# ratschlab/metagraph

Measured on AMD Instinct MI355X. Metric: aligned reads/sec (150 bp, k=31), higher is better.
Workload: dtype int32; 1 GPU; 10000000 synthetic 150 bp reads per GPU vs 104197894-edge k=31 BOSS graph (98 Mbp iid genome + 200000 SNP windows), CLI-default scoring; reads_per_gpu=10000000, graph_edges=104197894, k=31, graph_mode=basic, parallelism=reads sharded x1, graph replicated

## Files before the change

### include/mgx.h

```cpp
#ifndef MGX_H_
#define MGX_H_

#include <stddef.h>
#include <stdint.h>

#ifdef __cplusplus
extern "C" {
#endif

#define MGX_ABI_VERSION 6

enum {
    MGX_OK = 0,
    MGX_ERR_INVALID = -1,
    MGX_ERR_NO_DEVICE = -2,
    MGX_ERR_UNSUPPORTED = -3,
    MGX_ERR_CONFIG = -4,
    MGX_ERR_CAPACITY = -5,
    MGX_ERR_OOM = -6
};

enum { MGX_MODE_BASIC = 0, MGX_MODE_CANONICAL = 1, MGX_MODE_PRIMARY = 2 };

enum { MGX_OP_CLIPPED = 0, MGX_OP_MISMATCH = 1, MGX_OP_MATCH = 2,
       MGX_OP_DELETION = 3, MGX_OP_INSERTION = 4, MGX_OP_NODE_INSERTION = 5 };

typedef struct mgx_boss_view {
    uint32_t k;
    uint32_t sigma;
    uint64_t n_edges;
    const uint8_t *W;
    const uint8_t *last;
    const uint64_t *F;
    const uint8_t *valid;
    uint32_t mode;
    uint32_t on_device;
} mgx_boss_view;

typedef struct mgx_config {
    uint64_t num_alternative_paths;
    uint64_t min_seed_length;
    uint64_t max_seed_length;
    uint64_t max_num_seeds_per_locus;
    int32_t min_cell_score;
    int32_t min_path_score;
    int32_t xdrop;
    int32_t _pad0;
    double min_exact_match;
    double max_nodes_per_seq_char;
    double max_ram_per_alignment;
    double rel_score_cutoff;
    int8_t gap_opening_penalty;
    int8_t gap_extension_penalty;
    int8_t left_end_bonus;
    int8_t right_end_bonus;
    uint8_t forward_and_reverse_complement;
    uint8_t chain_alignments;
    uint8_t post_chain_alignments;
    uint8_t global_xdrop;
    uint8_t allow_left_trim;
    uint8_t no_backtrack;
    uint8_t seed_complexity_filter;
    uint8_t alignment_edit_distance;
    int8_t alignment_match_score;
    int8_t alignment_mm_transition_score;
    int8_t alignment_mm_transversion_score;
    uint8_t _pad1[1];
    int8_t score_matrix[128][128];
} mgx_config;

void mgx_config_init_default(mgx_config *c);
void mgx_config_init_cli(mgx_config *c, uint32_t k);
void mgx_config_set_dna_matrix(mgx_config *c, int8_t match, int8_t mm_transition, int8_t mm_transversion);
void mgx_config_set_unit_matrix(mgx_config *c, int8_t match);
void mgx_config_set_scoring_matrix(mgx_config *c);

#define MGX_MAX_ALTERNATIVE_PATHS 4u

#define MGX_MAX_QUERY_LENGTH 32704u

typedef struct mgx_limits {
    uint32_t max_query_length;
    uint32_t max_columns;
    uint32_t max_seeds;
    uint64_t cell_arena_bytes;
} mgx_limits;
void mgx_limits_init_default(mgx_limits *l, uint32_t max_query_length);
int mgx_aligner_get_limits(const struct mgx_aligner *a, mgx_limits *out);

typedef struct mgx_graph mgx_graph;
typedef struct mgx_aligner mgx_aligner;

typedef struct mgx_cigar_op { uint32_t len; uint8_t op; uint8_t _pad[3]; } mgx_cigar_op;

typedef struct mgx_alignment {
    int32_t score;
    uint32_t offset;
    uint32_t clipping;
    uint32_t end_clipping;
    uint32_t num_matches;
    uint32_t n_nodes;
    uint32_t n_cigar;
    uint32_t seq_len;
    uint64_t nodes_begin;
    uint64_t cigar_begin;
    uint64_t seq_begin;
    uint8_t orientation;
    uint8_t _pad[3];
    uint32_t n_labels;
    uint64_t labels_begin;
} mgx_alignment;

typedef struct mgx_results {
    uint64_t n_queries;
    const uint64_t *aln_begin;
    const mgx_alignment *alignments;
    const uint64_t *nodes;
    const mgx_cigar_op *cigar;
    const char *seqs;
    const int32_t *status;
    const uint32_t *labels;
} mgx_results;

typedef struct mgx_mapping {
    uint64_t n_queries;
    const uint64_t *node_begin;
    const uint64_t *nodes_fwd;
    const uint64_t *nodes_rc;
} mgx_mapping;

typedef struct mgx_stats {
    uint64_t n_reads;
    uint64_t n_rank_lines;
    uint64_t n_select_lines;
    uint64_t n_bit_lines;
    uint64_t n_columns;
    uint64_t n_extensions;
    uint64_t n_seeds;
    uint64_t n_map_lines;
    uint64_t n_capacity_errors;
    uint64_t phase_cycles[8];
    uint64_t extend_cycles[8];
    double seed_kernel_ms, align_kernel_ms;
    double seeding_ms, sort_ms, extend_ms;
    uint64_t n_seed_lines;
    uint64_t n_fast_columns;
    uint64_t extend_kernels;
    uint64_t n_lane_reads;
    double lane_ms;
    uint64_t n_lane_lines;
    uint64_t n_lane_columns;
    uint64_t lane_bail_reads[32];
    uint64_t n_capacity_retried;
    uint64_t n_seed_lane_reads;
    double seed_lane_ms;
    uint64_t seed_lane_left_reads[16];
    uint64_t n_lane_exact_reads;
    uint64_t n_lane_exact_path_reads;
} mgx_stats;
enum { MGX_KERNEL_GRP8 = 1, MGX_KERNEL_GRP8_PRIM = 2, MGX_KERNEL_GRP8_ALT = 4, MGX_KERNEL_EXT64 = 8, MGX_KERNEL_LANE = 16,
       MGX_KERNEL_LAB64 = 32, MGX_KERNEL_GRP8_LAB = 64,
       MGX_KERNEL_LAB64_BX = 128, MGX_KERNEL_GRP8_LAB_BX = 256  };

int mgx_device_count(void);
const char *mgx_last_error(void);
uint32_t mgx_abi_version(void);

int mgx_graph_create(const mgx_boss_view *view, int device, mgx_graph **out);
void mgx_graph_destroy(mgx_graph *g);
uint32_t mgx_graph_k(const mgx_graph *g);
uint64_t mgx_graph_max_index(const mgx_graph *g);
uint64_t mgx_graph_device_bytes(const mgx_graph *g);
uint64_t mgx_graph_num_edges(const mgx_graph *g);
uint32_t mgx_graph_mode(const mgx_graph *g);

int mgx_aligner_create(const mgx_graph *g, const mgx_config *config,
                       const mgx_limits *limits, mgx_aligner **out);
void mgx_aligner_destroy(mgx_aligner *a);
int mgx_aligner_get_config(const mgx_aligner *a, mgx_config *out);

int mgx_align_batch(mgx_aligner *a, const char *seqs, const uint64_t *offsets, uint64_t n_queries,
                    int seqs_on_device, mgx_results *out);

int mgx_align_batch_device(mgx_aligner *a, const char *seqs, const uint64_t *offsets, uint64_t n_queries,
                           int seqs_on_device);
int mgx_fetch_results(mgx_aligner *a, mgx_results *out);
int mgx_device_results(mgx_aligner *a, const void **headers, uint64_t *header_bytes, uint64_t *n_queries,
                       const void **stream, uint64_t *stream_words);
typedef struct mgx_results_sizes { uint64_t n_alignments, n_nodes, n_cigar, n_seq_bytes, n_labels; } mgx_results_sizes;
int mgx_decode_results_device(mgx_aligner *a, mgx_results *out, mgx_results_sizes *sizes);
void mgx_decode_kernel_launch_counts(uint64_t *out4);
uint64_t mgx_device_stream_capacity(const mgx_aligner *a);
typedef struct mgx_raw_store mgx_raw_store;
int mgx_results_from_raw(const void *headers, uint64_t n_queries, const uint32_t *stream, uint64_t stream_words,
                         mgx_raw_store **store, mgx_results *out);
void mgx_raw_store_free(mgx_raw_store *store);
int mgx_chain_alignments(const mgx_config *config, uint32_t k, const mgx_results *in, const char *seqs, const uint64_t *offsets,
                         mgx_raw_store **store, mgx_results *out);
void mgx_aligner_keep_seeds(mgx_aligner *a, int keep);
int mgx_fetch_seed_info(mgx_aligner *a, uint32_t *info6, uint32_t *seeds, uint32_t *max_seeds_out);

int mgx_map_batch(mgx_aligner *a, const char *seqs, const uint64_t *offsets, uint64_t n_queries,
                  int seqs_on_device, mgx_mapping *out);

typedef struct mgx_map_counts { uint32_t n_discovered, n_kmers, n_unique; } mgx_map_counts;
typedef struct mgx_map_summary {
    uint64_t n_queries;
    const mgx_map_counts *counts;
    const uint64_t *node_begin;
    const uint64_t *nodes;
} mgx_map_summary;
enum { MGX_MAP_WANT_NODES = 1, MGX_MAP_KEEP_NODES = 2 };
int mgx_map_summary_batch(mgx_aligner *a, const char *seqs, const uint64_t *offsets, uint64_t n_queries,
                          int seqs_on_device, uint32_t map_length ,
                          uint32_t flags, mgx_map_summary *out);
int mgx_map_present(const mgx_map_counts *c, uint64_t query_len, uint32_t k, uint32_t map_length, double discovery_fraction);
enum { MGX_MAP_FMT_NODES = 0, MGX_MAP_FMT_COUNT_KMERS = 1, MGX_MAP_FMT_QUERY_PRESENCE = 2, MGX_MAP_FMT_FILTER_PRESENT = 3 };
size_t mgx_format_map(const mgx_map_summary *s, uint64_t query_index, const char *header, const char *query, size_t query_len,
                      uint32_t k, uint32_t map_length, int format, double discovery_fraction, char *buf, size_t buf_len);
void mgx_map_kernel_launch_counts(uint64_t *out4);

int mgx_aligner_stats(const mgx_aligner *a, mgx_stats *out);
void mgx_kernel_launch_counts(uint64_t *out5);

int mgx_aligner_set_pipeline(mgx_aligner *a, const char *name);
int mgx_device_trim(int device);
int mgx_aligner_set_stream(mgx_aligner *a, void *hip_stream);
int mgx_aligner_create_stream(mgx_aligner *a);
void *mgx_aligner_get_stream(const mgx_aligner *a);

typedef struct mgx_gather mgx_gather;
uint64_t mgx_gather_unique_id_bytes(void);
int mgx_gather_unique_id(void *id_out, uint64_t id_bytes);
int mgx_gather_create_rank(const void *unique_id, uint64_t id_bytes, int rank, int world, int root, int device, mgx_gather **out);
int mgx_gather_create_comm(void *nccl_comm, int rank, int world, int root, int device, mgx_gather **out);
int mgx_gather_create_local(const int *devices, int n_devices, int root, mgx_gather **out );
void mgx_gather_destroy(mgx_gather *g);
int mgx_gather_world(const mgx_gather *g);
int mgx_gather_rank(const mgx_gather *g);
int mgx_gather_start(mgx_gather *g, mgx_aligner *a);
int mgx_gather_finish(mgx_gather *g, uint64_t *n_queries, const void **headers, const uint32_t **streams, uint64_t *stream_words);

size_t mgx_format_tsv(const mgx_results *res, uint64_t query_index, const char *header,
                      const char *query, size_t query_len, int32_t min_path_score,
                      char *buf, size_t buf_len);

size_t mgx_format_json(const mgx_results *res, uint64_t query_index, const char *header,
                       const char *query, size_t query_len, uint32_t k, char *buf, size_t buf_len);

typedef struct mgx_annotation mgx_annotation;
int mgx_annotation_create(uint64_t n_rows, uint32_t n_labels, const uint64_t *const *columns, int device, mgx_annotation **out);
int mgx_annotation_create_sparse(uint64_t n_rows, uint32_t n_labels, const uint64_t *col_begin, const uint64_t *rows,
                                 int on_device, int device, mgx_annotation **out);
void mgx_annotation_destroy(mgx_annotation *a);
uint64_t mgx_annotation_device_bytes(const mgx_annotation *a);
uint64_t mgx_annotation_num_rows(const mgx_annotation *a);
uint32_t mgx_annotation_num_labels(const mgx_annotation *a);
int mgx_annotation_get_rows(mgx_annotation *a, const uint64_t *rows, uint64_t n, int rows_on_device,
                            uint64_t *out_begin, uint32_t *out_labels, uint64_t cap, int out_on_device, uint64_t *n_labels_out);

int mgx_annotation_set_coordinates(mgx_annotation *a, uint32_t n_labels, const uint64_t *col_begin, const uint64_t *rows,
                                   const uint64_t *coord_begin, const int64_t *coords);
int mgx_annotation_set_coordinates_device(mgx_annotation *a, uint32_t n_labels, const uint64_t *col_begin, const uint64_t *rows,
                                          const uint64_t *coord_begin, const int64_t *coords);
int mgx_annotation_has_coordinates(const mgx_annotation *a);
int mgx_annotation_get_row_tuples(mgx_annotation *a, const uint64_t *rows, uint64_t n, uint64_t *out_begin, uint32_t *out_labels,
                                  uint64_t label_cap, uint64_t *out_coord_begin, int64_t *out_coords, uint64_t coord_cap,
                                  uint64_t *n_labels_out, uint64_t *n_coords_out);

typedef struct mgx_chain_anchor {
    uint64_t label;
    int64_t coordinate;
    int32_t seed_clipping, seed_end;
    int32_t chain_score;
    uint32_t seed_index;
} mgx_chain_anchor;
int mgx_chain_seeds(const mgx_config *config, int device, const mgx_chain_anchor *anchors, const uint64_t *list_begin,
                    const uint32_t *query_size, uint64_t n_lists, mgx_chain_anchor *sorted_out, uint32_t *backtrace_out);

int mgx_seed_chainer_create(const mgx_graph *graph, const mgx_config *config, const mgx_limits *limits,
                            const struct mgx_annotation *annotation, mgx_aligner **out);
typedef struct mgx_chain_seed { uint32_t clipping, length, offset, n_nodes; uint64_t nodes_begin; } mgx_chain_seed;
typedef struct mgx_chain_tables {
    uint64_t n_queries;
    const uint64_t *seed_begin;
    const mgx_chain_seed *seeds;
    const uint64_t *nodes;
    const uint64_t *num_matching;
    const uint64_t *list_begin;
    const mgx_chain_anchor *anchors;
    const uint32_t *backtrace;
    const int32_t *status;
} mgx_chain_tables;
#define MGX_CHAIN_TABLES_ON_DEVICE 1u
int mgx_chain_tables_batch(mgx_aligner *a, const char *seqs, const uint64_t *offsets, uint64_t n, int seqs_on_device,
                           uint32_t flags, mgx_chain_tables *out);
int mgx_chain_tables_fetch(mgx_aligner *a, mgx_chain_tables *out_host);
void mgx_chain_tables_kernel_launch_counts(uint64_t *out4);

int mgx_labeled_aligner_create(const mgx_graph *graph, const mgx_config *config, const mgx_limits *limits,
                               const mgx_annotation *annotation, mgx_aligner **out);
size_t mgx_format_tsv_labeled(const mgx_results *res, uint64_t query_index, const char *header,
                              const char *query, size_t query_len, int32_t min_path_score,
                              const char *const *label_names, uint32_t n_label_names, char *buf, size_t buf_len);
typedef struct mgx_text {
    uint64_t n_queries;
    const char *text;
    const uint64_t *line_begin;
} mgx_text;
int mgx_format_tsv_batch(mgx_aligner *a, const char *headers, const uint64_t *header_offsets,
                         const char *const *label_names, uint32_t n_label_names, mgx_text *out);
void mgx_format_kernel_launch_counts(uint64_t *out4);
int mgx_format_map_batch(mgx_aligner *a, const char *headers, const uint64_t *header_offsets, int format,
                         double discovery_fraction, mgx_text *out);
void mgx_format_map_kernel_launch_counts(uint64_t *out4);
int mgx_format_json_batch(mgx_aligner *a, const char *headers, const uint64_t *header_offsets,
                          uint64_t first, uint64_t n, mgx_text *out);
void mgx_format_json_kernel_launch_counts(uint64_t *out4);

#define MGX_READS_FASTA 1u
#define MGX_READS_FASTQ 2u
typedef struct mgx_read_parser mgx_read_parser;
typedef struct mgx_reads {
    uint64_t n_records, consumed;
    uint32_t format;
    const char *seqs;
    const uint64_t *offsets;
    const uint64_t *host_offsets;
    const char *names;
    const uint64_t *name_offsets;
} mgx_reads;
int mgx_read_parser_create(int device, mgx_read_parser **out);
void mgx_read_parser_destroy(mgx_read_parser *p);
int mgx_parse_reads(mgx_read_parser *p, const char *text, uint64_t n_bytes, int text_on_device, int final, uint32_t flags,
                    mgx_reads *out);
int mgx_read_parser_slice(mgx_read_parser *p, uint64_t first, uint64_t n, const char **seqs, const uint64_t **offsets);
int mgx_read_parser_fetch(mgx_read_parser *p, char *seqs_out, uint64_t *offsets_out);
void mgx_parse_kernel_launch_counts(uint64_t *out4);
void *mgx_pinned_alloc(size_t bytes);
void mgx_pinned_free(void *p);

int mgx_results_from_raw_labeled(const void *headers, uint64_t n_queries, const uint32_t *stream, uint64_t stream_words,
                                 int labeled, mgx_raw_store **store, mgx_results *out);

typedef struct mgx_boss_file {
    uint32_t k;
    uint32_t sigma;
    uint32_t mode;
    uint32_t state;
    uint64_t n_edges;
    const uint64_t *F;
    const uint8_t *W;
    const uint8_t *last;
    void *owner;
} mgx_boss_file;
int mgx_boss_file_read(const char *path, mgx_boss_file *out);
void mgx_boss_file_free(mgx_boss_file *f);
int mgx_edgemask_read(const char *path, uint32_t state, uint64_t n_edges, uint8_t *valid_out);
int mgx_graph_load_dbg(const char *path, int device, mgx_graph **out);
int mgx_graph_load_dbg_device(const char *path, int device, mgx_graph **out);
int mgx_boss_file_decode_device(const char *path, int device, mgx_boss_file *out);
void mgx_dbg_decode_kernel_launch_counts(uint64_t *out4);

typedef struct mgx_column_file mgx_column_file;
int mgx_column_file_read(const char *const *paths, uint32_t n_paths, mgx_column_file **out);
void mgx_column_file_free(mgx_column_file *f);
uint64_t mgx_column_file_num_rows(const mgx_column_file *f);
uint32_t mgx_column_file_num_labels(const mgx_column_file *f);
const char *mgx_column_file_label(const mgx_column_file *f, uint32_t j);
const uint64_t *mgx_column_file_col_begin(const mgx_column_file *f);
const uint64_t *mgx_column_file_rows(const mgx_column_file *f);
int mgx_annotation_create_from_file(const mgx_column_file *f, int device, mgx_annotation **out);
int mgx_column_coord_file_read(const char *const *paths, uint32_t n_paths, mgx_column_file **out);
const uint64_t *mgx_column_file_coord_begin(const mgx_column_file *f);
const int64_t *mgx_column_file_coords(const mgx_column_file *f);
int mgx_annotation_load_columns_device(const char *const *paths, uint32_t n_paths, int device, mgx_annotation **out, mgx_column_file **names_out);
int mgx_column_file_decode_device(const char *const *paths, uint32_t n_paths, int device, mgx_column_file **out);
int mgx_annotation_load_coord_columns_device(const char *const *paths, uint32_t n_paths, int device, mgx_annotation **out, mgx_column_file **names_out);
int mgx_column_coord_file_decode_device(const char *const *paths, uint32_t n_paths, int device, mgx_column_file **out);
void mgx_column_decode_kernel_launch_counts(uint64_t *out4);

#ifdef __cplusplus
}
#endif
#endif
```

### metagraph_amd/capi.py

```python
import ctypes as C
import os

MGX_OK = 0
MGX_ABI_VERSION = 6
MGX_ERR_INVALID, MGX_ERR_NO_DEVICE, MGX_ERR_UNSUPPORTED, MGX_ERR_CONFIG, MGX_ERR_CAPACITY, MGX_ERR_OOM = -1, -2, -3, -4, -5, -6
OP_CHARS = "SX=DIG"


class BossView(C.Structure):
    _fields_ = [("k", C.c_uint32), ("sigma", C.c_uint32), ("n_edges", C.c_uint64),
                ("W", C.c_void_p), ("last", C.c_void_p), ("F", C.POINTER(C.c_uint64)),
                ("valid", C.c_void_p), ("mode", C.c_uint32), ("on_device", C.c_uint32)]


class BossFile(C.Structure):
    _fields_ = [("k", C.c_uint32), ("sigma", C.c_uint32), ("mode", C.c_uint32), ("state", C.c_uint32), ("n_edges", C.c_uint64),
                ("F", C.POINTER(C.c_uint64)), ("W", C.POINTER(C.c_uint8)), ("last", C.POINTER(C.c_uint8)), ("owner", C.c_void_p)]


class Config(C.Structure):
    _fields_ = [("num_alternative_paths", C.c_uint64), ("min_seed_length", C.c_uint64),
                ("max_seed_length", C.c_uint64), ("max_num_seeds_per_locus", C.c_uint64),
                ("min_cell_score", C.c_int32), ("min_path_score", C.c_int32), ("xdrop", C.c_int32),
                ("_pad0", C.c_int32),
                ("min_exact_match", C.c_double), ("max_nodes_per_seq_char", C.c_double),
                ("max_ram_per_alignment", C.c_double), ("rel_score_cutoff", C.c_double),
                ("gap_opening_penalty", C.c_int8), ("gap_extension_penalty", C.c_int8),
                ("left_end_bonus", C.c_int8), ("right_end_bonus", C.c_int8),
                ("forward_and_reverse_complement", C.c_uint8), ("chain_alignments", C.c_uint8),
                ("post_chain_alignments", C.c_uint8), ("global_xdrop", C.c_uint8),
                ("allow_left_trim", C.c_uint8), ("no_backtrack", C.c_uint8),
                ("seed_complexity_filter", C.c_uint8), ("alignment_edit_distance", C.c_uint8),
                ("alignment_match_score", C.c_int8), ("alignment_mm_transition_score", C.c_int8),
                ("alignment_mm_transversion_score", C.c_int8), ("_pad1", C.c_uint8 * 1),
                ("score_matrix", (C.c_int8 * 128) * 128)]


class Limits(C.Structure):
    _fields_ = [("max_query_length", C.c_uint32), ("max_columns", C.c_uint32), ("max_seeds", C.c_uint32),
                ("cell_arena_bytes", C.c_uint64)]


class CigarOp(C.Structure):
    _fields_ = [("len", C.c_uint32), ("op", C.c_uint8), ("_pad", C.c_uint8 * 3)]


class Alignment(C.Structure):
    _fields_ = [("score", C.c_int32), ("offset", C.c_uint32), ("clipping", C.c_uint32),
                ("end_clipping", C.c_uint32), ("num_matches", C.c_uint32), ("n_nodes", C.c_uint32),
                ("n_cigar", C.c_uint32), ("seq_len", C.c_uint32), ("nodes_begin", C.c_uint64),
                ("cigar_begin", C.c_uint64), ("seq_begin", C.c_uint64), ("orientation", C.c_uint8),
                ("_pad", C.c_uint8 * 3), ("n_labels", C.c_uint32), ("labels_begin", C.c_uint64)]


class Results(C.Structure):
    _fields_ = [("n_queries", C.c_uint64), ("aln_begin", C.POINTER(C.c_uint64)),
                ("alignments", C.POINTER(Alignment)), ("nodes", C.POINTER(C.c_uint64)),
                ("cigar", C.POINTER(CigarOp)), ("seqs", C.POINTER(C.c_char)), ("status", C.POINTER(C.c_int32)),
                ("labels", C.POINTER(C.c_uint32))]


class ResultsSizes(C.Structure):
    _fields_ = [("n_alignments", C.c_uint64), ("n_nodes", C.c_uint64), ("n_cigar", C.c_uint64), ("n_seq_bytes", C.c_uint64),
                ("n_labels", C.c_uint64)]


class Mapping(C.Structure):
    _fields_ = [("n_queries", C.c_uint64), ("node_begin", C.POINTER(C.c_uint64)),
                ("nodes_fwd", C.POINTER(C.c_uint64)), ("nodes_rc", C.POINTER(C.c_uint64))]


class MapCounts(C.Structure):
    _fields_ = [("n_discovered", C.c_uint32), ("n_kmers", C.c_uint32), ("n_unique", C.c_uint32)]


class MapSummary(C.Structure):
    _fields_ = [("n_queries", C.c_uint64), ("counts", C.POINTER(MapCounts)),
                ("node_begin", C.POINTER(C.c_uint64)), ("nodes", C.POINTER(C.c_uint64))]


class Text(C.Structure):
    _fields_ = [("n_queries", C.c_uint64), ("text", C.c_void_p), ("line_begin", C.POINTER(C.c_uint64))]


class Reads(C.Structure):
    _fields_ = [("n_records", C.c_uint64), ("consumed", C.c_uint64), ("format", C.c_uint32), ("seqs", C.c_void_p),
                ("offsets", C.c_void_p), ("host_offsets", C.POINTER(C.c_uint64)), ("names", C.c_void_p),
                ("name_offsets", C.POINTER(C.c_uint64))]


class ChainAnchor(C.Structure):
    _fields_ = [("label", C.c_uint64), ("coordinate", C.c_int64), ("seed_clipping", C.c_int32), ("seed_end", C.c_int32),
                ("chain_score", C.c_int32), ("seed_index", C.c_uint32)]


class ChainSeed(C.Structure):
    _fields_ = [("clipping", C.c_uint32), ("length", C.c_uint32), ("offset", C.c_uint32), ("n_nodes", C.c_uint32),
                ("nodes_begin", C.c_uint64)]


class ChainTables(C.Structure):
    _fields_ = [("n_queries", C.c_uint64), ("seed_begin", C.POINTER(C.c_uint64)), ("seeds", C.POINTER(ChainSeed)),
                ("nodes", C.POINTER(C.c_uint64)), ("num_matching", C.POINTER(C.c_uint64)), ("list_begin", C.POINTER(C.c_uint64)),
                ("anchors", C.POINTER(ChainAnchor)), ("backtrace", C.POINTER(C.c_uint32)), ("status", C.POINTER(C.c_int32))]


MGX_CHAIN_TABLES_ON_DEVICE = 1
MGX_READS_FASTA, MGX_READS_FASTQ = 1, 2
MGX_MAP_WANT_NODES = 1
MGX_MAP_KEEP_NODES = 2
MGX_MAP_FMT_NODES, MGX_MAP_FMT_COUNT_KMERS, MGX_MAP_FMT_QUERY_PRESENCE, MGX_MAP_FMT_FILTER_PRESENT = 0, 1, 2, 3


class Stats(C.Structure):
    _fields_ = [("n_reads", C.c_uint64), ("n_rank_lines", C.c_uint64), ("n_select_lines", C.c_uint64),
                ("n_bit_lines", C.c_uint64), ("n_columns", C.c_uint64), ("n_extensions", C.c_uint64),
                ("n_seeds", C.c_uint64), ("n_map_lines", C.c_uint64), ("n_capacity_errors", C.c_uint64), ("phase_cycles", C.c_uint64 * 8), ("extend_cycles", C.c_uint64 * 8),
                ("seed_kernel_ms", C.c_double), ("align_kernel_ms", C.c_double),
                ("seeding_ms", C.c_double), ("sort_ms", C.c_double), ("extend_ms", C.c_double), ("n_seed_lines", C.c_uint64),
                ("n_fast_columns", C.c_uint64), ("extend_kernels", C.c_uint64), ("n_lane_reads", C.c_uint64),
                ("lane_ms", C.c_double), ("n_lane_lines", C.c_uint64), ("n_lane_columns", C.c_uint64),
                ("lane_bail_reads", C.c_uint64 * 32), ("n_capacity_retried", C.c_uint64),
                ("n_seed_lane_reads", C.c_uint64), ("seed_lane_ms", C.c_double), ("seed_lane_left_reads", C.c_uint64 * 16),
                ("n_lane_exact_reads", C.c_uint64), ("n_lane_exact_path_reads", C.c_uint64)]


KERNEL_GRP8, KERNEL_GRP8_PRIM, KERNEL_GRP8_ALT, KERNEL_EXT64, KERNEL_LANE, KERNEL_LAB64, KERNEL_GRP8_LAB = 1, 2, 4, 8, 16, 32, 64
KERNEL_LAB64_BX, KERNEL_GRP8_LAB_BX = 128, 256


def results_to_py(res):
    out = []
    for q in range(res.n_queries):
        alns = []
        for ai in range(res.aln_begin[q], res.aln_begin[q + 1]):
            a = res.alignments[ai]
            nodes = [res.nodes[a.nodes_begin + i] for i in range(a.n_nodes)]
            cig = "".join("%d%s" % (res.cigar[a.cigar_begin + i].len, OP_CHARS[res.cigar[a.cigar_begin + i].op])
                          for i in range(a.n_cigar))
            seq = C.string_at(C.addressof(res.seqs.contents) + a.seq_begin, a.seq_len).decode() if a.seq_len else ""
            d = {"score": a.score, "offset": a.offset, "clipping": a.clipping,
                 "end_clipping": a.end_clipping, "num_matches": a.num_matches, "nodes": nodes,
                 "cigar": cig, "sequence": seq, "orientation": int(a.orientation)}
            if res.labels:
                d["labels"] = [res.labels[a.labels_begin + i] for i in range(a.n_labels)]
            alns.append(d)
        out.append(alns)
    return out


def chain_alignments(config, k, res, queries):
    import numpy as np
    blob = b"".join(q.encode() if isinstance(q, str) else bytes(q) for q in queries)
    offs = np.zeros(len(queries) + 1, dtype=np.uint64)
    offs[1:] = np.cumsum([len(q) for q in queries])
    store, out = C.c_void_p(), Results()
    rc = lib().mgx_chain_alignments(C.byref(config), k, C.byref(res), blob, offs.ctypes.data, C.byref(store), C.byref(out))
    if rc:
        raise RuntimeError(lib().mgx_last_error().decode())
    try:
        return results_to_py(out)
    finally:
        lib().mgx_raw_store_free(store)


def results_arrays(res):
    import numpy as np
    n = int(res.n_queries)

    def arr(ptr, count, dtype):
        if not count:
            return np.zeros(0, dtype=dtype)
        nbytes = count * np.dtype(dtype).itemsize
        return np.frombuffer((C.c_char * nbytes).from_address(C.addressof(ptr.contents)), dtype=dtype, count=count)

    aln_begin = arr(res.aln_begin, n + 1, np.uint64)
    na = int(aln_begin[-1]) if n else 0
    aln_dt = np.dtype([("score", "<i4"), ("offset", "<u4"), ("clipping", "<u4"), ("end_clipping", "<u4"),
                       ("num_matches", "<u4"), ("n_nodes", "<u4"), ("n_cigar", "<u4"), ("seq_len", "<u4"),
                       ("nodes_begin", "<u8"), ("cigar_begin", "<u8"), ("seq_begin", "<u8"), ("orientation", "u1"),
                       ("_pad", "u1", (3,)), ("n_labels", "<u4"), ("labels_begin", "<u8")])
    assert aln_dt.itemsize == C.sizeof(Alignment)
    alns = arr(res.alignments, na, aln_dt)
    tn = int(alns["n_nodes"].sum()) if na else 0
    tc = int(alns["n_cigar"].sum()) if na else 0
    ts = int(alns["seq_len"].sum()) if na else 0
    cig_dt = np.dtype([("len", "<u4"), ("op", "u1"), ("_pad", "u1", (3,))])
    return {"n": n, "aln_begin": aln_begin, "alns": alns, "nodes": arr(res.nodes, tn, np.uint64),
            "cigar": arr(res.cigar, tc, cig_dt), "seqs": arr(res.seqs, ts, np.uint8),
            "status": arr(res.status, n, np.int32)}


def count_result_mismatches(res_a, res_b):
    import numpy as np
    a, b = results_arrays(res_a), results_arrays(res_b)
    assert a["n"] == b["n"]
    fields = ["score", "offset", "clipping", "end_clipping", "num_matches", "n_nodes", "n_cigar", "seq_len", "orientation"]
    same = np.array_equal(a["aln_begin"], b["aln_begin"]) and len(a["alns"]) == len(b["alns"]) \
        and all(np.array_equal(a["alns"][f], b["alns"][f]) for f in fields) \
        and np.array_equal(a["nodes"], b["nodes"]) and np.array_equal(a["cigar"]["len"], b["cigar"]["len"]) \
        and np.array_equal(a["cigar"]["op"], b["cigar"]["op"]) and np.array_equal(a["seqs"], b["seqs"])
    if same:
        return 0
    pa, pb = results_to_py(res_a), results_to_py(res_b)
    return sum(1 for x, y in zip(pa, pb) if x != y)


_ROOT = os.path.dirname(os.path.dirname(os.path.abspath(__file__)))
LIB_PATH = os.environ.get("MGX_LIB_PATH") or os.path.join(_ROOT, "metagraph_amd", "_build", "libmgx.so")
_lib = None


def lib():
    global _lib
    if _lib is not None:
        return _lib
    if not os.path.exists(LIB_PATH):
        raise OSError("libmgx.so not built: run `python -c 'import __graft_entry__ as g; g.build()'` "
                      "(needs hipcc); the aligner has no CPU fallback")
    L = C.CDLL(LIB_PATH)
    L.mgx_last_error.restype = C.c_char_p
    L.mgx_abi_version.restype = C.c_uint32
    if L.mgx_abi_version() != MGX_ABI_VERSION:
        raise OSError("libmgx.so has ABI version %d, this binding was written for %d: rebuild" % (L.mgx_abi_version(), MGX_ABI_VERSION))
    L.mgx_annotation_create.argtypes = [C.c_uint64, C.c_uint32, C.POINTER(C.c_void_p), C.c_int, C.POINTER(C.c_void_p)]
    L.mgx_annotation_destroy.argtypes = [C.c_void_p]
    L.mgx_annotation_create_sparse.argtypes = [C.c_uint64, C.c_uint32, C.c_void_p, C.c_void_p, C.c_int, C.c_int, C.POINTER(C.c_void_p)]
    L.mgx_labeled_aligner_create.argtypes = [C.c_void_p, C.POINTER(Config), C.POINTER(Limits), C.c_void_p, C.POINTER(C.c_void_p)]
    L.mgx_seed_chainer_create.argtypes = [C.c_void_p, C.POINTER(Config), C.POINTER(Limits), C.c_void_p, C.POINTER(C.c_void_p)]
    L.mgx_chain_tables_batch.argtypes = [C.c_void_p, C.c_void_p, C.c_void_p, C.c_uint64, C.c_int, C.c_uint32, C.POINTER(ChainTables)]
    L.mgx_chain_tables_fetch.argtypes = [C.c_void_p, C.POINTER(ChainTables)]
    L.mgx_chain_tables_kernel_launch_counts.argtypes = [C.POINTER(C.c_uint64)]
    L.mgx_chain_tables_kernel_launch_counts.restype = None
    L.mgx_format_tsv_labeled.argtypes = [C.POINTER(Results), C.c_uint64, C.c_char_p, C.c_char_p, C.c_size_t, C.c_int32,
                                         C.POINTER(C.c_char_p), C.c_uint32, C.c_char_p, C.c_size_t]
    L.mgx_format_tsv_labeled.restype = C.c_size_t
    L.mgx_annotation_device_bytes.argtypes = [C.c_void_p]
    L.mgx_annotation_device_bytes.restype = C.c_uint64
    L.mgx_annotation_get_rows.argtypes = [C.c_void_p, C.c_void_p, C.c_uint64, C.c_int, C.c_void_p, C.c_void_p, C.c_uint64, C.c_int,
                                          C.POINTER(C.c_uint64)]
    L.mgx_device_count.restype = C.c_int
    L.mgx_boss_file_read.argtypes = [C.c_char_p, C.POINTER(BossFile)]
    L.mgx_boss_file_free.argtypes = [C.POINTER(BossFile)]
    L.mgx_edgemask_read.argtypes = [C.c_char_p, C.c_uint32, C.c_uint64, C.c_void_p]
    L.mgx_graph_load_dbg.argtypes = [C.c_char_p, C.c_int, C.POINTER(C.c_void_p)]
    L.mgx_graph_load_dbg_device.argtypes = [C.c_char_p, C.c_int, C.POINTER(C.c_void_p)]
    L.mgx_boss_file_decode_device.argtypes = [C.c_char_p, C.c_int, C.POINTER(BossFile)]
    L.mgx_dbg_decode_kernel_launch_counts.argtypes = [C.POINTER(C.c_uint64)]
    L.mgx_dbg_decode_kernel_launch_counts.restype = None
    L.mgx_column_file_read.argtypes = [C.POINTER(C.c_char_p), C.c_uint32, C.POINTER(C.c_void_p)]
    L.mgx_column_file_free.argtypes = [C.c_void_p]
    L.mgx_column_file_num_rows.argtypes = [C.c_void_p]
    L.mgx_column_file_num_rows.restype = C.c_uint64
    L.mgx_column_file_num_labels.argtypes = [C.c_void_p]
    L.mgx_column_file_num_labels.restype = C.c_uint32
    L.mgx_column_file_label.argtypes = [C.c_void_p, C.c_uint32]
    L.mgx_column_file_label.restype = C.c_char_p
    L.mgx_column_file_col_begin.argtypes = [C.c_void_p]
    L.mgx_column_file_col_begin.restype = C.POINTER(C.c_uint64)
    L.mgx_column_file_rows.argtypes = [C.c_void_p]
    L.mgx_column_file_rows.restype = C.POINTER(C.c_uint64)
    L.mgx_annotation_create_from_file.argtypes = [C.c_void_p, C.c_int, C.POINTER(C.c_void_p)]
    L.mgx_annotation_load_columns_device.argtypes = [C.POINTER(C.c_char_p), C.c_uint32, C.c_int, C.POINTER(C.c_void_p), C.POINTER(C.c_void_p)]
    L.mgx_column_file_decode_device.argtypes = [C.POINTER(C.c_char_p), C.c_uint32, C.c_int, C.POINTER(C.c_void_p)]
    L.mgx_column_coord_file_read.argtypes = [C.POINTER(C.c_char_p), C.c_uint32, C.POINTER(C.c_void_p)]
    L.mgx_column_file_coord_begin.argtypes = [C.c_void_p]
    L.mgx_column_file_coord_begin.restype = C.POINTER(C.c_uint64)
    L.mgx_column_file_coords.argtypes = [C.c_void_p]
    L.mgx_column_file_coords.restype = C.POINTER(C.c_int64)
    L.mgx_annotation_load_coord_columns_device.argtypes = [C.POINTER(C.c_char_p), C.c_uint32, C.c_int, C.POINTER(C.c_void_p), C.POINTER(C.c_void_p)]
    L.mgx_column_coord_file_decode_device.argtypes = [C.POINTER(C.c_char_p), C.c_uint32, C.c_int, C.POINTER(C.c_void_p)]
    L.mgx_column_decode_kernel_launch_counts.argtypes = [C.POINTER(C.c_uint64)]
    L.mgx_column_decode_kernel_launch_counts.restype = None
    L.mgx_graph_create.argtypes = [C.POINTER(BossView), C.c_int, C.POINTER(C.c_void_p)]
    L.mgx_graph_destroy.argtypes = [C.c_void_p]
    L.mgx_graph_k.argtypes = [C.c_void_p]
    L.mgx_graph_k.restype = C.c_uint32
    L.mgx_graph_max_index.argtypes = [C.c_void_p]
    L.mgx_graph_max_index.restype = C.c_uint64
    L.mgx_graph_device_bytes.argtypes = [C.c_void_p]
    L.mgx_graph_num_edges.argtypes = [C.c_void_p]
    L.mgx_graph_num_edges.restype = C.c_uint64
    L.mgx_graph_mode.argtypes = [C.c_void_p]
    L.mgx_graph_mode.restype = C.c_uint32
    L.mgx_graph_device_bytes.restype = C.c_uint64
    L.mgx_aligner_create.argtypes = [C.c_void_p, C.POINTER(Config), C.POINTER(Limits), C.POINTER(C.c_void_p)]
    L.mgx_aligner_destroy.argtypes = [C.c_void_p]
    L.mgx_aligner_get_config.argtypes = [C.c_void_p, C.POINTER(Config)]
    L.mgx_aligner_get_limits.argtypes = [C.c_void_p, C.POINTER(Limits)]
    L.mgx_align_batch.argtypes = [C.c_void_p, C.c_void_p, C.c_void_p, C.c_uint64, C.c_int, C.POINTER(Results)]
    L.mgx_align_batch_device.argtypes = [C.c_void_p, C.c_void_p, C.c_void_p, C.c_uint64, C.c_int]
    L.mgx_fetch_results.argtypes = [C.c_void_p, C.POINTER(Results)]
    L.mgx_aligner_keep_seeds.argtypes = [C.c_void_p, C.c_int]
    L.mgx_device_results.argtypes = [C.c_void_p, C.POINTER(C.c_void_p), C.POINTER(C.c_uint64), C.POINTER(C.c_uint64),
                                     C.POINTER(C.c_void_p), C.POINTER(C.c_uint64)]
    L.mgx_device_stream_capacity.argtypes = [C.c_void_p]
    L.mgx_device_stream_capacity.restype = C.c_uint64
    L.mgx_results_from_raw.argtypes = [C.c_void_p, C.c_uint64, C.c_void_p, C.c_uint64, C.POINTER(C.c_void_p), C.POINTER(Results)]
    L.mgx_chain_alignments.argtypes = [C.POINTER(Config), C.c_uint32, C.POINTER(Results), C.c_char_p, C.c_void_p,
                                       C.POINTER(C.c_void_p), C.POINTER(Results)]
    L.mgx_chain_alignments.restype = C.c_int
    L.mgx_results_from_raw_labeled.argtypes = [C.c_void_p, C.c_uint64, C.c_void_p, C.c_uint64, C.c_int, C.POINTER(C.c_void_p), C.POINTER(Results)]
    L.mgx_raw_store_free.argtypes = [C.c_void_p]
    L.mgx_gather_unique_id_bytes.restype = C.c_uint64
    L.mgx_gather_unique_id.argtypes = [C.c_void_p, C.c_uint64]
    L.mgx_gather_create_rank.argtypes = [C.c_void_p, C.c_uint64, C.c_int, C.c_int, C.c_int, C.c_int, C.POINTER(C.c_void_p)]
    L.mgx_gather_create_comm.argtypes = [C.c_void_p, C.c_int, C.c_int, C.c_int, C.c_int, C.POINTER(C.c_void_p)]
    L.mgx_gather_create_local.argtypes = [C.POINTER(C.c_int), C.c_int, C.c_int, C.POINTER(C.c_void_p)]
    L.mgx_gather_destroy.argtypes = [C.c_void_p]
    L.mgx_gather_destroy.restype = None
    L.mgx_gather_world.argtypes = [C.c_void_p]
    L.mgx_gather_rank.argtypes = [C.c_void_p]
    L.mgx_gather_start.argtypes = [C.c_void_p, C.c_void_p]
    L.mgx_gather_finish.argtypes = [C.c_void_p, C.POINTER(C.c_uint64), C.POINTER(C.c_void_p), C.POINTER(C.c_void_p), C.POINTER(C.c_uint64)]
    L.mgx_map_batch.argtypes = [C.c_void_p, C.c_void_p, C.c_void_p, C.c_uint64, C.c_int, C.POINTER(Mapping)]
    L.mgx_map_summary_batch.argtypes = [C.c_void_p, C.c_void_p, C.c_void_p, C.c_uint64, C.c_int, C.c_uint32, C.c_uint32,
                                        C.POINTER(MapSummary)]
    L.mgx_map_present.argtypes = [C.POINTER(MapCounts), C.c_uint64, C.c_uint32, C.c_uint32, C.c_double]
    L.mgx_format_map.argtypes = [C.POINTER(MapSummary), C.c_uint64, C.c_char_p, C.c_char_p, C.c_size_t, C.c_uint32, C.c_uint32,
                                 C.c_int, C.c_double, C.c_char_p, C.c_size_t]
    L.mgx_format_map.restype = C.c_size_t
    L.mgx_map_kernel_launch_counts.argtypes = [C.POINTER(C.c_uint64)]
    L.mgx_map_kernel_launch_counts.restype = None
    L.mgx_format_tsv_batch.argtypes = [C.c_void_p, C.c_char_p, C.c_void_p, C.POINTER(C.c_char_p), C.c_uint32, C.POINTER(Text)]
    L.mgx_format_kernel_launch_counts.argtypes = [C.POINTER(C.c_uint64)]
    L.mgx_format_kernel_launch_counts.restype = None
    L.mgx_format_map_batch.argtypes = [C.c_void_p, C.c_char_p, C.c_void_p, C.c_int, C.c_double, C.POINTER(Text)]
    L.mgx_format_map_kernel_launch_counts.argtypes = [C.POINTER(C.c_uint64)]
    L.mgx_format_map_kernel_launch_counts.restype = None
    L.mgx_format_json_batch.argtypes = [C.c_void_p, C.c_char_p, C.c_void_p, C.c_uint64, C.c_uint64, C.POINTER(Text)]
    L.mgx_format_json_kernel_launch_counts.argtypes = [C.POINTER(C.c_uint64)]
    L.mgx_format_json_kernel_launch_counts.restype = None
    L.mgx_decode_results_device.argtypes = [C.c_void_p, C.POINTER(Results), C.POINTER(ResultsSizes)]
    L.mgx_decode_kernel_launch_counts.argtypes = [C.POINTER(C.c_uint64)]
    L.mgx_decode_kernel_launch_counts.restype = None
    L.mgx_read_parser_create.argtypes = [C.c_int, C.POINTER(C.c_void_p)]
    L.mgx_read_parser_destroy.argtypes = [C.c_void_p]
    L.mgx_read_parser_destroy.restype = None
    L.mgx_parse_reads.argtypes = [C.c_void_p, C.c_void_p, C.c_uint64, C.c_int, C.c_int, C.c_uint32, C.POINTER(Reads)]
    L.mgx_read_parser_slice.argtypes = [C.c_void_p, C.c_uint64, C.c_uint64, C.POINTER(C.c_void_p), C.POINTER(C.c_void_p)]
    L.mgx_read_parser_fetch.argtypes = [C.c_void_p, C.c_void_p, C.c_void_p]
    L.mgx_parse_kernel_launch_counts.argtypes = [C.POINTER(C.c_uint64)]
    L.mgx_parse_kernel_launch_counts.restype = None
    L.mgx_pinned_alloc.argtypes = [C.c_size_t]
    L.mgx_pinned_alloc.restype = C.c_void_p
    L.mgx_pinned_free.argtypes = [C.c_void_p]
    L.mgx_pinned_free.restype = None
    L.mgx_aligner_stats.argtypes = [C.c_void_p, C.POINTER(Stats)]
    L.mgx_config_init_default.argtypes = [C.POINTER(Config)]
    L.mgx_config_init_cli.argtypes = [C.POINTER(Config), C.c_uint32]
    L.mgx_config_set_dna_matrix.argtypes = [C.POINTER(Config), C.c_int8, C.c_int8, C.c_int8]
    L.mgx_config_set_unit_matrix.argtypes = [C.POINTER(Config), C.c_int8]
    L.mgx_config_set_scoring_matrix.argtypes = [C.POINTER(Config)]
    L.mgx_limits_init_default.argtypes = [C.POINTER(Limits), C.c_uint32]
    L.mgx_format_tsv.argtypes = [C.POINTER(Results), C.c_uint64, C.c_char_p, C.c_char_p, C.c_size_t,
                                 C.c_int32, C.c_char_p, C.c_size_t]
    L.mgx_format_tsv.restype = C.c_size_t
    L.mgx_format_json.argtypes = [C.POINTER(Results), C.c_uint64, C.c_char_p, C.c_char_p, C.c_size_t,
                                  C.c_uint32, C.c_char_p, C.c_size_t]
    L.mgx_format_json.restype = C.c_size_t
    _lib = L
    return L


INT32_MAX = 2**31 - 1
NINF = -2**31 + 100
UINT64_MAX = 2**64 - 1
DBL_MAX = 1.7976931348623157e308


def config_default():
    c = Config()
    c.num_alternative_paths = 1
    c.max_num_seeds_per_locus = UINT64_MAX
    c.min_cell_score = NINF
    c.min_path_score = 0
    c.xdrop = INT32_MAX
    c.min_exact_match = 0.0
    c.max_nodes_per_seq_char = DBL_MAX
    c.max_ram_per_alignment = DBL_MAX
    c.rel_score_cutoff = 0.0
    c.gap_opening_penalty = -5
    c.gap_extension_penalty = -2
    c.forward_and_reverse_complement = 1
    c.global_xdrop = 1
    c.allow_left_trim = 1
    c.seed_complexity_filter = 1
    return c


def set_dna_matrix(c, match, transition, transversion):
    for i in range(128):
        for j in range(128):
            c.score_matrix[i][j] = transversion
    for a, b in (("A", "G"), ("G", "A"), ("C", "T"), ("T", "C")):
        c.score_matrix[ord(a)][ord(b)] = transition
    for a in "ACGT":
        c.score_matrix[ord(a)][ord(a)] = match


def set_unit_matrix(c, match):
    for i in range(128):
        for j in range(128):
            c.score_matrix[i][j] = -match
    for a in "ACGT":
        c.score_matrix[ord(a)][ord(a)] = match


def config_cli(k):
    c = config_default()
    c.min_seed_length = min(19, k)
    c.max_seed_length = UINT64_MAX
    c.max_num_seeds_per_locus = 1000
    c.min_path_score = 0
    c.xdrop = 27
    c.min_exact_match = 0.7
    c.max_nodes_per_seq_char = 5.0
    c.max_ram_per_alignment = 200.0
    c.rel_score_cutoff = 0.95
    c.gap_opening_penalty = -6
    c.gap_extension_penalty = -2
    c.left_end_bonus = 5
    c.right_end_bonus = 5
    c.alignment_edit_distance = 0
    c.alignment_match_score, c.alignment_mm_transition_score, c.alignment_mm_transversion_score = 2, 3, 3
    set_dna_matrix(c, 2, -3, -3)
    return c
# ... 10 lines not shown
```

### metagraph_amd/csrc/host_state.hpp

```cpp
#pragma once
#include <hip/hip_runtime.h>

#include <algorithm>
#include <chrono>
#include <cstdio>
#include <cstdlib>
#include <cstring>
#include <map>
#include <mutex>
#include <string>
#include <vector>

#include "../../include/mgx.h"
#include "host_common.hpp"

#define MGX_INTERNAL __attribute__((visibility("hidden")))

MGX_INTERNAL int fail(int code, const char *fmt, ...);
MGX_INTERNAL int hip_fail(hipError_t e, const char *expr, const char *file, int line);

#define HIP_TRY(expr)                                                                              \
    do {                                                                                           \
        hipError_t e_ = (expr);                                                                    \
        if (e_ != hipSuccess) return hip_fail(e_, #expr, __FILE__, __LINE__);                      \
    } while (0)

struct DevPool {
    enum { MAX_DEV = 16 };
    std::mutex mu;
    std::multimap<size_t, void *> blocks[MAX_DEV];
    size_t held[MAX_DEV] = { 0 };
    static int dev() { int d = 0; (void)hipGetDevice(&d); return d >= 0 && d < MAX_DEV ? d : -1; }
    void *take(size_t want, size_t *got) {
        const int d = dev();
        if (d < 0) return nullptr;
        std::lock_guard<std::mutex> lock(mu);
        auto it = blocks[d].lower_bound(want);
        if (it == blocks[d].end() || it->first > want + want / 2 + (1u << 20)) return nullptr;
        void *p = it->second;
        *got = it->first;
        held[d] -= it->first;
        blocks[d].erase(it);
        return p;
    }
    void give(void *p, size_t bytes) {
        const int d = dev();
        if (d < 0) { (void)hipFree(p); return; }
        std::lock_guard<std::mutex> lock(mu);
        blocks[d].emplace(bytes, p);
        held[d] += bytes;
    }
    size_t held_bytes() {
        const int d = dev();
        if (d < 0) return 0;
        std::lock_guard<std::mutex> lock(mu);
        return held[d];
    }
    void flush() {
        const int d = dev();
        if (d < 0) return;
        std::lock_guard<std::mutex> lock(mu);
        for (auto &e : blocks[d]) (void)hipFree(e.second);
        blocks[d].clear();
        held[d] = 0;
    }
};
MGX_INTERNAL extern DevPool g_pool;

struct DevBuf {
    void *p = nullptr;
    size_t bytes = 0;
    bool pooled = false;
    ~DevBuf() { release(); }
    void release() {
        if (!p) return;
        if (pooled) g_pool.give(p, bytes); else (void)hipFree(p);
        p = nullptr; bytes = 0;
    }
    int ensure(size_t n, bool exact = false) {
        if (n <= bytes) return MGX_OK;
        release();
        size_t want = exact ? n : n + n / 8 + 256;
        if (pooled) {
            size_t got = 0;
            if (void *q = g_pool.take(want, &got)) { p = q; bytes = got; return MGX_OK; }
        }
        hipError_t e = hipMalloc(&p, want);
        if (e != hipSuccess && g_pool.held_bytes()) {
            (void)hipGetLastError();
            g_pool.flush();
            e = hipMalloc(&p, want);
        }
        if (e != hipSuccess) { p = nullptr; return fail(MGX_ERR_OOM, "hipMalloc(%zu) failed: %s", want, hipGetErrorString(e)); }
        bytes = want;
        return MGX_OK;
    }
    template <class T> T *as() const { return static_cast<T *>(p); }
};

struct mgx_graph {
    int device = 0;
    mgx::DevGraph g;
    DevBuf blocks, last_hint, w_hint[4], sel_anchor, firstc, terminus, valid, prefix_tbl;
    uint64_t bytes = 0;
    uint32_t mode = MGX_MODE_BASIC;
    bool primary_tables = false;
    mutable std::mutex label_mu;
    mutable DevBuf canon_repr;
    mutable bool canon_repr_ready = false;
    mutable std::map<uint64_t, bool> dummy_clean;
};

#ifdef MGX_PROBES
static inline bool probe_env_set(const char *name) { const char *e = getenv(name); return e && *e && strcmp(e, "0") != 0; }
static inline uint32_t probe_env_u32(const char *name, uint32_t dflt) { const char *e = getenv(name); return e ? (uint32_t)atoi(e) : dflt; }
static inline uint32_t probe_env_pct(const char *name) { const char *e = getenv(name); return e ? (uint32_t)std::min(100, std::max(1, atoi(e))) : 100u; }
#else
static inline bool probe_env_set(const char *) { return false; }
static inline uint32_t probe_env_u32(const char *, uint32_t dflt) { return dflt; }
static inline uint32_t probe_env_pct(const char *) { return 100u; }
#endif
static inline bool env_int(const char *name, int *v) {
    const char *e = getenv(name);
    if (e) *v = atoi(e);
    return e != nullptr;
}

struct HostStageTimer {
    const char *name;
    std::chrono::steady_clock::time_point t0;
    static bool on() { static const bool v = probe_env_set("MGX_HOST_TIMERS"); return v; }
    explicit HostStageTimer(const char *n) : name(n), t0(std::chrono::steady_clock::now()) {}
    ~HostStageTimer() {
        if (on()) fprintf(stderr, "mgx host stage %-14s %8.1f us\n", name,
                          std::chrono::duration<double, std::micro>(std::chrono::steady_clock::now() - t0).count());
    }
};

enum CursorSlot {
    CUR_OUT = 0,
    CUR_READ = 1,
    CUR_SEED = 2,
    CUR_LMAX = CUR_SEED,
    CUR_RETRY = 3,
    CUR_MAP = 4,
    CUR_LANE_BAIL = 5,
    CUR_LANE_DONE = 6,
    CUR_SL_BAIL = 8,
    CUR_SL_DONE = 9,
    CUR_SL_BAIL2 = 10,
    CUR_SL_BAIL_BACK = 11,
    CUR_WORDS = 16
};

enum AlignEvent {
    EV_MAP_BEGIN, EV_MAP_END,
    EV_ALIGN_BEGIN, EV_ALIGN_END,
    EV_SEEDED,
    EV_SORTED,
    EV_LANE_END,
    EV_SEED_LANE_END,
    EV_COUNT
};

struct ChainTabState {
    enum { CT_PAIRS = 0, CT_SEEDS, CT_NODES, CT_ANCHORS, CT_ARRAYS };
    DevBuf counts, begins;
    DevBuf pair_key, pair_key_alt, pair_val, pair_val_alt;
    DevBuf kept, n_kept;
    DevBuf seeds, nodes, num_matching, status, qsize, penalty;
    DevBuf anchors, anchors_alt, backtrace, perm, perm_alt, k32, k32_alt, k64, k64_alt, sort_tmp, sort_tmp_anchors;
    std::vector<int32_t> h_penalty;
    uint64_t n = 0, n_seeds = 0, n_nodes = 0, n_anchors = 0;
    bool have = false;
    std::vector<uint64_t> h_seed_begin, h_nodes, h_num_matching, h_list_begin;
    std::vector<mgx_chain_seed> h_seeds;
    std::vector<mgx_chain_anchor> h_anchors;
    std::vector<uint32_t> h_backtrace;
    std::vector<int32_t> h_status;
};

struct mgx_aligner {
    const mgx_graph *graph = nullptr;
    const mgx_annotation *anno = nullptr;
    bool anno_dummy_clean = false;
    bool chainer = false;
    ChainTabState ct;
    mgx_config cfg;
    mgx::DevConfig dcfg;
    mgx_limits user_lim;
    bool have_user_lim = false;
    DevBuf mlen_fwd, mlen_rc;
    DevBuf pk_fwd, pk_rc, iv_fwd, iv_rc;
    DevBuf rng_fwd, rng_rc;
    bool have_rng = false;
    DevBuf score_matrix, seqs, offsets, counts, node_begin, nodes_fwd, nodes_rc, arena, results, stream, cursors, d_stats, d_stats_map, scan_tmp, dbg_seeds;
    DevBuf seed_hdr, seed_stream, work_key, work_key_sorted, order_in, order, sort_tmp, retry_list;
    DevBuf resume_pool[2], retry_list2, retry_key[2];
    DevBuf lane_scratch, lane_params, lane_bail, lane_hist;
    bool packed_valid = false;
    uint32_t lane_epoch = 0;
    uint64_t lane_done = 0;
    uint64_t lane_exact = 0;
    uint64_t lane_exact_path = 0;
    unsigned long long lane_hist_h[32] = { 0 };
    DevBuf seedlane_scratch, seedlane_params, seedlane_bail, seedlane_hist;
    uint64_t seedlane_launched = 0;
    uint32_t n_passes = 0;
    mgx::DevLimits lim;
    uint64_t n_reads = 0, total_kmers = 0;
    uint32_t n_slots = 0;
    bool keep_seeds = false;
    std::vector<mgx::ReadResult> h_results;
    std::vector<uint32_t> h_stream;
    mgx::HostResults host;
    mgx::HostResults host_chained;
    mgx::HostResults host_retried;
    bool retry_capacity = true;
    uint32_t label_scale = 1;
    const char *last_d_seqs = nullptr;
    const uint64_t *last_d_offsets = nullptr;
    hipStream_t hstream = nullptr;
    int device = 0;
    bool own_stream = false;
    uint64_t stage_generation = 0;
    uint64_t aligned_generation = 0;
    std::vector<uint64_t> m_node_begin, m_fwd, m_rc;
    DevBuf ms_counts, ms_nodes, ms_sorted;
    std::vector<mgx_map_counts> h_ms_counts;
    std::vector<uint64_t> h_ms_nodes;
    uint64_t ms_generation = 0;
    const char *ms_d_seqs = nullptr;
    const uint64_t *ms_d_offsets = nullptr;
    uint32_t ms_map_length = 0, ms_lmax = 0;
    bool ms_have_nodes = false;
    DevBuf mf_threshold;
    std::vector<uint64_t> h_mf_threshold;
    DevBuf tf_headers, tf_header_offsets, tf_names, tf_len, tf_begin, tf_text, tf_cap, tf_patch;
    char *h_text = nullptr;
    size_t h_text_bytes = 0;
    std::vector<uint64_t> h_line_begin;
    DevBuf rd_counts, rd_begins, rd_totals, rd_alns, rd_nodes, rd_cigar, rd_seqs, rd_status, rd_labels;
    enum { RD_H_ALN_BEGIN = 0, RD_H_ALNS, RD_H_NODES, RD_H_CIGAR, RD_H_SEQS, RD_H_STATUS, RD_H_LABELS, RD_H_N };
    void *h_rd[RD_H_N] = {};
    size_t h_rd_bytes[RD_H_N] = {};
    bool aligned_empty = false;
    mgx_stats hstats;
    hipEvent_t ev[EV_COUNT] = {};
    uint64_t kernels_ran = 0;
    uint64_t seed_scale = 1, seed_cap = 0;
    uint64_t arena_stride = 0;
    uint64_t out_words = 0;
    uint64_t out_min_words = 0;
    bool no_fast = false;
    struct Options {
        int ext64 = 1;
        int groups_per_wave = -1;
        int multi_pass = -1;
        int resume_cap = -1;
        int no_compact = 0, no_alias = 0, no_bt_runs = 0, no_flat = 0;
        int lane = -1;
        int exact = -1;
        int seed_lane = -1;
        int seed_wps = 8;
        int device_share = 1;
        int decode_on_device = 0;
        int map_pipe = 1;
    } opt;
};

static inline unsigned long long *cursor(const mgx_aligner *A, CursorSlot s) { return A->cursors.as<unsigned long long>() + s; }
static inline hipError_t clear_cursors(mgx_aligner *A, CursorSlot first, CursorSlot last) {
    return hipMemsetAsync(cursor(A, first), 0, (size_t)(last - first + 1) * 8, A->hstream);
}
static inline hipError_t copy_sync(mgx_aligner *A, void *dst, const void *src, size_t bytes, hipMemcpyKind kind) {
    if (hipError_t e = hipMemcpyAsync(dst, src, bytes, kind, A->hstream)) return e;
    return hipStreamSynchronize(A->hstream);
}

MGX_INTERNAL int aligner_create(const mgx_graph *g, const mgx_config *config, const mgx_limits *limits, const mgx_annotation *anno,
                                mgx_aligner **out);
MGX_INTERNAL int collect_stats(mgx_aligner *A, bool mapped, bool aligned);
MGX_INTERNAL int run_seeding(mgx_aligner *A, const char *d_seqs, const uint64_t *d_offsets, uint64_t n, uint32_t Lmax, uint64_t *seeds_wanted);
MGX_INTERNAL int refuse_chainer(const mgx_aligner *A, const char *call);
MGX_INTERNAL int exclusive_sum(mgx_aligner *A, uint64_t *in, uint64_t *out, uint64_t n);
MGX_INTERNAL hipError_t load_sort_kernels();
MGX_INTERNAL hipError_t load_map_kernels();

MGX_INTERNAL int graph_dummy_rows_clean(const mgx_graph *g, const mgx_annotation *anno, bool *clean);
MGX_INTERNAL int graph_canon_repr(const mgx_graph *g);

MGX_INTERNAL int stage_batch(mgx_aligner *A, const char *seqs, const uint64_t *offsets, uint64_t n, int on_device,
                             const char **d_seqs, const uint64_t **d_offsets, uint32_t *Lmax_out, uint32_t window = 0);
MGX_INTERNAL int run_map(mgx_aligner *A, const char *d_seqs, const uint64_t *d_offsets, uint64_t n, bool do_rc, bool mapped, uint32_t Lmax,
                         bool raw_edges = false);

MGX_INTERNAL int realign_capacity_queries(mgx_aligner *A, const char *d_seqs, const uint64_t *d_offsets, uint64_t n,
                                          const std::vector<uint64_t> &todo, std::vector<mgx::HostResults> &fixed,
                                          std::vector<uint8_t> &have, std::vector<uint64_t> &h_off, std::vector<char> &h_seq);
```

### metagraph_amd/csrc/kernel_units.hpp

```cpp
#pragma once
#include <stddef.h>
#include <stdint.h>

constexpr size_t MGX_ALIGN_PARAMS_BYTES = 728;
constexpr size_t MGX_LANE_PARAMS_BYTES = 856;
constexpr size_t MGX_SEED_LANE_PARAMS_BYTES = 824;
constexpr size_t MGX_DEV_GRAPH_BYTES = 160;
constexpr size_t MGX_FORMAT_ARGS_BYTES = 128;
constexpr size_t MGX_PARSE_ARGS_BYTES = 144;
constexpr size_t MGX_MAPFMT_ARGS_BYTES = 120;
constexpr size_t MGX_JSONFMT_ARGS_BYTES = 120;
constexpr size_t MGX_DECODE_ARGS_BYTES = 104;
constexpr unsigned MGX_SEED_STATIC_LDS_BYTES = 1792;

#ifndef MGX_SEL_ANCHOR_MAX
#define MGX_SEL_ANCHOR_MAX 8192
#endif

struct mgx_annotation;

extern "C" {

void mgx_set_last_error(const char *msg);

#define MGX_DECLARE_GRP8_BUILD(sfx)                                                                                          \
    int mgx_launch_align_grp8##sfx(const void *params, uint32_t n_groups, uint32_t lds_bytes, int phase, void *stream);      \
    int mgx_grp_waves_per_simd8##sfx(void);                                                                                  \
    unsigned mgx_grp_static_lds8##sfx(void);
MGX_DECLARE_GRP8_BUILD()
MGX_DECLARE_GRP8_BUILD(_prim)
MGX_DECLARE_GRP8_BUILD(_alt)
MGX_DECLARE_GRP8_BUILD(_lab)
MGX_DECLARE_GRP8_BUILD(_labx)
#undef MGX_DECLARE_GRP8_BUILD
int mgx_grp_max_alt8_lab(void);
int mgx_grp_max_alt8_labx(void);

int mgx_launch_ext64(const void *params, uint32_t blocks, uint32_t lds_bytes, void *stream);
unsigned mgx_ext64_static_lds(void);
int mgx_ext64_waves_per_simd(void);
int mgx_launch_lab64(const void *params, uint32_t blocks, uint32_t lds_bytes, void *stream);
unsigned mgx_lab64_static_lds(void);
int mgx_lab64_waves_per_simd(void);
int mgx_lab64_max_alt(void);
int mgx_launch_lab64x(const void *params, uint32_t blocks, uint32_t lds_bytes, void *stream);
unsigned mgx_lab64x_static_lds(void);
int mgx_lab64x_waves_per_simd(void);
int mgx_lab64x_max_alt(void);

int mgx_launch_seed(const void *params, uint32_t blocks, uint32_t lds_bytes, int wps8, void *stream);
int mgx_launch_seed_primary(const void *params, uint32_t blocks, uint32_t lds_bytes, int wps8, void *stream);
unsigned mgx_seed_static_lds(void);
int mgx_seed_load(void);

int mgx_launch_lane(const void *d_params, uint32_t blocks, void *stream);
int mgx_launch_lane_exact(const void *d_params, uint32_t blocks, int labeled, void *stream);
int mgx_lane_waves_per_simd(void);

int mgx_launch_seed_lane(const void *d_params, uint32_t blocks, int long_reads, void *stream);
int mgx_seed_lane_waves_per_simd(void);

int mgx_launch_map_summary(const uint64_t *node_begin, const uint32_t *fwd, const uint32_t *rc, uint32_t *sorted, void *counts,
                           uint64_t *out_nodes, const uint64_t *valid, uint64_t n_reads, uint32_t n_edges, int mode, int long_form,
                           void *stream);
int mgx_launch_map_subk(const void *dev_graph, const char *seqs, const uint64_t *offsets, const uint64_t *node_begin, uint32_t *nodes,
                        uint64_t n_reads, uint32_t map_length, void *stream);
uint32_t mgx_map_summary_short_max(void);

int mgx_launch_format_size(const void *args, void *stream);
int mgx_launch_format_write(const void *args, void *stream);
int mgx_launch_format_patch(uint64_t *line_len, const uint32_t *queries, const uint64_t *lens, uint32_t m, void *stream);

int mgx_launch_mapfmt_size(const void *args, void *stream);
int mgx_launch_mapfmt_write(const void *args, void *stream);

int mgx_launch_jsonfmt_size(const void *args, void *stream);
int mgx_launch_jsonfmt_write(const void *args, void *stream);

int mgx_launch_decode_size(const void *args, void *stream);
int mgx_launch_decode_write(const void *args, void *stream);

int mgx_launch_parse_count(const void *args, void *stream);
int mgx_launch_parse_table(const void *args, void *stream);
int mgx_launch_parse_classify(const void *args, void *stream);
int mgx_launch_parse_records(const void *args, void *stream);
int mgx_launch_parse_copy(const void *args, int names, void *stream);

void mgx_annotation_device_view(const mgx_annotation *a, int *device, uint64_t *n_rows, const uint64_t **head,
                                const uint32_t **count, const uint32_t **more);
uint64_t mgx_annotation_uid(const mgx_annotation *a);
void mgx_annotation_coord_view(const mgx_annotation *a, const uint64_t **row_entry, const uint64_t **coord_off, const int64_t **coords);

}
```

### metagraph_amd/csrc/lane_read.hpp

```cpp
#pragma once
#include "lane_types.hpp"

namespace mgx {

struct LaneChip {
    int32_t lane;
    uint64_t *qw; int32_t qstride;
    uint32_t *cold; int32_t cstride;
};

enum { CD_B_SCORE, CD_B_NOD, CD_B_I, CD_B_POS, CD_T_SCORE, CD_T_NOD, CD_T_POS,
       CD_FA_ALIVE, CD_FA_CONV, CD_FA_MAX,
       CD_D_SCORE0, CD_D_SCORE1, CD_D_SCORE2, CD_D_MAX0, CD_D_MAX1, CD_D_MAX2,
       CD_KID_N0, CD_KID_C, CD_KID_N1, CD_KID_R0, CD_KID_R1,
       CD_TABLE_CAP, CD_TSB_LO, CD_TSB_HI, CD_CELL_TOP, CD_NCOLS, CD_F_NODE, CD_F_IDX, CD_F_MAX,
       CD_SEED_LEN, CD_SEED_OFF, CD_NODE0, CD_CTR, CD_FWD_N_NODES, CD_FWD_N_SEQ, CD_HMS, CD_REPLAY_TOP, CD_S8_FILTER,
       LANE_COLD_WORDS };
static_assert(LANE_MAX_DEFER == 3, "CD_D_* above");
#define LANE_CI(f) (*(int32_t *)(chip.cold + (f) * chip.cstride))
#define LANE_CU(f) (*(chip.cold + (f) * chip.cstride))
#define LANE_REPLAY_MATCHING() ((LANE_CI(CD_HMS) >> 4) & 1)
#define LANE_SET_REPLAY_MATCHING(v) (LANE_CI(CD_HMS) = (LANE_CI(CD_HMS) & ~16) | ((v) ? 16 : 0))
#define LANE_TIE_MODE() ((LANE_CI(CD_HMS) >> 5) & 1)
#define LANE_SET_TIE_MODE(v) (LANE_CI(CD_HMS) = (LANE_CI(CD_HMS) & ~32) | ((v) ? 32 : 0))
// ... 844 lines not shown
        if (LANE_TIE_MODE() && ((double)tsize / (double)window_size >= cfg.max_nodes_per_seq_char
                                || (double)table_size_bytes() / 1000000.0 > cfg.max_ram_per_alignment)) LANE_BAIL(27);
        LANE_OPAQUE(read);
        const int32_t seed_off = c_seed_off, seed_len = c_seed_len;
        const uint32_t node0 = c_node0;
        const int32_t sroot = (cfg.left_end_bonus && !clipping) ? cfg.left_end_bonus : 0;
        const int32_t root_pushes = (int32_t)gld(arec() + 19), root_size = 1 + root_pushes;
        const int32_t root_ins = imax(sroot + go, NINF + ge);
        auto root_S = [&](int32_t pos) -> int32_t {
            return pos == 0 ? sroot : (pos >= 1 && pos <= root_pushes ? root_ins + (pos - 1) * ge : NINF);
        };
        (void)seed_len;
        if (!pass) {
        const int s = LANE_STRAND();
        const SeedHdr *hp2 = P.seed_hdr + read;
        const DevSeed *seeds = P.seed_stream + gld(&hp2->off) + (s ? (int32_t)gld(&hp2->n_seeds[0]) : 0);
        const uint32_t *rnodes = (s ? P.nodes_rc : P.nodes_fwd) + gld(P.node_begin + read);
        bool node0_merged = false;
        for (int32_t t = 1; t < n; ++t) {
            const DevSeed *sj = seeds + t;
            const int32_t cl = (int32_t)gld(&sj->clipping), len = (int32_t)gld(&sj->length), so = (int32_t)gld(&sj->offset);
            const int32_t nn = (int32_t)gld(&sj->n_nodes);
            const uint32_t ln = so == 0 ? gld(rnodes + cl + nn - 1) : gld(&sj->node);
            const int32_t lpos = len + cl - 1;
            const int32_t lscore = len * m + (!cl ? cfg.left_end_bonus : 0) + (!(L - cl - len) ? cfg.right_end_bonus : 0);
            if (ln == node0) {
                int32_t *cv = (int32_t *)(arec() + 32);
                if (!node0_merged) {
                    gst(arec() + 13, 0u); gst(arec() + 14, 0u);
                    for (int32_t c = 1; c < tsize; ++c) {
                        if (gld(lane_slot_word(slots(), c, 8)) != node0) break;
                        if (!(gld(lane_slot_word(slots(), c, 10)) & LANE_GEOM_ROW)) LANE_BAIL(7);
                        (void)lane_merge_column(slots(), LP.max_cols, cv, arec() + 13, c, start, cfg.rel_score_cutoff);
                    }
                    node0_merged = true;
                }
                const int32_t vstart = (int32_t)gld(arec() + 13), vlen = (int32_t)gld(arec() + 14);
                if (vlen == 0 || lpos < vstart || lpos - vstart >= vlen) LANE_BAIL(19);
                if ((int32_t)gld(cv + lpos) < lscore) LANE_BAIL(19);
                continue;
            }
            uint32_t hs = lane_hash(ln, hmask);
            int32_t idx = -1;
            for (;;) {
                const uint64_t he = gld(htab() + hs);
                if ((uint32_t)(he >> 44) != ptag) break;
                if ((uint32_t)he == ln) { idx = (int32_t)((he >> 32) & 0xFFFu); break; }
                hs = (hs + 1) & hmask;
            }
            if (idx < 0) LANE_BAIL(19);
            if (gld(lane_slot_word(slots(), idx, 8)) != ln) LANE_BAIL(19);
            const uint32_t geom = gld(lane_slot_word(slots(), idx, 10));
            const int32_t cbegin = (int32_t)(geom & 0xFFFF), csize = (int32_t)((geom >> 16) & 0xFF);
            const int32_t skip = cbegin ? 0 : 1;
            const int32_t qs = start + cbegin - (cbegin ? 1 : 0), qn = csize - skip;
            if (lpos < qs || lpos - qs >= qn) LANE_BAIL(19);
            if (!(geom & LANE_GEOM_ROW)) LANE_BAIL(19);
            const int32_t a = lpos - start + 1, x = a - (cbegin & ~3);
            int32_t v = NINF;
            if (a - cbegin >= 0 && a - cbegin < csize + 5 && x < LFW) {
                const int32_t d = (int32_t)(int8_t)gld(lane_s8_byte(slots(), LP.max_cols, idx, x));
                if (d != -128) v = (int32_t)gld(lane_slot_word(slots(), idx, 9)) + d;
            }
            if (v < lscore) LANE_BAIL(19);
        }
        }
        bool got = b_score != INT32_MIN;
        if (!got && !pass) LANE_BAIL(18);
        int32_t x_score = 0, x_offset = 0, x_clip = 0, x_end_clip = 0, x_n_runs = 0, x_j_hi = 0, x_n_nodes = 0, x_n_seq = 0;
        if (got) {
        const int32_t k_minus_1 = k - 1;
        const int32_t min_trace_length = k - seed_off;
        const int32_t cap = (int32_t)lim.max_path;
        const int32_t j_start = b_i;
        int32_t j = b_i, pos = b_pos;
        const int32_t score = b_score, end_pos = b_pos;
        int32_t n_runs = 0, n_trace = 0, n_seq = 0, n_path = 0;
        uint32_t cur_run = 0;
        int32_t align_offset = seed_off;
        int32_t j_stop = j;
        bool bad = false;
        auto push_op = [&](uint32_t op, uint32_t num) {
            if (n_runs == 0 || (cur_run & 7) != op) {
                if (n_runs >= LANE_MAX_RUNS) { bad = true; return; }
                if (n_runs) gst(lane_run_word(slots(), LP.max_cols, n_runs - 1), cur_run);
                cur_run = (num << 3) | op;
                ++n_runs;
            } else {
                cur_run += num << 3;
            }
        };
        auto slot_geom = [&](int32_t jj) -> uint32_t { return gld(lane_slot_word(slots(), jj, 10)); };
        auto slot_link = [&](int32_t jj) -> uint32_t { return gld(lane_slot_word(slots(), jj, 11)); };
        auto slot_flags = [&](int32_t jj, uint32_t geom, int32_t p) -> uint32_t {
            const int32_t begin = (int32_t)(geom & 0xFFFF), size = (int32_t)((geom >> 16) & 0xFF);
            const int32_t jx = p - begin, x = p - (begin & ~3);
            if (!(jx >= 0 && jx < size + 5 && x < LFW)) return 0;
            return gld(lane_slot_flag(slots(), jj, x));
        };
        for (;;) {
            if (!j) break;
            const uint32_t geom = slot_geom(j);
            const uint32_t link = slot_link(j);
            const uint32_t ccode = (geom >> 24) & 7u;
            const int32_t col_offset = (int32_t)(link >> 16);
            align_offset = imin(col_offset, k_minus_1);
            const uint32_t fl = slot_flags(j, geom, pos);
            const uint32_t last_op = n_runs ? (cur_run & 7) : 99u;
            if (!(fl & CF_REAL)) {
                j_stop = j;
                j = 0;
            } else if (pos && (fl & CF_S_IS_E) && (n_runs == 0 || last_op != OP_DELETION)) {
                uint32_t lop = OP_INSERTION;
                while (lop == OP_INSERTION && !bad) {
                    push_op(lop, 1);
                    lop = (slot_flags(j, geom, pos) & CF_E_EXT) ? OP_INSERTION : OP_MATCH;
                    --pos;
                }
            } else if (pos && (fl & CF_MATCH)) {
                ++n_trace;
                const int32_t ap = clipping + pos;
                const uint32_t op = (ap >= 1 && ap <= L) ? (qcode(ap - 1) + 1 == ccode ? OP_MATCH : OP_MISMATCH) : OP_CLIPPED;
                ++n_seq;
                push_op(op, 1);
                if (col_offset >= k_minus_1) ++n_path;
                --pos;
                j = (int32_t)(link & 0xFFFFu);
                j_stop = j;
            } else if ((fl & CF_S_IS_F) && (n_runs == 0 || last_op != OP_INSERTION)) {
                uint32_t lop = OP_DELETION;
                while (lop == OP_DELETION && j && !bad) {
                    const uint32_t g2 = slot_geom(j);
                    const uint32_t l2 = slot_link(j);
                    const int32_t o2 = (int32_t)(l2 >> 16);
                    align_offset = imin(o2, k_minus_1);
                    lop = (slot_flags(j, g2, pos) & CF_F_EXT) ? OP_DELETION : OP_MATCH;
                    ++n_trace;
                    ++n_seq;
                    push_op(OP_DELETION, 1);
                    if (o2 >= k_minus_1) ++n_path;
                    j = (int32_t)(l2 & 0xFFFFu);
                    j_stop = j;
                }
            } else {
                j_stop = j;
                break;
            }
            if (bad || n_seq > cap || n_path > cap) LANE_BAIL(20);
        }
        if (bad) LANE_BAIL(21);
        if (n_runs) gst(lane_run_word(slots(), LP.max_cols, n_runs - 1), cur_run);
        if (!(n_trace >= min_trace_length && n_path)) LANE_BAIL(22);
        {
            int32_t cur_cell_score;
            if (j == 0) {
                cur_cell_score = root_S(pos);
                if (!(pos >= 0 && pos < root_size + 5)) cur_cell_score = NINF;
            } else {
                const uint32_t geom = slot_geom(j);
                const int32_t begin = (int32_t)(geom & 0xFFFF), size = (int32_t)((geom >> 16) & 0xFF);
                const int32_t jx = pos - begin, x = pos - (begin & ~3);
                cur_cell_score = NINF;
                if (jx >= 0 && jx < size + 5 && x < LFW) {
                    if (!(geom & LANE_GEOM_ROW)) LANE_BAIL(29);
                    const int32_t v = (int32_t)(int8_t)gld(lane_s8_byte(slots(), LP.max_cols, j, x));
                    const int32_t cb = (int32_t)gld(lane_slot_word(slots(), j, 9));
                    if (v != -128) cur_cell_score = cb + v;
                }
            }
            const int32_t bt_best = score - cur_cell_score;
            if (score - min_cell_score < bt_best) LANE_BAIL(23);
            if (!(score >= min_start_score && (!pos || cur_cell_score == 0) && (pos || cur_cell_score == sroot)
                  && (cfg.allow_left_trim || !j))) LANE_BAIL(24);
        }
        x_clip = clipping + pos;
        x_end_clip = L - (clipping + end_pos);
        x_score = score; x_offset = align_offset; x_n_runs = n_runs;
        (void)j_stop;
        x_j_hi = j_start; x_n_seq = n_seq; x_n_nodes = n_path;
        if (x_offset && x_n_nodes > 1) {
            const int32_t trim = imin(x_offset, x_n_nodes - 1);
            if (trim > 0) { x_n_nodes -= trim; x_offset -= trim; }
        }
        }
        if (!pass) {
            gst(arec() + 0, (uint32_t)x_score); gst(arec() + 1, (uint32_t)x_offset); gst(arec() + 2, (uint32_t)x_clip);
            gst(arec() + 3, (uint32_t)x_end_clip); gst(arec() + 4, (uint32_t)x_n_runs); gst(arec() + 5, (uint32_t)x_j_hi);
            gst(arec() + 6, (uint32_t)x_n_nodes); gst(arec() + 7, (uint32_t)x_n_seq);
            LANE_SET_HAVE_ALN(1); LANE_SET_MODE(LANE_EMIT_SLOTS);
            if (!have_rc) break;
            if (!(x_score >= cfg.min_path_score)) LANE_SET_HAVE_ALN(0);
            if (!(x_clip && !x_offset)) break;
            if (!x_n_nodes) LANE_BAIL(26);
            {
                int32_t jj = x_j_hi, ni = x_n_nodes - 1;
                for (int32_t xx = x_n_seq - 1; xx >= 0; --xx) {
                    const uint32_t node = gld(lane_slot_word(slots(), jj, 8)), geom = gld(lane_slot_word(slots(), jj, 10)), link = gld(lane_slot_word(slots(), jj, 11));
                    gst(pa_code() + xx, (geom >> 24) & 7u);
                    if ((int32_t)(link >> 16) >= k - 1) { if (ni >= 0) gst(pa_node() + ni, node); --ni; }
                    jj = (int32_t)(link & 0xFFFFu);
                }
                for (int32_t xx = 0; xx < x_n_runs; ++xx) gst(runs_fwd() + xx, gld(lane_run_word(slots(), LP.max_cols, xx)));
            }
            gst(arec() + 8, (uint32_t)LANE_HAVE_ALN()); gst(arec() + 9, (uint32_t)x_score); gst(arec() + 10, (uint32_t)x_clip);
            gst(arec() + 11, (uint32_t)x_end_clip);
            c_fwd_n_nodes = x_n_nodes; c_fwd_n_seq = x_n_seq;
            LANE_SET_MODE(LANE_EMIT_ARRAYS);
            gst(arec() + 18, (uint32_t)x_end_clip);
            c_seed_len = x_n_seq; c_seed_off = 0; c_node0 = gld(pa_node() + (x_n_nodes - 1));
            if (!load_strand(1 - LANE_STRAND())) LANE_BAIL(5);
            LANE_CU(CD_S8_FILTER) = 0;
            return LR_AGAIN;
        }
        const int32_t fw_added = (int32_t)gld(arec() + 8);
        if (!got) { if (!fw_added) LANE_BAIL(31); break; }
        if (!x_offset && x_n_nodes) {
            bool take = true;
            if (fw_added) {
                const int32_t fw_score = (int32_t)gld(arec() + 9), fw_clip = (int32_t)gld(arec() + 10), fw_end_clip = (int32_t)gld(arec() + 11);
                const int32_t gcut = fw_score > 0 ? (int32_t)((double)fw_score * cfg.rel_score_cutoff) : fw_score;
                const int32_t b_qlen = L - x_clip - x_end_clip, f_qlen = L - fw_clip - fw_end_clip;
                const int32_t b_clip_rev = x_end_clip;
                const bool less = fw_score != x_score ? fw_score > x_score : (b_qlen != f_qlen ? b_qlen > f_qlen : b_clip_rev > fw_clip);
                if (x_score < gcut || less) take = false;
            }
            if (take) {
                LANE_SET_HAVE_ALN(1); LANE_SET_MODE(LANE_EMIT_SLOTS_REVERSED);
                gst(arec() + 0, (uint32_t)x_score); gst(arec() + 1, 0u); gst(arec() + 2, (uint32_t)x_end_clip);
                gst(arec() + 3, (uint32_t)x_clip); gst(arec() + 4, (uint32_t)x_n_runs); gst(arec() + 5, (uint32_t)x_j_hi);
                gst(arec() + 6, (uint32_t)x_n_nodes); gst(arec() + 7, (uint32_t)x_n_seq);
            }
        }
        } while (0);
    }
    LANE_T(5);
    {
        ReadResult &rr = R.rr;
        rr.status = ST_OK; rr.n_alignments = 0; rr.score = 0; rr.offset = 0; rr.n_nodes = rr.n_cigar = rr.seq_len = 0;
        rr.orientation = 0; rr.stream_off = 0;
        const SeedHdr *hp = P.seed_hdr + read;
        rr.num_matches_fwd = gld(&hp->num_matching[0]); rr.num_matches_rc = gld(&hp->num_matching[1]);
        rr.n_seeds_fwd = (uint32_t)gld(&hp->n_seeds[0]); rr.n_seeds_rc = (uint32_t)gld(&hp->n_seeds[1]);
        if (P.labeled) {
            const uint32_t nsw = gld(arec() + 15), nmw = gld(arec() + 25);
            rr.n_seeds_fwd = nsw & 0xFFFFu; rr.n_seeds_rc = nsw >> 16; rr.num_matches_fwd = nmw & 0xFFFFu; rr.num_matches_rc = nmw >> 16;
        }
        rr.n_extensions = (uint32_t)n_extensions; rr.n_columns = n > 0 ? (uint32_t)cols_done : 0u;
    }
    gst(arec() + 26, gld(arec() + 26) + (n > 0 ? (uint32_t)cols_done : 0u));
    gst(arec() + 27, gld(arec() + 27) + (LANE_CU(CD_CTR) & 0xFFFFu));
    gst(arec() + 28, gld(arec() + 28) + (LANE_CU(CD_CTR) >> 16));
    {
        const int32_t have_aln = n > 0 ? LANE_HAVE_ALN() : 0;
        const int32_t a_n_nodes = have_aln ? (int32_t)gld(arec() + 6) : 0;
        R.have_aln = (have_aln && a_n_nodes) ? 1 : 0;
        R.mode = LANE_MODE();
        R.strand = LANE_STRAND();
        R.words = 0; R.trim = 0;
        if (R.have_aln) {
            R.score = (int32_t)gld(arec() + 0); R.offset = (int32_t)gld(arec() + 1); R.clip = (int32_t)gld(arec() + 2);
            R.end_clip = (int32_t)gld(arec() + 3); R.n_runs = (int32_t)gld(arec() + 4); R.j_hi = (int32_t)gld(arec() + 5);
            R.n_nodes = a_n_nodes; R.n_seq = (int32_t)gld(arec() + 7);
            R.words = (uint32_t)R.n_nodes + (uint32_t)((R.clip ? 1 : 0) + R.n_runs + (R.end_clip ? 1 : 0)) + ((uint32_t)R.n_seq + 3) / 4;
            if (P.labeled) { R.words += 2; R.label = LANE_LABEL(); }
        }
    }
    LANE_T(6);
    return LR_DONE;
}

#undef replay_top
#undef c_fwd_n_nodes
#undef c_fwd_n_seq
#undef c_seed_len
#undef c_seed_off
#undef c_node0
#undef b_score
#undef b_nod
#undef b_i
#undef b_pos
#undef t_score
#undef t_nod
#undef t_pos
#undef fa_alive
#undef fa_conv
#undef fa_max_val
#undef d_score
#undef d_max
#undef kid_node0
#undef kid_codes
#undef kid_node1
#undef kid_rank0
#undef kid_rank1
#undef table_cap
#undef tsb_lo
#undef tsb_hi
#undef table_size_bytes
#undef cell_top
#undef cols_done
#undef f_node
#undef f_idx
#undef f_max_val

enum { LANE_EXACT_NONE = 0, LANE_EXACT_SPAN = 1, LANE_EXACT_PATH = 2 };

struct alignas(16) LaneNodeQuad { uint32_t v[4]; };
MGX_DEV bool lane_all_nodes(const uint32_t *p, const int32_t n) {
    int32_t x = 0;
    for (; x < n && ((uintptr_t)(p + x) & 15u); ++x)
        if (!gld(p + x)) return false;
    for (; x + 4 <= n; x += 4) {
        const LaneNodeQuad q = gld((const LaneNodeQuad *)(p + x));
        if (!q.v[0] || !q.v[1] || !q.v[2] || !q.v[3]) return false;
    }
    for (; x < n; ++x)
        if (!gld(p + x)) return false;
    return true;
}

MGX_DEV bool lane_exact_label_filter(const AlignParams &P, const uint64_t read, const SeedHdr *hp, const int32_t L, const bool have_rc,
                                     int32_t ns[2], uint32_t nm[2], uint32_t *label_out) {
    const int32_t k = (int32_t)P.g.k;
    uint32_t label = 0;
    bool have_label = false;
    const int32_t ns0_h = ns[0];
    for (int s2 = 0; s2 < 2; ++s2) {
        const int32_t n_in = ns[s2];
        if (!n_in) continue;
        if (s2 && !have_rc) continue;
        const DevSeed *sd0 = P.seed_stream + gld(&hp->off) + (s2 ? ns0_h : 0);
        const uint32_t *rn = (s2 ? P.nodes_rc : P.nodes_fwd) + gld(P.node_begin + read);
        uint64_t cov[4] = { 0, 0, 0, 0 };
        uint32_t cnt_m = 0;
        int32_t last_end = 0;
        bool counting = true;
        for (int32_t j = 0; j < n_in; ++j) {
            const DevSeed *sj = sd0 + j;
            const int32_t cl = (int32_t)gld(&sj->clipping), so = (int32_t)gld(&sj->offset), len = (int32_t)gld(&sj->length);
            const uint32_t node0 = so == 0 ? gld(rn + cl) : gld(&sj->node);
            uint64_t h = 0;
            if (node0 && node0 <= P.g.n && (uint64_t)node0 - 1 < P.anno_rows) h = gld(P.anno_head + ((uint64_t)node0 - 1));
            if ((h & 0xFFFF) != 1) return false;
            const uint32_t lbl = (uint32_t)(h >> 16);
            if (!have_label) { label = lbl; have_label = true; } else if (lbl != label) return false;
            const int32_t lo = cl, hi = imin(cl + k - so, L);
#pragma unroll
            for (int wq = 0; wq < 4; ++wq) {
                const int32_t a = imin(imax(lo - 64 * wq, 0), 64), b = imin(imax(hi - 64 * wq, 0), 64);
                const uint64_t below_b = b >= 64 ? ~0ull : (1ull << b) - 1ull, below_a = a >= 64 ? ~0ull : (1ull << a) - 1ull;
                cov[wq] |= below_b & ~below_a;
            }
            if (counting) {
                const int32_t q_end = cl + len;
                if (q_end > last_end) cnt_m += (uint32_t)((q_end - cl) - (cl < last_end ? last_end - cl : 0));
                last_end = q_end;
                if (so) counting = false;
            }
        }
        const uint32_t cnt = (uint32_t)(popc64(cov[0]) + popc64(cov[1]) + popc64(cov[2]) + popc64(cov[3]));
        const bool keep = !((double)cnt < P.cfg.min_exact_match * (double)L);
        ns[s2] = keep ? n_in : 0; nm[s2] = keep ? cnt_m : 0u;
    }
    *label_out = label;
    return have_label;
}

MGX_DEV bool lane_all_rows(const AlignParams &P, const uint32_t *p, const int32_t n, const uint32_t label) {
    const uint64_t want = ((uint64_t)label << 16) | 1u, gn = P.g.n, rows = P.anno_rows;
    const uint64_t *head = P.anno_head;
    auto row_ok = [&](const uint32_t node) -> bool { return node && node <= gn && (uint64_t)node - 1 < rows; };
    int32_t x = 0;
    for (; x < n && ((uintptr_t)(p + x) & 15u); ++x) {
        const uint32_t v = gld(p + x);
        if (!row_ok(v) || gld(head + ((uint64_t)v - 1)) != want) return false;
    }
    for (; x + 4 <= n; x += 4) {
        const LaneNodeQuad q = gld((const LaneNodeQuad *)(p + x));
        if (!row_ok(q.v[0]) || !row_ok(q.v[1]) || !row_ok(q.v[2]) || !row_ok(q.v[3])) return false;
        const uint64_t h0 = gld(head + ((uint64_t)q.v[0] - 1)), h1 = gld(head + ((uint64_t)q.v[1] - 1));
        const uint64_t h2 = gld(head + ((uint64_t)q.v[2] - 1)), h3 = gld(head + ((uint64_t)q.v[3] - 1));
        if (((h0 ^ want) | (h1 ^ want) | (h2 ^ want) | (h3 ^ want)) != 0) return false;
    }
    for (; x < n; ++x) {
        const uint32_t v = gld(p + x);
        if (!row_ok(v) || gld(head + ((uint64_t)v - 1)) != want) return false;
    }
    return true;
}

template <bool LABELED>
MGX_DEV int lane_exact_class(const LaneParams &LP, const uint64_t read, int32_t *L_out, int *strand, uint32_t hdr4[4], uint32_t *label_out) {
    const AlignParams &P = LP.P;
    const DevConfig &cfg = P.cfg;
    if (P.labeled && (!LABELED || !(P.labeled & 2u))) return LANE_EXACT_NONE;
    const bool labeled = LABELED && P.labeled != 0;
    const int32_t k = (int32_t)P.g.k;
    const int32_t L = (int32_t)(gld(P.offsets + read + 1) - gld(P.offsets + read));
    if (L > (int32_t)P.lim.Lmax || L > LANE_MAX_L || L < k) return LANE_EXACT_NONE;
    const SeedHdr *hp = P.seed_hdr + read;
    if (gld(&hp->status) != ST_OK) return LANE_EXACT_NONE;
    uint32_t nm[2] = { gld(&hp->num_matching[0]), gld(&hp->num_matching[1]) };
    int32_t ns[2] = { (int32_t)gld(&hp->n_seeds[0]), (int32_t)gld(&hp->n_seeds[1]) };
    const int32_t ns0_h = ns[0];
    const bool have_rc = cfg.fwd_and_rc != 0;
    const int32_t full = LP.self_score * L + cfg.left_end_bonus + cfg.right_end_bonus;
    uint32_t label = 0;
    if (labeled) {
        if (full < cfg.min_path_score || full < cfg.min_cell_score) return LANE_EXACT_NONE;
        bool cand = false;
        for (int s2 = 0; s2 < (have_rc ? 2 : 1); ++s2) {
            if (ns[s2] <= 0) continue;
            const DevSeed *sf = P.seed_stream + gld(&hp->off) + (s2 ? ns0_h : 0);
            cand = cand || (gld(&sf->clipping) == 0 && gld(&sf->offset) == 0 && ((int32_t)gld(&sf->length) == L || LP.exact >= 2u));
        }
        if (!cand) return LANE_EXACT_NONE;
        if (!lane_exact_label_filter(P, read, hp, L, have_rc, ns, nm, &label)) return LANE_EXACT_NONE;
    }
    const uint32_t nm0 = nm[0], nm1 = nm[1];
    const int32_t ns0 = ns[0], ns1 = ns[1];
    const int first = nm0 >= nm1 ? 0 : 1;
    const int s = have_rc ? first : 0;
    if (have_rc) {
        const uint32_t m_first = first ? nm1 : nm0, m_second = first ? nm0 : nm1;
        const int32_t n_second = first ? ns0 : ns1;
        if ((double)m_second >= (double)m_first * cfg.rel_score_cutoff && n_second > 0) return LANE_EXACT_NONE;
    }
    if ((s ? ns1 : ns0) <= 0) return LANE_EXACT_NONE;
    const DevSeed *s0 = P.seed_stream + gld(&hp->off) + (s ? ns0_h : 0);
    if (!(gld(&s0->clipping) == 0 && gld(&s0->offset) == 0)) return LANE_EXACT_NONE;
    const int32_t len = (int32_t)gld(&s0->length);
    if (len != L && LP.exact < 2u) return LANE_EXACT_NONE;
    if (full < cfg.min_path_score || full < cfg.min_cell_score) return LANE_EXACT_NONE;
    const uint32_t *rn = (s ? P.nodes_rc : P.nodes_fwd) + gld(P.node_begin + read);
    const int32_t nk = L - k + 1;
    if (len != L) {
        const int32_t next = len - k + 1;
        if (next > 0 && next < nk && !gld(rn + next)) return LANE_EXACT_NONE;
        if (!labeled && !lane_all_nodes(rn, nk)) return LANE_EXACT_NONE;
    }
    if (labeled && !lane_all_rows(P, rn, nk, label)) return LANE_EXACT_NONE;
    *L_out = L; *strand = s; *label_out = label;
    hdr4[0] = nm0; hdr4[1] = nm1; hdr4[2] = (uint32_t)ns0; hdr4[3] = (uint32_t)ns1;
    return len == L ? LANE_EXACT_SPAN : LANE_EXACT_PATH;
}

template <bool LABELED>
MGX_DEV int lane_exact_t(const LaneParams &LP, const uint64_t read, LaneResult &R) {
    int32_t L = 0;
    int s = 0;
    uint32_t h[4], label = 0;
    const int cls = lane_exact_class<LABELED>(LP, read, &L, &s, h, &label);
    if (cls == LANE_EXACT_NONE) return cls;
    const int32_t k = (int32_t)LP.P.g.k;
    ReadResult &rr = R.rr;
    rr.status = ST_OK; rr.n_alignments = 0; rr.score = 0; rr.offset = 0; rr.n_nodes = rr.n_cigar = rr.seq_len = 0;
    rr.orientation = 0; rr.stream_off = 0;
    rr.num_matches_fwd = h[0]; rr.num_matches_rc = h[1]; rr.n_seeds_fwd = h[2]; rr.n_seeds_rc = h[3];
    rr.n_extensions = 0; rr.n_columns = 0;
    R.have_aln = 1; R.mode = LANE_EMIT_EXACT; R.strand = s; R.trim = 0; R.label = label;
    R.score = LP.self_score * L + LP.P.cfg.left_end_bonus + LP.P.cfg.right_end_bonus;
    R.offset = 0; R.clip = 0; R.end_clip = 0; R.n_runs = 1; R.j_hi = 0; R.n_nodes = L - k + 1; R.n_seq = L;
    R.words = (uint32_t)R.n_nodes + 1u + ((uint32_t)L + 3) / 4 + ((LABELED && LP.P.labeled) ? 2u : 0u);
    return cls;
}
MGX_DEV int lane_exact(const LaneParams &LP, const uint64_t read, LaneResult &R) {
    return LP.P.labeled ? lane_exact_t<true>(LP, read, R) : lane_exact_t<false>(LP, read, R);
}

MGX_DEV int lane_read(const LaneParams &LP, uint64_t read, const uint32_t item, const int pass, uint8_t *scratch, const LaneChip &chip,
                      LaneCounters &ctr, LaneResult &R) {
    if (!pass && LP.exact && lane_exact(LP, read, R) != LANE_EXACT_NONE) return LR_DONE;
    return lane_read_dp(LP, read, item, pass, scratch, chip, ctr, R);
}

template <bool WITH_EXACT>
MGX_DEV void lane_emit_t(const LaneParams &LP, const uint64_t read, const uint8_t *scratch, const LaneChip &chip, LaneResult &R,
                         const uint64_t so) {
    const AlignParams &P = LP.P;
    const uint8_t *slots = scratch;
    ReadResult &rr = R.rr;
    if (R.have_aln) {
        if (so + R.words > P.out_capacity) {
            rr.status = ST_CAPACITY;
        } else {
            uint32_t *dst = P.out_stream + so;
            const int32_t n_cigar = (R.clip ? 1 : 0) + R.n_runs + (R.end_clip ? 1 : 0);
            uint8_t *dseq = (uint8_t *)(dst + R.n_nodes + n_cigar);
            const int32_t k_minus_1 = (int32_t)P.g.k - 1;
            int32_t nc = 0;
            if (R.clip) gst(dst + R.n_nodes + nc++, ((uint32_t)R.clip << 3) | OP_CLIPPED);
            if (R.mode == LANE_EMIT_SLOTS) {
                for (int32_t x = R.n_runs - 1; x >= 0; --x) gst(dst + R.n_nodes + nc++, gld(lane_run_word(slots, LP.max_cols, x)));
                int32_t j = R.j_hi, ni = R.n_nodes - 1;
                for (int32_t x = R.n_seq - 1; x >= 0; --x) {
                    const uint32_t node = gld(lane_slot_word(slots, j, 8)), geom = gld(lane_slot_word(slots, j, 10)), link = gld(lane_slot_word(slots, j, 11));
                    gst(dseq + x, decode_code((geom >> 24) & 7u));
                    if ((int32_t)(link >> 16) >= k_minus_1) { if (ni >= 0) gst(dst + ni, node); --ni; }
                    j = (int32_t)(link & 0xFFFFu);
                }
            } else if (WITH_EXACT && R.mode == LANE_EMIT_EXACT) {
                const uint64_t off = gld(P.offsets + read);
                const uint32_t *rn = (R.strand ? P.nodes_rc : P.nodes_fwd) + gld(P.node_begin + read);
                const uint64_t *pw = LP.pk[R.strand] + packed_word_begin(off, read);
                for (int32_t x = 0; x < R.n_nodes; ++x) gst(dst + x, gld(rn + x));
                gst(dst + R.n_nodes + nc++, ((uint32_t)R.n_seq << 3) | OP_MATCH);
                uint32_t *dw = dst + R.n_nodes + n_cigar;
                uint64_t qw = 0;
                for (int32_t x = 0; x < R.n_seq; x += 4) {
                    if (!(x & 31)) qw = gld(pw + (x >> 5));
                    uint32_t v = 0;
                    for (int t = 0; t < 4; ++t)
                        if (x + t < R.n_seq) v |= (uint32_t)decode_code(((uint32_t)(qw >> (2 * ((x + t) & 31))) & 3u) + 1u) << (8 * t);
                    gst(dw + (x >> 2), v);
                }
            } else if (R.mode == LANE_EMIT_ARRAYS) {
                const uint32_t *pn = (const uint32_t *)(lane_rest(LP, scratch, chip.lane) + (uint64_t)LP.hash_slots * 8) + 4 * LFW;
                const uint32_t *pc = pn + LP.max_cols, *pr = pc + LP.max_cols;
                for (int32_t x = R.n_runs - 1; x >= 0; --x) gst(dst + R.n_nodes + nc++, gld(pr + x));
                for (int32_t x = 0; x < R.n_nodes; ++x) gst(dst + x, gld(pn + x));
                for (int32_t x = 0; x < R.n_seq; ++x) gst(dseq + x, decode_code(gld(pc + x)));
            } else {
                for (int32_t x = 0; x < R.n_runs; ++x) gst(dst + R.n_nodes + nc++, gld(lane_run_word(slots, LP.max_cols, x)));
                int32_t j = R.j_hi, ni = 0;
                for (int32_t x = 0; x < R.n_seq; ++x) {
                    const uint32_t node = gld(lane_slot_word(slots, j, 8)), geom = gld(lane_slot_word(slots, j, 10)), link = gld(lane_slot_word(slots, j, 11));
                    gst(dseq + x, decode_code(5u - ((geom >> 24) & 7u)));
                    if ((int32_t)(link >> 16) >= k_minus_1) { if (ni < R.n_nodes) gst(dst + ni, node); ++ni; }
                    j = (int32_t)(link & 0xFFFFu);
                }
            }
            if (R.end_clip) gst(dst + R.n_nodes + nc++, ((uint32_t)R.end_clip << 3) | OP_CLIPPED);
            for (int32_t x = R.n_seq; x & 3; ++x) gst(dseq + x, (uint8_t)0);
            if (P.labeled) {
                uint32_t *lab = dst + R.n_nodes + n_cigar + ((uint32_t)R.n_seq + 3) / 4;
                gst(lab, 1u); gst(lab + 1, R.label);
            }
            rr.score = R.score; rr.offset = (uint32_t)R.offset;
            rr.n_nodes = (uint32_t)R.n_nodes; rr.n_cigar = (uint32_t)n_cigar; rr.seq_len = (uint32_t)R.n_seq;
            rr.orientation = (uint32_t)R.strand; rr.stream_off = so;
            rr.n_alignments = 1;
        }
    }
    {
        ReadResult *dst = P.results + read;
        gst(&dst->status, rr.status); gst(&dst->n_alignments, rr.n_alignments); gst(&dst->score, rr.score); gst(&dst->offset, rr.offset);
        gst(&dst->n_nodes, rr.n_nodes); gst(&dst->n_cigar, rr.n_cigar); gst(&dst->seq_len, rr.seq_len); gst(&dst->orientation, rr.orientation);
        gst(&dst->stream_off, rr.stream_off);
        gst(&dst->num_matches_fwd, rr.num_matches_fwd); gst(&dst->num_matches_rc, rr.num_matches_rc);
        gst(&dst->n_seeds_fwd, rr.n_seeds_fwd); gst(&dst->n_seeds_rc, rr.n_seeds_rc);
        gst(&dst->n_extensions, rr.n_extensions); gst(&dst->n_columns, rr.n_columns);
    }
    if (P.dbg_seeds) {
        const SeedHdr *hp = P.seed_hdr + read;
        const uint64_t h_off = gld(&hp->off);
        const int32_t ns0 = (int32_t)gld(&hp->n_seeds[0]), ns1 = (int32_t)gld(&hp->n_seeds[1]);
        for (int st = 0; st < 2; ++st) {
            const int32_t cnt = P.labeled ? (int32_t)(st ? rr.n_seeds_rc : rr.n_seeds_fwd) : (st ? ns1 : ns0);
            const DevSeed *src = P.seed_stream + h_off + (st ? ns0 : 0);
            for (int32_t i = 0; i < cnt; ++i) {
                DevSeed *d = P.dbg_seeds + ((uint64_t)read * 2 + st) * P.lim.max_seeds + i;
                gst(&d->clipping, gld(&src[i].clipping)); gst(&d->length, gld(&src[i].length));
                gst(&d->offset, gld(&src[i].offset)); gst(&d->n_nodes, gld(&src[i].n_nodes)); gst(&d->node, gld(&src[i].node));
            }
        }
    }
}

MGX_DEV void lane_emit(const LaneParams &LP, const uint64_t read, const uint8_t *scratch, const LaneChip &chip, LaneResult &R,
                       const uint64_t so) {
    lane_emit_t<true>(LP, read, scratch, chip, R, so);
}

}
```

### metagraph_amd/csrc/lane_types.hpp

```cpp
#pragma once
#include <algorithm>
#include <cstdlib>
#include <string>

#include "../../include/mgx.h"
#include "align_types.hpp"


namespace mgx {

#ifndef MGX_LANE_MAX_L
#define MGX_LANE_MAX_L 256
#endif
constexpr int LANE_MAX_L = MGX_LANE_MAX_L;
constexpr int LANE_MAX_L_HOST = 256;
constexpr int LANE_QWORDS = LANE_MAX_L / 32 + 2;
constexpr int LANE_MAX_RUNS = 16;
constexpr int LANE_MAX_SEEDS = 512;
constexpr int LANE_SLOT_WORDS = 12;
constexpr int LANE_WAVE = 64;
constexpr int LANE_MAX_DEFER = 3;
constexpr int LANE_DSLOT_WORDS = 80;
constexpr uint32_t LANE_GEOM_ROW = 1u << 31;
constexpr int LANE_S8_FILTER_SEEDS = 16;
constexpr int LANE_S8_WORDS = 8;

struct LaneParams {
    AlignParams P;
    const uint64_t *pk[2];
    const uint32_t *iv[2];
    uint8_t *scratch;
    uint64_t wave_stride;
    uint64_t rest_stride;
    uint32_t max_cols;
    uint32_t hash_slots;
    uint32_t tag_seed;
    uint32_t t4[4];
    int32_t self_score;
    uint32_t *bail_list;
    unsigned long long *bail_count;
    unsigned long long *done_count;
    unsigned long long *bail_hist;
    uint32_t exact;
    uint32_t done_key;
};
constexpr int LANE_HIST_EXACT = 48;
constexpr int LANE_HIST_EXACT_PATH = 49;

inline uint32_t lane_max_cols(uint32_t Lmax, int32_t xdrop) {
    return Lmax + (uint32_t)std::min<int64_t>(Lmax, std::max<int64_t>(xdrop, 0)) + 8;
}

inline uint64_t lane_rest_bytes(uint32_t max_cols, uint32_t hash_slots) {
    return (uint64_t)hash_slots * 8 + 2 * 2 * 32 * 4
           + (uint64_t)max_cols * 8 + LANE_MAX_RUNS * 4 + 32 * 4 + (uint64_t)(LANE_MAX_L_HOST + 8) * 4
           + (uint64_t)LANE_MAX_DEFER * LANE_DSLOT_WORDS * 4;
}
inline uint64_t lane_slots_bytes(uint32_t max_cols) { return (uint64_t)max_cols * LANE_SLOT_WORDS * LANE_WAVE * 4; }
inline uint64_t lane_s8_bytes(uint32_t max_cols) { return (uint64_t)max_cols * LANE_S8_WORDS * LANE_WAVE * 4; }
inline uint64_t lane_runs_bytes() { return (uint64_t)LANE_MAX_RUNS * LANE_WAVE * 4; }
inline uint64_t lane_wave_scratch_bytes(uint32_t max_cols, uint64_t rest_stride) {
    return lane_slots_bytes(max_cols) + lane_s8_bytes(max_cols) + lane_runs_bytes() + (uint64_t)LANE_WAVE * rest_stride;
}


inline bool lane_exact_config(const mgx_config &c, const DevConfig &d, uint32_t labeled_flags) {
    if ((labeled_flags & 1u) && !(labeled_flags & 2u)) return false;
    const char acgt[4] = { 'A', 'C', 'G', 'T' };
    const int m = c.score_matrix[(int)'A'][(int)'A'];
    for (int x = 0; x < 4; ++x)
        for (int y = 0; y < 4; ++y)
            if (x != y && c.score_matrix[(int)acgt[x]][(int)acgt[y]] >= m) return false;
    if (c.gap_opening_penalty >= 0) return false;
    if (c.right_end_bonus < 0 || d.right_end_bonus < 0) return false;
    if (c.xdrop < 0) return false;
    return true;
}

constexpr bool LANE_EXACT_AUTO_LABELED = true;

inline bool lane_enabled(const mgx_config &c, const DevConfig &d, uint32_t k, uint32_t Lmax, bool no_fast, LaneParams *LP, std::string *why,
                         uint32_t labeled_flags = 0) {
    auto no = [&](const char *w) { if (why) *why = w; return false; };
    if ((labeled_flags & 1u) && !(labeled_flags & 2u)) return no("label-aware: rows of dummy nodes hold labels");
    if (d.num_alt != 1 || d.post_chain) return no("alternative paths");
    if (d.canonical != 0) return no("CANONICAL / PRIMARY graph");
    if (k > 32 || k < 2) return no("k > 32: reads are not 2-bit packed");
    if (Lmax < 1 || Lmax > (uint32_t)LANE_MAX_L_HOST) return no("reads longer than a lane takes");
    if (no_fast || c.xdrop > 30000) return no("chain path off");
    if (d.branch_xdrop) return no("per-branch x-drop (global_xdrop = 0): the lane kernels encode the global rule");
    const char acgt[4] = { 'A', 'C', 'G', 'T' };
    const int m = c.score_matrix[(int)'A'][(int)'A'];
    if (m <= 0) return no("match score");
    for (int x = 0; x < 4; ++x) {
        if (c.score_matrix[(int)acgt[x]][(int)acgt[x]] != m) return no("match scores differ");
        uint32_t row = 0;
        for (int y = 0; y < 4; ++y) {
            const int v = c.score_matrix[(int)acgt[x]][(int)acgt[y]];
            if (v > m) return no("a mismatch scores above a match");
            row |= (uint32_t)(uint8_t)(int8_t)v << (8 * y);
        }
        LP->t4[x] = row;
    }
    if (c.gap_opening_penalty > 0 || c.gap_extension_penalty > 0) return no("positive gap scores");
    if (c.left_end_bonus < 0) return no("negative left end bonus");
    if (!(c.rel_score_cutoff >= 0.0 && c.rel_score_cutoff <= 1.0)) return no("rel_score_cutoff outside [0, 1]");
    LP->self_score = m;
    const char *ex = std::getenv("MGX_EMU_LANE_EXACT");
    const uint32_t level = (ex && (*ex == '1' || *ex == '2') && !ex[1]) ? (uint32_t)(*ex - '0') : 0u;
    LP->exact = (level && lane_exact_config(c, d, labeled_flags)) ? level : 0u;
    return true;
}

}
```

### metagraph_amd/csrc/mgx.hip

```cpp
#include <hip/hip_runtime.h>
#include "pack_swar.hpp"
#include <hipcub/hipcub.hpp>

#include <atomic>
#include <cstdarg>
#include <memory>

#define MGX_NO_EXTEND 1
#include "seed_kernel.hpp"
#include "host_state.hpp"
#include "lane_types.hpp"
#include "seed_lane.hpp"
#include "kernel_units.hpp"

using namespace mgx;
static_assert(sizeof(AlignParams) == MGX_ALIGN_PARAMS_BYTES && sizeof(LaneParams) == MGX_LANE_PARAMS_BYTES
              && sizeof(SeedLaneParams) == MGX_SEED_LANE_PARAMS_BYTES, "a parameter block differs from what the kernel units take");

static thread_local std::string g_err;
DevPool g_pool;

int fail(int code, const char *fmt, ...) {
    char buf[512];
    va_list ap;
    va_start(ap, fmt);
    vsnprintf(buf, sizeof(buf), fmt, ap);
    va_end(ap);
    g_err = buf;
    return code;
}
int hip_fail(hipError_t e, const char *expr, const char *file, int line) {
    return fail(e == hipErrorOutOfMemory ? MGX_ERR_OOM : MGX_ERR_NO_DEVICE, "%s: %s (%s:%d)", expr, hipGetErrorString(e), file, line);
}

__global__ void k_iota(uint32_t *v, uint64_t n) {
    uint64_t i = (uint64_t)blockIdx.x * blockDim.x + threadIdx.x;
    if (i < n) v[i] = (uint32_t)i;
}

hipError_t load_sort_kernels() {
    hipFuncAttributes attr;
    return hipFuncGetAttributes(&attr, reinterpret_cast<const void *>(&k_iota));
}

int exclusive_sum(mgx_aligner *A, uint64_t *in, uint64_t *out, uint64_t n) {
    size_t tmp_bytes = 0;
    HIP_TRY(hipcub::DeviceScan::ExclusiveSum(nullptr, tmp_bytes, in, out, (int)n, A->hstream));
    if (int rc = A->scan_tmp.ensure(tmp_bytes + 16)) return rc;
    HIP_TRY(hipcub::DeviceScan::ExclusiveSum(A->scan_tmp.p, tmp_bytes, in, out, (int)n, A->hstream));
    return MGX_OK;
}


enum LaunchCounter { CNT_NONE = -1, CNT_GRP8 = 0, CNT_GRP8_PRIM, CNT_GRP8_ALT, CNT_EXT64, CNT_LANE, CNT_N };
static std::atomic<uint64_t> g_kernel_launches[CNT_N];

struct ExtBuild {
    int (*launch_grp)(const void *params, uint32_t n_groups, uint32_t lds_bytes, int phase, void *stream);
    int (*launch_64)(const void *params, uint32_t blocks, uint32_t lds_bytes, void *stream);
    int (*waves_per_simd)(void);
    unsigned (*static_lds)(void);
    uint64_t kernel_bit;
    LaunchCounter counter;
};
enum ExtBuildId { EXT_GRP8, EXT_GRP8_PRIM, EXT_GRP8_ALT, EXT_GRP8_LAB, EXT_EXT64, EXT_LAB64, EXT_GRP8_LAB_BX, EXT_LAB64_BX };
static const ExtBuild g_ext_builds[] = {
    { mgx_launch_align_grp8, nullptr, mgx_grp_waves_per_simd8, mgx_grp_static_lds8, MGX_KERNEL_GRP8, CNT_GRP8 },
    { mgx_launch_align_grp8_prim, nullptr, mgx_grp_waves_per_simd8_prim, mgx_grp_static_lds8_prim, MGX_KERNEL_GRP8_PRIM, CNT_GRP8_PRIM },
    { mgx_launch_align_grp8_alt, nullptr, mgx_grp_waves_per_simd8_alt, mgx_grp_static_lds8_alt, MGX_KERNEL_GRP8_ALT, CNT_GRP8_ALT },
    { mgx_launch_align_grp8_lab, nullptr, mgx_grp_waves_per_simd8_lab, mgx_grp_static_lds8_lab, MGX_KERNEL_GRP8_LAB, CNT_NONE },
    { nullptr, mgx_launch_ext64, mgx_ext64_waves_per_simd, mgx_ext64_static_lds, MGX_KERNEL_EXT64, CNT_EXT64 },
    { nullptr, mgx_launch_lab64, mgx_lab64_waves_per_simd, mgx_lab64_static_lds, MGX_KERNEL_LAB64, CNT_NONE },
    { mgx_launch_align_grp8_labx, nullptr, mgx_grp_waves_per_simd8_labx, mgx_grp_static_lds8_labx, MGX_KERNEL_GRP8_LAB_BX, CNT_NONE },
    { nullptr, mgx_launch_lab64x, mgx_lab64x_waves_per_simd, mgx_lab64x_static_lds, MGX_KERNEL_LAB64_BX, CNT_NONE },
};
static uint32_t waves_per_cu(const ExtBuild &b) { return 4u * (uint32_t)b.waves_per_simd(); }
static const ExtBuild &group_build(bool labeled, bool primary, uint64_t agg_cap, bool branch_xdrop) {
    return g_ext_builds[labeled ? (branch_xdrop ? EXT_GRP8_LAB_BX : EXT_GRP8_LAB) : agg_cap > 1 ? EXT_GRP8_ALT : primary ? EXT_GRP8_PRIM : EXT_GRP8];
}

static uint32_t lds_budget(uint32_t waves_cu, uint32_t static_lds, uint32_t margin) { return (160u * 1024u) / waves_cu - static_lds - margin; }
static uint32_t lds_per_read(uint32_t Lmax, uint32_t waves_cu, uint32_t static_lds, uint32_t margin, uint32_t reads_per_wave = 1) {
    return std::min<uint32_t>(fast_lds_bytes(Lmax), lds_budget(waves_cu, static_lds, margin) / reads_per_wave) & ~15u;
}


extern "C" {

int mgx_device_count(void) {
    int n = 0;
    if (hipGetDeviceCount(&n) != hipSuccess) return 0;
    return n;
}
const char *mgx_last_error(void) { return g_err.c_str(); }
void mgx_set_last_error(const char *msg) { g_err = msg ? msg : ""; }
uint32_t mgx_abi_version(void) { return MGX_ABI_VERSION; }

void mgx_config_init_default(mgx_config *c) {
    memset(c, 0, sizeof(*c));
    c->num_alternative_paths = 1;
    c->max_num_seeds_per_locus = UINT64_MAX;
    c->min_cell_score = INT32_MIN + 100;
    c->min_path_score = 0;
    c->xdrop = INT32_MAX;
    c->max_nodes_per_seq_char = 1.7976931348623157e308;
    c->max_ram_per_alignment = 1.7976931348623157e308;
    c->gap_opening_penalty = -5;
    c->gap_extension_penalty = -2;
    c->forward_and_reverse_complement = 1;
    c->global_xdrop = 1;
    c->allow_left_trim = 1;
    c->seed_complexity_filter = 1;
}

void mgx_config_set_dna_matrix(mgx_config *c, int8_t match, int8_t mm_transition, int8_t mm_transversion) {
    for (int i = 0; i < 128; ++i)
        for (int j = 0; j < 128; ++j) c->score_matrix[i][j] = mm_transversion;
    c->score_matrix['A']['G'] = c->score_matrix['G']['A'] = mm_transition;
    c->score_matrix['C']['T'] = c->score_matrix['T']['C'] = mm_transition;
    c->score_matrix['A']['A'] = c->score_matrix['C']['C'] = c->score_matrix['G']['G'] = c->score_matrix['T']['T'] = match;
}

void mgx_config_set_unit_matrix(mgx_config *c, int8_t match) {
    for (int i = 0; i < 128; ++i)
        for (int j = 0; j < 128; ++j) c->score_matrix[i][j] = (int8_t)-match;
    c->score_matrix['A']['A'] = c->score_matrix['C']['C'] = c->score_matrix['G']['G'] = c->score_matrix['T']['T'] = match;
}

void mgx_config_set_scoring_matrix(mgx_config *c) {
    if (c->alignment_edit_distance) {
        mgx_config_set_unit_matrix(c, 1);
        c->left_end_bonus = 0;
        c->right_end_bonus = 0;
    } else {
        mgx_config_set_dna_matrix(c, c->alignment_match_score, (int8_t)-c->alignment_mm_transition_score,
                                  (int8_t)-c->alignment_mm_transversion_score);
    }
}

void mgx_config_init_cli(mgx_config *c, uint32_t k) {
    mgx_config_init_default(c);
    c->min_seed_length = std::min<uint64_t>(19, k);
    c->max_seed_length = UINT64_MAX;
    c->max_num_seeds_per_locus = 1000;
    c->xdrop = 27;
    c->min_exact_match = 0.7;
    c->max_nodes_per_seq_char = 5.0;
    c->max_ram_per_alignment = 200.0;
    c->rel_score_cutoff = 0.95;
    c->gap_opening_penalty = -6;
    c->gap_extension_penalty = -2;
    c->left_end_bonus = 5;
    c->right_end_bonus = 5;
    c->alignment_edit_distance = 0;
    c->alignment_match_score = 2;
    c->alignment_mm_transition_score = 3;
    c->alignment_mm_transversion_score = 3;
    mgx_config_set_scoring_matrix(c);
}

void mgx_limits_init_default(mgx_limits *l, uint32_t max_query_length) {
    memset(l, 0, sizeof(*l));
    l->max_query_length = max_query_length;
}

}

static int aligner_create_for(const mgx_graph *g, const mgx_config *config, const mgx_limits *limits, const mgx_annotation *anno, bool chainer,
                              mgx_aligner **out) {
    if (!g || !config || !out) return fail(MGX_ERR_INVALID, "null argument");
    auto *A = new mgx_aligner();
    std::unique_ptr<mgx_aligner> guard(A);
    A->chainer = chainer;
    A->graph = g;
    A->anno = anno;
    A->device = g->device;
    for (DevBuf *b : { &A->mlen_fwd, &A->mlen_rc, &A->pk_fwd, &A->pk_rc, &A->iv_fwd, &A->iv_rc, &A->rng_fwd, &A->rng_rc, &A->score_matrix,
                       &A->seqs, &A->offsets, &A->counts, &A->node_begin, &A->nodes_fwd, &A->nodes_rc, &A->arena, &A->results, &A->stream,
                       &A->cursors, &A->d_stats, &A->d_stats_map, &A->scan_tmp, &A->dbg_seeds, &A->seed_hdr, &A->seed_stream, &A->work_key,
                       &A->work_key_sorted, &A->order_in, &A->order, &A->sort_tmp, &A->retry_list, &A->resume_pool[0], &A->resume_pool[1],
                       &A->retry_list2, &A->retry_key[0], &A->retry_key[1], &A->lane_scratch, &A->lane_params, &A->lane_bail, &A->lane_hist, &A->seedlane_scratch, &A->seedlane_params,
                       &A->seedlane_bail, &A->seedlane_hist, &A->ms_counts, &A->ms_nodes, &A->ms_sorted, &A->mf_threshold, &A->tf_headers, &A->tf_header_offsets,
                       &A->tf_names, &A->tf_len, &A->tf_begin, &A->tf_text, &A->tf_cap, &A->tf_patch, &A->rd_counts, &A->rd_begins, &A->rd_totals, &A->rd_alns,
                       &A->rd_nodes, &A->rd_cigar, &A->rd_seqs, &A->rd_status, &A->rd_labels,
                       &A->ct.counts, &A->ct.begins, &A->ct.pair_key, &A->ct.pair_key_alt, &A->ct.pair_val, &A->ct.pair_val_alt, &A->ct.kept, &A->ct.n_kept,
                       &A->ct.seeds, &A->ct.nodes, &A->ct.num_matching, &A->ct.status, &A->ct.qsize, &A->ct.penalty, &A->ct.anchors, &A->ct.anchors_alt,
                       &A->ct.backtrace, &A->ct.perm, &A->ct.perm_alt, &A->ct.k32, &A->ct.k32_alt, &A->ct.k64, &A->ct.k64_alt, &A->ct.sort_tmp, &A->ct.sort_tmp_anchors })
        b->pooled = true;
    {
        std::string err;
        int rc = prepare_config(*config, g->g.k, &A->cfg, &A->dcfg, &err, anno != nullptr);
        if (rc) return fail(rc, "%s", err.c_str());
    }
    if (anno) {
        const int lab_max_alt = std::min(std::min(mgx_lab64_max_alt(), mgx_grp_max_alt8_lab()), std::min(mgx_lab64x_max_alt(), mgx_grp_max_alt8_labx()));
        if (A->cfg.num_alternative_paths > (uint64_t)lab_max_alt)
            return fail(MGX_ERR_UNSUPPORTED, "label-aware alignment: num_alternative_paths <= %d on the device", lab_max_alt);
        int adev = 0; uint64_t arows = 0; const uint64_t *h; const uint32_t *c, *m;
        mgx_annotation_device_view(anno, &adev, &arows, &h, &c, &m);
        if (adev != g->device) return fail(MGX_ERR_INVALID, "the annotation lives on device %d, the graph on device %d", adev, g->device);
        if (!chainer && mgx_annotation_has_coordinates(anno) && g->mode == MGX_MODE_BASIC)
            return fail(MGX_ERR_UNSUPPORTED, "label-aware alignment with coordinates (seed chaining) is not on the device");
        if (arows < g->g.n) return fail(MGX_ERR_INVALID, "the annotation has %llu rows, the graph %llu nodes (row = node - 1)",
                                        (unsigned long long)arows, (unsigned long long)g->g.n);
    }
    if (g->mode == MGX_MODE_CANONICAL) { A->dcfg.canonical = 1; A->dcfg.fwd_and_rc = 1; }
    if (g->mode == MGX_MODE_PRIMARY) { A->dcfg.canonical = g->primary_tables ? 3 : 2; A->dcfg.fwd_and_rc = 1; }
    mgx_config &c = A->cfg;
    if (limits) { A->user_lim = *limits; A->have_user_lim = true; }
    HIP_TRY(hipSetDevice(g->device));
    if (anno) {
        if (int rc = graph_dummy_rows_clean(g, anno, &A->anno_dummy_clean)) return rc;
        if (g->mode == MGX_MODE_CANONICAL) if (int rc = graph_canon_repr(g)) return rc;
    }
    if (int rc = A->score_matrix.ensure(128 * 128)) return rc;
    HIP_TRY(hipMemcpy(A->score_matrix.p, c.score_matrix, 128 * 128, hipMemcpyHostToDevice));
    if (int rc = A->cursors.ensure(CUR_WORDS * 8)) return rc;
    if (int rc = A->d_stats.ensure(sizeof(KernelStats))) return rc;
    if (int rc = A->d_stats_map.ensure(sizeof(KernelStats))) return rc;
    for (auto &e : A->ev) HIP_TRY(hipEventCreate(&e));
    memset(&A->hstats, 0, sizeof(A->hstats));
    memset(&A->lim, 0, sizeof(A->lim));
    *out = guard.release();
    return MGX_OK;
}

int aligner_create(const mgx_graph *g, const mgx_config *config, const mgx_limits *limits, const mgx_annotation *anno, mgx_aligner **out) {
    return aligner_create_for(g, config, limits, anno, false, out);
}
int refuse_chainer(const mgx_aligner *A, const char *call) {
    return A && A->chainer ? fail(MGX_ERR_UNSUPPORTED, "%s: a seed-chainer handle runs mgx_chain_tables_batch / mgx_chain_tables_fetch only", call) : MGX_OK;
}

extern "C" {

int mgx_aligner_create(const mgx_graph *g, const mgx_config *config, const mgx_limits *limits, mgx_aligner **out) {
    return aligner_create(g, config, limits, nullptr, out);
}
int mgx_seed_chainer_create(const mgx_graph *g, const mgx_config *config, const mgx_limits *limits, const mgx_annotation *annotation,
                            mgx_aligner **out) {
    if (!g || !config || !annotation || !out) return fail(MGX_ERR_INVALID, "null argument");
    if (g->mode != MGX_MODE_BASIC)
        return fail(MGX_ERR_UNSUPPORTED, "mgx_seed_chainer_create: graph mode %u (the reference has k-mer coordinates on BASIC graphs only)", g->mode);
    if (!mgx_annotation_has_coordinates(annotation))
        return fail(MGX_ERR_UNSUPPORTED, "mgx_seed_chainer_create: the annotation has no k-mer coordinates (LabeledAligner chains seeds only with them)");
    if (!config->forward_and_reverse_complement)
        return fail(MGX_ERR_UNSUPPORTED, "mgx_seed_chainer_create: forward_and_reverse_complement = 0 (the reference chains only where it seeds both strands)");
    if (config->chain_alignments)
        return fail(MGX_ERR_UNSUPPORTED, "mgx_seed_chainer_create: chain_alignments is set by LabeledAligner itself, never by the caller");
    mgx_config c = *config;
    c.global_xdrop = 0;
    if (int rc = aligner_create_for(g, &c, limits, annotation, true, out)) return rc;
    (*out)->cfg.chain_alignments = 1;
    return MGX_OK;
}
int mgx_labeled_aligner_create(const mgx_graph *g, const mgx_config *config, const mgx_limits *limits, const mgx_annotation *annotation,
                               mgx_aligner **out) {
    if (!annotation) return fail(MGX_ERR_INVALID, "null argument");
    return aligner_create(g, config, limits, annotation, out);
}

void mgx_aligner_destroy(mgx_aligner *a) {
    if (!a) return;
    (void)hipSetDevice(a->device);
    (void)hipStreamSynchronize(a->hstream);
    for (auto &e : a->ev) if (e) (void)hipEventDestroy(e);
    if (a->h_text) (void)hipHostFree(a->h_text);
    for (void *p : a->h_rd) if (p) (void)hipHostFree(p);
    if (a->own_stream) (void)hipStreamDestroy(a->hstream);
    delete a;
}

int mgx_aligner_get_config(const mgx_aligner *a, mgx_config *out) { *out = a->cfg; return MGX_OK; }

int mgx_aligner_get_limits(const mgx_aligner *a, mgx_limits *out) {
    if (!a || !out) return fail(MGX_ERR_INVALID, "null argument");
    memset(out, 0, sizeof(*out));
    out->max_query_length = a->lim.Lmax;
    out->max_columns = a->lim.max_columns;
    out->max_seeds = a->lim.max_seeds;
    out->cell_arena_bytes = (uint64_t)a->lim.cell_words * 4;
    return MGX_OK;
}

}

static int work_key_bits(uint64_t n) {
    int b = 12;
    for (uint64_t seg = n ? (n - 1) >> WORK_SEGMENT_SHIFT : 0; seg; seg >>= 1) ++b;
    return std::min(b, 32);
}

struct AlignPlan {
    uint64_t n = 0;
    bool labeled = false;
    uint32_t cus = 0;
    bool lane_ok = false;
    uint32_t lane_blocks = 0;
    uint64_t n_exact = 0;
    int key_bits = 0;
    LaneParams LP;
    uint64_t agg_cap = 1;
    const ExtBuild *grp = nullptr;
    uint64_t wave_slots = 0;
    uint64_t stride = 0, slots = 0;
    size_t sort_tmp_bytes = 0;
    AlignParams P;
};

static int plan_lane(mgx_aligner *A, AlignPlan &pl) {
    const DevLimits &l = A->lim;
    LaneParams &LP = pl.LP;
    memset(&LP, 0, sizeof(LP));
    std::string lane_why;
    pl.lane_blocks = pl.cus * 4u * (uint32_t)mgx_lane_waves_per_simd();
    pl.lane_ok = A->opt.lane != 0 && A->packed_valid && A->opt.multi_pass != 1
                 && lane_enabled(A->cfg, A->dcfg, A->graph->g.k, l.Lmax, A->no_fast, &LP, &lane_why,
                                 pl.labeled ? (1u | (A->anno_dummy_clean ? 2u : 0u)) : 0u)
                 && (A->opt.lane == 1 || pl.n >= (uint64_t)pl.lane_blocks * 16);
    const uint32_t lflags = pl.labeled ? (1u | (A->anno_dummy_clean ? 2u : 0u)) : 0u;
    const bool exact_auto = pl.n >= (uint64_t)pl.lane_blocks * 16 && (!pl.labeled || LANE_EXACT_AUTO_LABELED);
    LP.exact = (pl.lane_ok && A->opt.exact != 0 && lane_exact_config(A->cfg, A->dcfg, lflags)
                && (A->opt.exact >= 1 || exact_auto)) ? (A->opt.exact >= 1 ? (uint32_t)A->opt.exact : 2u) : 0u;
    pl.key_bits = work_key_bits(pl.n) + (LP.exact ? 1 : 0);
    LP.done_key = LP.exact ? 1u << work_key_bits(pl.n) : 0u;
    if (!pl.lane_ok) return MGX_OK;
    LP.max_cols = lane_max_cols(l.Lmax, A->dcfg.xdrop);
    LP.hash_slots = next_pow2(2ull * LP.max_cols);
    if (int hm; env_int("MGX_LANE_HASH_MULT", &hm)) LP.hash_slots *= (uint32_t)std::max(1, hm);
    LP.rest_stride = (lane_rest_bytes(LP.max_cols, LP.hash_slots) + 63) & ~63ull;
    LP.wave_stride = lane_wave_scratch_bytes(LP.max_cols, LP.rest_stride);
    const size_t before = A->lane_scratch.bytes;
    if (A->lane_scratch.ensure((size_t)pl.lane_blocks * LP.wave_stride, true) != MGX_OK) pl.lane_ok = false;
    else if (A->lane_scratch.bytes != before) HIP_TRY(hipMemsetAsync(A->lane_scratch.p, 0, A->lane_scratch.bytes, A->hstream));
    return MGX_OK;
}

static int size_arena(mgx_aligner *A, AlignPlan &pl) {
    const DevLimits &l = A->lim;
    const uint64_t n = pl.n, stride = arena_bytes(l);
    pl.stride = stride;
    size_t free_b = 0, total_b = 0;
    HIP_TRY(hipMemGetInfo(&free_b, &total_b));
    pl.wave_slots = (uint64_t)pl.cus * 4 * MGX_ALIGN_WAVES_PER_SIMD;
    pl.agg_cap = std::max<uint64_t>(1, A->cfg.post_chain_alignments ? (uint64_t)post_chain_capacity(A->cfg.num_alternative_paths) : A->cfg.num_alternative_paths);
    pl.grp = &group_build(pl.labeled, A->dcfg.canonical >= 2, pl.agg_cap, A->dcfg.branch_xdrop != 0);
    const uint64_t want_slots = std::max<uint64_t>(pl.wave_slots, (uint64_t)pl.cus * waves_per_cu(*pl.grp) * 8);
    const uint64_t later = n * (sizeof(ReadResult) + sizeof(SeedHdr) + 24 + 16)
                           + (n * (((uint64_t)l.Lmax + l.Lmax / 4 + 40) * pl.agg_cap) + 1024) * 4
                           + (n * 24 + A->total_kmers / 8 + 4096) * A->seed_scale * sizeof(DevSeed) + (1ull << 30);
    const uint64_t held = A->results.bytes + A->stream.bytes + A->seed_stream.bytes + A->seed_hdr.bytes;
    const uint64_t need_later = later > held ? later - held : 0;
    const uint64_t avail = (uint64_t)free_b + A->arena.bytes + g_pool.held_bytes();
    uint64_t budget = avail > need_later ? (avail - need_later) / 10 * 9 : avail / 2;
    const uint64_t share = (uint64_t)std::max(1, A->opt.device_share);
    budget /= share;
    uint64_t slots = std::min<uint64_t>(std::min<uint64_t>((want_slots + share - 1) / share, std::max<uint64_t>(n, 1)), std::max<uint64_t>(1, budget / stride));
    if (slots == 0) slots = 1;
    const size_t before = A->arena.bytes;
    if (int rc = A->arena.ensure(slots * stride, true)) return rc;
    if (A->arena.bytes != before || A->arena_stride != stride) {
        HIP_TRY(hipMemsetAsync(A->arena.p, 0, A->arena.bytes, A->hstream));
        A->arena_stride = stride;
    }
    pl.slots = slots;
    A->n_slots = (uint32_t)slots;
    if (probe_env_set("MGX_DEBUG_SLOTS")) fprintf(stderr, "run_align: n %llu stride %llu want_slots %llu slots %llu free %.1f GB\n", (unsigned long long)n, (unsigned long long)stride, (unsigned long long)want_slots, (unsigned long long)slots, free_b / 1e9);
    return MGX_OK;
}

static int size_buffers(mgx_aligner *A, AlignPlan &pl) {
    const DevLimits &l = A->lim;
    const uint64_t n = pl.n;
    if (int rc = A->results.ensure(n * sizeof(ReadResult))) return rc;
    uint64_t words_per_read = ((uint64_t)l.Lmax + l.Lmax / 4 + 40) * pl.agg_cap;
    if (pl.labeled) words_per_read = words_per_read * 2 + 16;
    A->out_words = std::max<uint64_t>(n * words_per_read + 1024, A->out_min_words);
    if (int rc = A->stream.ensure(A->out_words * 4)) return rc;
    if (A->keep_seeds) {
        if (int rc = A->dbg_seeds.ensure(n * 2 * (uint64_t)l.max_seeds * sizeof(DevSeed))) return rc;
        HIP_TRY(hipMemsetAsync(A->dbg_seeds.p, 0, n * 2 * (uint64_t)l.max_seeds * sizeof(DevSeed), A->hstream));
    }
    HIP_TRY(clear_cursors(A, CUR_OUT, CUR_RETRY));
    HIP_TRY(hipMemsetAsync(A->d_stats.p, 0, sizeof(KernelStats), A->hstream));
    A->seed_cap = std::min<uint64_t>(n * 2 * (uint64_t)l.max_seeds, (n * 24 + A->total_kmers / 8 + 4096) * A->seed_scale);
    if (int rc = A->seed_hdr.ensure(n * sizeof(SeedHdr))) return rc;
    if (int rc = A->seed_stream.ensure(A->seed_cap * sizeof(DevSeed))) return rc;
    if (int rc = A->work_key.ensure(n * 4)) return rc;
    if (int rc = A->work_key_sorted.ensure(n * 4)) return rc;
    if (int rc = A->order_in.ensure(n * 4)) return rc;
    if (int rc = A->order.ensure(n * 4)) return rc;
    if (int rc = A->retry_list.ensure(n * 4 + 4)) return rc;
    HIP_TRY(hipcub::DeviceRadixSort::SortPairs(nullptr, pl.sort_tmp_bytes, A->work_key.as<uint32_t>(), A->work_key_sorted.as<uint32_t>(),
                                               A->order_in.as<uint32_t>(), A->order.as<uint32_t>(), (int)n, 0, pl.key_bits, A->hstream));
    return A->sort_tmp.ensure(pl.sort_tmp_bytes);
}

static void fill_params(mgx_aligner *A, AlignPlan &pl, const char *d_seqs, const uint64_t *d_offsets) {
    AlignParams &P = pl.P;
    memset(&P, 0, sizeof(P));
    P.g = A->graph->g;
    P.cfg = A->dcfg;
    P.lim = A->lim;
    P.score_matrix = A->score_matrix.as<int8_t>();
    P.seqs = d_seqs;
    P.offsets = d_offsets;
    P.node_begin = A->node_begin.as<uint64_t>();
    P.nodes_fwd = A->nodes_fwd.as<uint32_t>();
    P.nodes_rc = A->nodes_rc.as<uint32_t>();
    P.mlen_fwd = A->mlen_fwd.as<uint8_t>();
    P.mlen_rc = A->mlen_rc.as<uint8_t>();
    P.rng_fwd = A->have_rng ? A->rng_fwd.as<uint2>() : nullptr;
    P.rng_rc = A->have_rng ? A->rng_rc.as<uint2>() : nullptr;
    P.n_reads = pl.n;
    P.arena = A->arena.as<uint8_t>();
    P.arena_stride = pl.stride;
    P.results = A->results.as<ReadResult>();
    P.out_stream = A->stream.as<uint32_t>();
    P.out_capacity = A->out_words;
    P.out_cursor = cursor(A, CUR_OUT);
    P.read_cursor = cursor(A, CUR_READ);
    P.stats = A->d_stats.as<KernelStats>();
    P.dbg_seeds = A->keep_seeds ? A->dbg_seeds.as<DevSeed>() : nullptr;
    P.no_fast = A->no_fast;
    if (A->packed_valid) {
        P.pkw[0] = A->pk_fwd.as<uint64_t>(); P.ivw[0] = A->iv_fwd.as<uint32_t>();
        P.pkw[1] = A->dcfg.fwd_and_rc ? A->pk_rc.as<uint64_t>() : nullptr; P.ivw[1] = A->dcfg.fwd_and_rc ? A->iv_rc.as<uint32_t>() : nullptr;
    }
    P.no_compact = A->opt.no_compact != 0;
    P.no_alias = A->opt.no_alias != 0;
    P.no_bt_runs = A->opt.no_bt_runs != 0;
    P.no_flat = A->opt.no_flat != 0 || A->cfg.post_chain_alignments;
    if (pl.labeled) {
        int adev = 0;
        mgx_annotation_device_view(A->anno, &adev, &P.anno_rows, &P.anno_head, &P.anno_count, &P.anno_more);
        P.labeled = 1u | (A->anno_dummy_clean ? 2u : 0u);
        P.anno_base = A->graph->mode == MGX_MODE_CANONICAL ? A->graph->canon_repr.as<uint32_t>() : nullptr;
        P.no_alias = 1;
    }
    P.ablate = probe_env_u32("MGX_ABLATE", 0u);
    P.seed_hdr = A->seed_hdr.as<SeedHdr>();
    P.seed_stream = A->seed_stream.as<DevSeed>();
    P.seed_capacity = A->seed_cap;
    P.seed_cursor = cursor(A, CUR_SEED);
    P.work_key = A->work_key.as<uint32_t>();
}

static int seed_by_lanes(mgx_aligner *A, AlignPlan &pl) {
    const DevLimits &l = A->lim;
    AlignParams &P = pl.P;
    const uint64_t n = pl.n;
    const bool seed_lane = A->opt.seed_lane != 0 && A->packed_valid && P.pkw[0] && P.ivw[0]
                           && (!A->dcfg.fwd_and_rc || (P.pkw[1] && P.ivw[1])) && P.mlen_fwd && P.rng_fwd
                           && (!A->dcfg.fwd_and_rc || (P.mlen_rc && P.rng_rc))
                           && seed_lane_enabled(A->dcfg, (uint32_t)A->graph->g.k, l.Lmax, true, true)
                           && (A->opt.seed_lane == 1 || n >= 4096);
    if (!seed_lane || !n) return MGX_OK;
    const bool long_reads = l.Lmax > (uint32_t)SL_SHORT_L;
    const uint32_t resident = pl.cus * 4 * (uint32_t)mgx_seed_lane_waves_per_simd();
    const uint32_t blocks1 = (uint32_t)std::min<uint64_t>(resident, (n + 63) / 64);
    const uint32_t blocks2 = (uint32_t)std::max<uint64_t>(1, std::min<uint64_t>(resident / (long_reads ? 2 : 1), (n / 4 + 63) / 64));
    const bool many = (uint64_t)A->graph->g.k >= A->dcfg.max_seed_length;
    const uint32_t me1 = many ? (long_reads ? SL_SEEDS_1_MANY_LONG : SL_SEEDS_1_MANY) : SL_SEEDS_1, mp1 = many ? SL_PENDING_1_MANY : SL_PENDING_1;
    const uint32_t me2 = long_reads ? SL_SEEDS_2_LONG : SL_SEEDS_2, mp2 = long_reads ? SL_PENDING_2_LONG : SL_PENDING_2;
    const uint64_t words1 = seed_lane_wave_scratch_words(me1, mp1), words2 = seed_lane_wave_scratch_words(me2, mp2);
    if (int rc = A->seedlane_scratch.ensure((size_t)std::max<uint64_t>(blocks1 * words1, blocks2 * words2) * 4)) return rc;
    if (int rc = A->seedlane_params.ensure(2 * sizeof(SeedLaneParams))) return rc;
    if (int rc = A->seedlane_bail.ensure(2 * (n * 4 + 4))) return rc;
    if (int rc = A->seedlane_hist.ensure(32 * 8)) return rc;
    HIP_TRY(hipMemsetAsync(A->seedlane_hist.p, 0, 32 * 8, A->hstream));
    HIP_TRY(clear_cursors(A, CUR_SL_BAIL, CUR_SL_BAIL_BACK));
    SeedLaneParams SP[2];
    memset(SP, 0, sizeof(SP));
    uint32_t *list1 = A->seedlane_bail.as<uint32_t>(), *list2 = list1 + n + 1;
    for (int ps = 0; ps < 2; ++ps) {
        SP[ps].P = P;
        SP[ps].P.n_items = n;
        SP[ps].scratch = A->seedlane_scratch.as<uint32_t>();
        SP[ps].long_reads = long_reads ? 1u : 0u;
        SP[ps].second_pass = (uint32_t)ps;
        SP[ps].list_len = n;
        SP[ps].done_count = cursor(A, CUR_SL_DONE);
    }
    SP[0].max_entries = me1; SP[0].max_pending = mp1;
    SP[0].bail_list = list1; SP[0].bail_count = cursor(A, CUR_SL_BAIL); SP[0].bail_count_back = cursor(A, CUR_SL_BAIL_BACK);
    SP[1].max_entries = me2; SP[1].max_pending = mp2;
    SP[1].in_list = list1; SP[1].in_count = cursor(A, CUR_SL_BAIL); SP[1].in_count_back = cursor(A, CUR_SL_BAIL_BACK);
    SP[1].bail_list = list2; SP[1].bail_count = cursor(A, CUR_SL_BAIL2);
    SP[1].bail_hist = A->seedlane_hist.as<unsigned long long>();
    HIP_TRY(copy_sync(A, A->seedlane_params.p, SP, sizeof(SP), hipMemcpyHostToDevice));
    if (int rc = mgx_launch_seed_lane(A->seedlane_params.p, blocks1, long_reads, A->hstream)) return fail(MGX_ERR_NO_DEVICE, "lane-per-read seeder: %d", rc);
    HIP_TRY(clear_cursors(A, CUR_READ, CUR_READ));
    if (int rc = mgx_launch_seed_lane(A->seedlane_params.as<SeedLaneParams>() + 1, blocks2, long_reads, A->hstream)) return fail(MGX_ERR_NO_DEVICE, "lane-per-read seeder, second pass: %d", rc);
    HIP_TRY(clear_cursors(A, CUR_READ, CUR_READ));
    P.seed_list = list2;
    P.n_items_ptr = cursor(A, CUR_SL_BAIL2);
    A->seedlane_launched = 1;
    return MGX_OK;
}

static int seed_by_waves(mgx_aligner *A, AlignPlan &pl) {
    const DevLimits &l = A->lim;
    AlignParams &P = pl.P;
    const bool primary = A->dcfg.canonical >= 2;
    const auto launch = primary ? mgx_launch_seed_primary : mgx_launch_seed;
    const uint32_t static_lds = mgx_seed_static_lds();
    uint32_t blocks, lds;
    const bool wps8 = A->opt.seed_wps == 8 && l.Lmax <= 192 && pl.slots >= (uint64_t)pl.cus * 4 * 8;
    if (wps8) {
        uint32_t lds8 = lds_per_read(l.Lmax, 4 * MGX_SEED_WPS, static_lds, 192u);
        lds8 = std::min<uint32_t>(lds8, probe_env_u32("MGX_SEED_LDS_CAP", lds8)) & ~15u;
        if (probe_env_set("MGX_SEED_LDS_PRINT")) fprintf(stderr, "k_seed: static_lds %u budget8 %u lds8 %u (fast_lds_bytes %u)\n", static_lds, lds_budget(4 * MGX_SEED_WPS, static_lds, 192u), lds8, fast_lds_bytes(l.Lmax));
        const uint32_t spct = probe_env_pct("MGX_SEED_WAVES_PCT");
        blocks = primary ? pl.cus * 4 * MGX_SEED_WPS : std::max(1u, pl.cus * 4 * MGX_SEED_WPS * spct / 100);
        lds = lds8;
    } else {
        blocks = (uint32_t)std::min<uint64_t>(pl.slots, pl.wave_slots);
        lds = lds_per_read(l.Lmax, 4 * MGX_ALIGN_WAVES_PER_SIMD, static_lds, 64u);
    }
    if (int rc = launch(&P, blocks, lds, wps8 ? 1 : 0, A->hstream))
        return primary ? fail(MGX_ERR_NO_DEVICE, "seeding kernel (PRIMARY): %d", rc) : hip_fail((hipError_t)rc, "hipGetLastError()", __FILE__, __LINE__);
    P.seed_list = nullptr; P.n_items_ptr = nullptr;
    return MGX_OK;
}

static int sort_by_work(mgx_aligner *A, AlignPlan &pl) {
    const uint64_t n = pl.n;
    k_iota<<<(uint32_t)((n + 255) / 256), 256, 0, A->hstream>>>(A->order_in.as<uint32_t>(), n);
    HIP_TRY(hipcub::DeviceRadixSort::SortPairs(A->sort_tmp.p, pl.sort_tmp_bytes, A->work_key.as<uint32_t>(), A->work_key_sorted.as<uint32_t>(),
                                               A->order_in.as<uint32_t>(), A->order.as<uint32_t>(), (int)n, 0, pl.key_bits, A->hstream));
    HIP_TRY(clear_cursors(A, CUR_READ, CUR_READ));
    pl.P.order = A->order.as<uint32_t>();
    return MGX_OK;
}

static int choose_multi_pass(mgx_aligner *A, const AlignPlan &pl, bool *multi) {
    *multi = false;
    if (pl.labeled || A->cfg.post_chain_alignments) return MGX_OK;
    *multi = A->opt.multi_pass == 1;
    if (A->opt.multi_pass < 0) {
        unsigned long long seeds_total = 0;
        HIP_TRY(copy_sync(A, &seeds_total, cursor(A, CUR_SEED), 8, hipMemcpyDeviceToHost));
        *multi = pl.n > 0 && seeds_total / pl.n >= 24;
    }
    return MGX_OK;
}

static int prepare_lane(mgx_aligner *A, AlignPlan &pl) {
    LaneParams &LP = pl.LP;
    if (int rc = A->lane_bail.ensure(pl.n * 4 + 4)) return rc;
    if (int rc = A->lane_params.ensure(sizeof(LaneParams))) return rc;
    if (int rc = A->lane_hist.ensure(64 * 8)) return rc;
    HIP_TRY(hipMemsetAsync(A->lane_hist.p, 0, 64 * 8, A->hstream));
    HIP_TRY(clear_cursors(A, CUR_LANE_BAIL, CUR_LANE_DONE));
    LP.pk[0] = A->pk_fwd.as<uint64_t>(); LP.pk[1] = A->pk_rc.as<uint64_t>();
    LP.iv[0] = A->iv_fwd.as<uint32_t>(); LP.iv[1] = A->iv_rc.as<uint32_t>();
    LP.scratch = A->lane_scratch.as<uint8_t>();
    LP.bail_list = A->lane_bail.as<uint32_t>();
    LP.bail_count = cursor(A, CUR_LANE_BAIL);
    LP.done_count = cursor(A, CUR_LANE_DONE);
    LP.bail_hist = A->lane_hist.as<unsigned long long>();
    return MGX_OK;
}

static int exact_by_lanes(mgx_aligner *A, AlignPlan &pl) {
    LaneParams &LP = pl.LP;
    LP.P = pl.P;
    LP.P.n_items = pl.n;
    HIP_TRY(copy_sync(A, A->lane_params.p, &LP, sizeof(LP), hipMemcpyHostToDevice));
    const uint32_t blocks = (uint32_t)std::min<uint64_t>((uint64_t)pl.cus * 4 * 8 * 4, (pl.n + 63) / 64);
    if (int rc = mgx_launch_lane_exact(A->lane_params.p, blocks, pl.labeled ? 1 : 0, A->hstream)) return fail(MGX_ERR_NO_DEVICE, "lane kernel, exact exit: %d", rc);
    unsigned long long done = 0;
    HIP_TRY(copy_sync(A, &done, cursor(A, CUR_LANE_DONE), 8, hipMemcpyDeviceToHost));
    pl.n_exact = done;
    unsigned long long path = 0;
    if (LP.exact >= 2u && done)
        HIP_TRY(copy_sync(A, &path, A->lane_hist.as<unsigned long long>() + LANE_HIST_EXACT_PATH, 8, hipMemcpyDeviceToHost));
    A->lane_exact = done - path;
    A->lane_exact_path = path;
    return MGX_OK;
}

static int extend_by_lanes(mgx_aligner *A, AlignPlan &pl, bool *all_done) {
    AlignParams &P = pl.P;
    LaneParams &LP = pl.LP;
    const uint64_t n = pl.n - pl.n_exact;
    if (n == 0) {
        A->lane_done = pl.n_exact;
        A->kernels_ran |= MGX_KERNEL_LANE;
        HIP_TRY(hipEventRecord(A->ev[EV_LANE_END], A->hstream));
        *all_done = true;
        return MGX_OK;
    }
    LP.P = P;
    LP.P.n_items = n;
    LP.tag_seed = ++A->lane_epoch * 0x632BE5ABu;
    HIP_TRY(copy_sync(A, A->lane_params.p, &LP, sizeof(LP), hipMemcpyHostToDevice));
    uint32_t blocks = (uint32_t)std::min<uint64_t>(pl.lane_blocks, (n + 63) / 64);
    if (int pct; env_int("MGX_LANE_BLOCKS_PCT", &pct)) blocks = std::max<uint32_t>(1u, (uint32_t)((uint64_t)blocks * (uint64_t)pct / 100));
    if (int rc = mgx_launch_lane(A->lane_params.p, blocks, A->hstream)) return fail(MGX_ERR_NO_DEVICE, "lane kernel: %d", rc);
    A->kernels_ran |= MGX_KERNEL_LANE;
    ++g_kernel_launches[CNT_LANE];
    HIP_TRY(hipEventRecord(A->ev[EV_LANE_END], A->hstream));
    unsigned long long counts[2] = { 0, 0 };
    HIP_TRY(copy_sync(A, counts, cursor(A, CUR_LANE_BAIL), 16, hipMemcpyDeviceToHost));
    A->lane_done = counts[1];
    HIP_TRY(copy_sync(A, A->lane_hist_h, A->lane_hist.p, 32 * 8, hipMemcpyDeviceToHost));
    if (int on; env_int("MGX_LANE_TIMERS", &on)) {
        unsigned long long t[16];
        HIP_TRY(copy_sync(A, t, A->lane_hist.as<unsigned long long>() + 32, sizeof(t), hipMemcpyDeviceToHost));
        fprintf(stderr, "k_lane timers (cycles of lane 0, summed over %u wavefronts): setup %llu children %llu column %llu node-table %llu commit %llu frontier %llu trace %llu result %llu | emit %llu kernel %llu\n",
                blocks, t[0], t[1], t[2], t[7], t[3], t[4], t[5], t[6], t[8], t[9]);
    }
    HIP_TRY(clear_cursors(A, CUR_READ, CUR_READ));
    P.order = A->lane_bail.as<uint32_t>();
    P.n_items = counts[0];
    *all_done = counts[0] == 0;
    return MGX_OK;
}

static int launch_extension(mgx_aligner *A, AlignPlan &pl) {
    const uint32_t Lmax = A->lim.Lmax;
    const int gpw_opt = A->opt.groups_per_wave;
    const uint64_t items = pl.P.n_items ? pl.P.n_items : pl.n;
    const ExtBuild *b = pl.grp;
    uint32_t gpw, count, lds;
    if (pl.labeled) {
        const ExtBuild &lab64 = g_ext_builds[A->dcfg.branch_xdrop ? EXT_LAB64_BX : EXT_LAB64];
        const uint64_t resident64 = (uint64_t)pl.cus * waves_per_cu(lab64);
        if ((items <= resident64 && A->opt.ext64 != 0) || A->opt.ext64 == 2) {
            b = &lab64; gpw = 1;
            count = (uint32_t)std::max<uint64_t>(1, std::min<uint64_t>(pl.slots, resident64));
        } else {
            gpw = gpw_opt > 0 ? (uint32_t)std::min(8, gpw_opt) : 0u;
            count = (uint32_t)pl.slots;
        }
    } else {
        const uint32_t pct = probe_env_pct("MGX_EXT_GROUPS_PCT");
        count = (uint32_t)std::min<uint64_t>(pl.slots, std::max<uint64_t>(1, pl.slots * pct / 100));
        const uint64_t resident_waves = (uint64_t)pl.cus * waves_per_cu(*pl.grp);
        const uint64_t busy = std::min<uint64_t>(count, std::max<uint64_t>(1, items));
        const uint64_t want_gpw = std::min<uint64_t>(8, std::max<uint64_t>(1, (busy + resident_waves - 1) / resident_waves));
        gpw = gpw_opt >= 0 ? (uint32_t)std::min(8, gpw_opt) : (want_gpw < 8 ? (uint32_t)want_gpw : 0u);
        if (A->opt.ext64 != 0 && gpw == 1) b = &g_ext_builds[EXT_EXT64];
    }
    if (b->launch_64) {
        lds = lds_per_read(Lmax, waves_per_cu(*b), b->static_lds(), 128u);
    } else {
        lds = lds_per_read(Lmax, waves_per_cu(*b), b->static_lds(), 64u, 8);
        if (!pl.labeled) lds = std::min<uint32_t>(lds, probe_env_u32("MGX_EXT_LDS_CAP", lds)) & ~15u;
    }
    pl.P.groups_per_wave = gpw;
    A->kernels_ran |= b->kernel_bit;
    if (b->counter != CNT_NONE) ++g_kernel_launches[b->counter];
    return b->launch_64 ? b->launch_64(&pl.P, count, lds, A->hstream) : b->launch_grp(&pl.P, count, lds, PH_EXTEND, A->hstream);
}

static int extend_multi_pass(mgx_aligner *A, AlignPlan &pl) {
    AlignParams &P = pl.P;
    const uint64_t n = pl.n;
    const uint32_t rb = resume_rec_bytes(A->lim, (uint32_t)std::max<uint64_t>(1, A->cfg.num_alternative_paths));
    size_t fb = 0, tb = 0;
    HIP_TRY(hipMemGetInfo(&fb, &tb));
    fb += g_pool.held_bytes();
    const uint64_t have = A->resume_pool[0].bytes + A->resume_pool[1].bytes;
    uint64_t cap = std::min<uint64_t>(n, ((uint64_t)fb / 2 + have) / (2ull * rb));
    if (cap > 0xFFFFFFF0ull) cap = 0xFFFFFFF0ull;
    if (A->opt.resume_cap >= 0) cap = std::min<uint64_t>(cap, (uint64_t)A->opt.resume_cap);
    if (cap == 0) {
        HIP_TRY((hipError_t)launch_extension(A, pl));
        return MGX_OK;
    }
    for (int b = 0; b < 2; ++b) {
        if (int rc = A->resume_pool[b].ensure(cap * rb, true)) return rc;
        if (int rc = A->retry_key[b].ensure(n * 4 + 4)) return rc;
    }
    if (int rc = A->retry_list2.ensure(n * 4 + 4)) return rc;
    DevBuf *lists[2] = { &A->retry_list, &A->retry_list2 };
    P.resume_rec_bytes = rb; P.resume_cap = (uint32_t)cap;
    P.retry_count = cursor(A, CUR_RETRY);
    P.resume_in = nullptr; P.resume_reads = nullptr;
    int out = 0;
    for (uint32_t pass = 0;; ++pass) {
        P.resume_out = A->resume_pool[out].as<uint8_t>();
        P.retry_list = lists[out]->as<uint32_t>();
        P.retry_key = A->retry_key[out].as<uint32_t>();
        P.seed_limit = multi_pass_seed_limit(pass);
        HIP_TRY((hipError_t)launch_extension(A, pl));
        unsigned long long c = 0;
        HIP_TRY(copy_sync(A, &c, cursor(A, CUR_RETRY), 8, hipMemcpyDeviceToHost));
        c = std::min<unsigned long long>(c, cap);
        A->n_passes = pass + 1;
        if (c == 0 || P.seed_limit == 0) break;
        k_iota<<<(uint32_t)((c + 255) / 256), 256, 0, A->hstream>>>(A->order_in.as<uint32_t>(), c);
        size_t tmp_bytes = pl.sort_tmp_bytes;
        HIP_TRY(hipcub::DeviceRadixSort::SortPairs(A->sort_tmp.p, tmp_bytes, A->retry_key[out].as<uint32_t>(), A->work_key_sorted.as<uint32_t>(),
                                                   A->order_in.as<uint32_t>(), A->order.as<uint32_t>(), (int)c, 0, 12, A->hstream));
        HIP_TRY(clear_cursors(A, CUR_READ, CUR_READ));
        HIP_TRY(clear_cursors(A, CUR_RETRY, CUR_RETRY));
        P.order = A->order.as<uint32_t>();
        P.n_items = c;
        P.resume_in = A->resume_pool[out].as<uint8_t>();
        P.resume_reads = lists[out]->as<uint32_t>();
        out ^= 1;
    }
    return MGX_OK;
}

static int seed_stage(mgx_aligner *A, const char *d_seqs, const uint64_t *d_offsets, uint64_t n, uint32_t Lmax, bool lane, AlignPlan &pl) {
    {
        std::string err;
        int rc = derive_limits(A->cfg, A->have_user_lim ? &A->user_lim : nullptr, Lmax, &A->lim, &err, A->anno != nullptr, A->label_scale);
        if (rc) return fail(rc, "%s", err.c_str());
    }
    hipDeviceProp_t prop;
    HIP_TRY(hipGetDeviceProperties(&prop, A->graph->device));
    pl.n = n;
    pl.labeled = A->anno != nullptr;
    pl.cus = (uint32_t)prop.multiProcessorCount;
    if (lane) {
        if (int rc = plan_lane(A, pl)) return rc;
    } else {
        memset(&pl.LP, 0, sizeof(pl.LP));
        pl.key_bits = work_key_bits(n);
    }
    if (int rc = size_arena(A, pl)) return rc;
    if (int rc = size_buffers(A, pl)) return rc;
    fill_params(A, pl, d_seqs, d_offsets);
    HIP_TRY(hipEventRecord(A->ev[EV_ALIGN_BEGIN], A->hstream));
    A->kernels_ran = 0;
    A->seedlane_launched = 0;
    if (int rc = seed_by_lanes(A, pl)) return rc;
    HIP_TRY(hipEventRecord(A->ev[EV_SEED_LANE_END], A->hstream));
    if (int rc = seed_by_waves(A, pl)) return rc;
    HIP_TRY(hipEventRecord(A->ev[EV_SEEDED], A->hstream));
    return MGX_OK;
}

static int run_align(mgx_aligner *A, const char *d_seqs, const uint64_t *d_offsets, uint64_t n, uint32_t Lmax) {
    AlignPlan pl;
    if (int rc = seed_stage(A, d_seqs, d_offsets, n, Lmax, true, pl)) return rc;
    A->n_passes = 1;
    A->lane_done = 0;
    A->lane_exact = 0;
    A->lane_exact_path = 0;
    memset(A->lane_hist_h, 0, sizeof(A->lane_hist_h));
    bool multi = false;
    const bool exact = pl.lane_ok && pl.LP.exact && n;
    if (exact) { if (int rc = choose_multi_pass(A, pl, &multi)) return rc; }
    const bool by_lanes = pl.lane_ok && !multi && n;
    if (by_lanes) { if (int rc = prepare_lane(A, pl)) return rc; }
    if (by_lanes && exact) { if (int rc = exact_by_lanes(A, pl)) return rc; }
    if (int rc = sort_by_work(A, pl)) return rc;
    HIP_TRY(hipEventRecord(A->ev[EV_SORTED], A->hstream));
    if (!exact) { if (int rc = choose_multi_pass(A, pl, &multi)) return rc; }
    HIP_TRY(hipEventRecord(A->ev[EV_LANE_END], A->hstream));
    bool all_done = false;
    if (pl.lane_ok && !multi && n) {
        if (int rc = extend_by_lanes(A, pl, &all_done)) return rc;
    }
    if (multi) {
        if (int rc = extend_multi_pass(A, pl)) return rc;
    } else if (!all_done) {
        HIP_TRY((hipError_t)launch_extension(A, pl));
    }
    HIP_TRY(hipEventRecord(A->ev[EV_ALIGN_END], A->hstream));
    return MGX_OK;
}

int run_seeding(mgx_aligner *A, const char *d_seqs, const uint64_t *d_offsets, uint64_t n, uint32_t Lmax, uint64_t *seeds_wanted) {
    AlignPlan pl;
    if (int rc = seed_stage(A, d_seqs, d_offsets, n, Lmax, false, pl)) return rc;
    for (AlignEvent e : { EV_SORTED, EV_LANE_END, EV_ALIGN_END }) HIP_TRY(hipEventRecord(A->ev[e], A->hstream));
    A->n_passes = 0;
    A->lane_done = A->lane_exact = A->lane_exact_path = 0;
    memset(A->lane_hist_h, 0, sizeof(A->lane_hist_h));
    unsigned long long wanted = 0;
    HIP_TRY(copy_sync(A, &wanted, cursor(A, CUR_SEED), 8, hipMemcpyDeviceToHost));
    *seeds_wanted = wanted;
    return MGX_OK;
}

int collect_stats(mgx_aligner *A, bool mapped, bool aligned) {
    HIP_TRY(hipStreamSynchronize(A->hstream));
    KernelStats ks, km;
    HIP_TRY(copy_sync(A, &ks, A->d_stats.p, sizeof(ks), hipMemcpyDeviceToHost));
    HIP_TRY(copy_sync(A, &km, A->d_stats_map.p, sizeof(km), hipMemcpyDeviceToHost));
    ks.rank_lines += km.rank_lines; ks.select_lines += km.select_lines; ks.bit_lines += km.bit_lines; ks.map_lines += km.map_lines;
    mgx_stats &s = A->hstats;
    memset(&s, 0, sizeof(s));
    s.n_reads = A->n_reads;
    s.n_rank_lines = ks.rank_lines; s.n_select_lines = ks.select_lines; s.n_bit_lines = ks.bit_lines;
    s.n_columns = ks.columns; s.n_extensions = ks.extensions; s.n_seeds = ks.seeds;
    s.n_map_lines = ks.map_lines; s.n_capacity_errors = ks.capacity_errors; s.n_seed_lines = ks.seed_lines;
    s.n_fast_columns = ks.fast_columns;
    s.extend_kernels = A->kernels_ran;
    s.n_lane_reads = A->lane_done;
    s.n_lane_exact_reads = A->lane_exact;
    s.n_lane_exact_path_reads = A->lane_exact_path;
    s.n_lane_lines = ks.lane_lines; s.n_lane_columns = ks.lane_columns;
    for (int x = 0; x < 32; ++x) s.lane_bail_reads[x] = A->lane_hist_h[x];
    if (int on; aligned && A->seedlane_launched && env_int("MGX_SL_TIMERS", &on)) {
        unsigned long long t[8];
        HIP_TRY(copy_sync(A, t, A->seedlane_hist.as<unsigned long long>() + 16, sizeof(t), hipMemcpyDeviceToHost));
        fprintf(stderr, "k_seed_lane timers (cycles of lane 0, summed over the wavefronts): strands %llu masks %llu scan %llu walks %llu dust %llu ranges+enumerate %llu publish %llu wave-mates %llu\n",
                t[0], t[1], t[2], t[3], t[4], t[5], t[6], t[7]);
    }
    if (aligned && A->seedlane_launched) {
        unsigned long long done = 0, why[16];
        HIP_TRY(copy_sync(A, &done, cursor(A, CUR_SL_DONE), 8, hipMemcpyDeviceToHost));
        HIP_TRY(copy_sync(A, why, A->seedlane_hist.p, sizeof(why), hipMemcpyDeviceToHost));
        s.n_seed_lane_reads = done;
        for (int x = 0; x < 16; ++x) s.seed_lane_left_reads[x] = why[x];
    }
    for (int x = 0; x < 8; ++x) { s.phase_cycles[x] = ks.cyc[x]; s.extend_cycles[x] = ks.xcyc[x]; }
    float ms = 0;
    if (mapped) { HIP_TRY(hipEventElapsedTime(&ms, A->ev[EV_MAP_BEGIN], A->ev[EV_MAP_END])); s.seed_kernel_ms = ms; }
    if (aligned) {
        HIP_TRY(hipEventElapsedTime(&ms, A->ev[EV_ALIGN_BEGIN], A->ev[EV_ALIGN_END])); s.align_kernel_ms = ms;
        HIP_TRY(hipEventElapsedTime(&ms, A->ev[EV_ALIGN_BEGIN], A->ev[EV_SEEDED])); s.seeding_ms = ms;
        HIP_TRY(hipEventElapsedTime(&ms, A->ev[EV_SEEDED], A->ev[EV_SORTED])); s.sort_ms = ms;
        HIP_TRY(hipEventElapsedTime(&ms, A->ev[EV_SORTED], A->ev[EV_ALIGN_END])); s.extend_ms = ms;
        HIP_TRY(hipEventElapsedTime(&ms, A->ev[EV_SORTED], A->ev[EV_LANE_END])); s.lane_ms = ms;
        if (A->seedlane_launched) { HIP_TRY(hipEventElapsedTime(&ms, A->ev[EV_ALIGN_BEGIN], A->ev[EV_SEED_LANE_END])); s.seed_lane_ms = ms; }
    }
    return MGX_OK;
}

extern "C" {

int mgx_device_trim(int device) {
    int cur = 0;
    HIP_TRY(hipGetDevice(&cur));
    HIP_TRY(hipSetDevice(device));
    g_pool.flush();
    HIP_TRY(hipSetDevice(cur));
    return MGX_OK;
}

int mgx_aligner_set_stream(mgx_aligner *A, void *hip_stream) {
    if (!A) return fail(MGX_ERR_INVALID, "null argument");
    HIP_TRY(hipSetDevice(A->graph->device));
    HIP_TRY(hipStreamSynchronize(A->hstream));
    if (A->own_stream) { (void)hipStreamDestroy(A->hstream); A->own_stream = false; }
    A->hstream = (hipStream_t)hip_stream;
    return MGX_OK;
}
int mgx_aligner_create_stream(mgx_aligner *A) {
    if (!A) return fail(MGX_ERR_INVALID, "null argument");
    HIP_TRY(hipSetDevice(A->graph->device));
    hipStream_t st = nullptr;
    HIP_TRY(hipStreamCreateWithFlags(&st, hipStreamNonBlocking));
    if (int rc = mgx_aligner_set_stream(A, st)) { (void)hipStreamDestroy(st); return rc; }
    A->own_stream = true;
    return MGX_OK;
}
void *mgx_aligner_get_stream(const mgx_aligner *A) { return A ? (void *)A->hstream : nullptr; }

int mgx_aligner_set_pipeline(mgx_aligner *A, const char *name) {
    if (!A) return fail(MGX_ERR_INVALID, "null argument");
    if (!name) return fail(MGX_ERR_INVALID, "unknown pipeline '(null)'");
    if (!strcmp(name, "general")) { A->no_fast = true; return MGX_OK; }
    if (!strcmp(name, "chain")) { A->no_fast = false; return MGX_OK; }
    if (strchr(name, '=')) {
        const std::string key(name, strchr(name, '=') - name);
        const int v = atoi(strchr(name, '=') + 1);
        mgx_aligner::Options &o = A->opt;
        if (key == "ext64") o.ext64 = v;
        else if (key == "groups_per_wave") o.groups_per_wave = std::min(8, v);
        else if (key == "multi_pass") o.multi_pass = v;
        else if (key == "resume_cap") o.resume_cap = std::max(-1, v);
        else if (key == "no_compact") o.no_compact = v;
        else if (key == "decode_on_device") o.decode_on_device = v != 0;
        else if (key == "no_alias") o.no_alias = v;
        else if (key == "no_bt_runs") o.no_bt_runs = v;
        else if (key == "no_flat") o.no_flat = v;
        else if (key == "lane") o.lane = v;
        else if (key == "exact") {
            if (v < -1 || v > 2) return fail(MGX_ERR_INVALID, "unknown option '%s'", name);
            o.exact = v;
        }
        else if (key == "device_share") o.device_share = std::max(1, std::min(v, 64));
        else if (key == "map_pipe") o.map_pipe = v;
        else if (key == "seed_wps") o.seed_wps = v;
        else if (key == "seed_lane") {
            if (v < -1 || v > 1) return fail(MGX_ERR_INVALID, "unknown option '%s'", name);
            o.seed_lane = v;
        }
        else if (key == "retry_capacity") A->retry_capacity = v != 0;
        else return fail(MGX_ERR_INVALID, "unknown option '%s'", name);
        return MGX_OK;
    }
    if (strcmp(name, "split8")) return fail(MGX_ERR_INVALID, "unknown pipeline '%s'", name);
    return MGX_OK;
}


int mgx_align_batch_device(mgx_aligner *A, const char *seqs, const uint64_t *offsets, uint64_t n, int on_device) {
    if (!A || !seqs || !offsets) return fail(MGX_ERR_INVALID, "null argument");
    if (int rc = refuse_chainer(A, "mgx_align_batch_device")) return rc;
    if (mgx_device_count() <= A->graph->device) return fail(MGX_ERR_NO_DEVICE, "no HIP device");
    HIP_TRY(hipSetDevice(A->graph->device));
    const char *d_seqs; const uint64_t *d_offsets; uint32_t Lmax;
    if (n == 0) { A->n_reads = 0; A->aligned_empty = true; return MGX_OK; }
    A->aligned_empty = false;
    { HostStageTimer t("stage_batch"); if (int rc = stage_batch(A, seqs, offsets, n, on_device, &d_seqs, &d_offsets, &Lmax)) return rc; }
    A->last_d_seqs = d_seqs; A->last_d_offsets = d_offsets; A->aligned_generation = A->stage_generation;
    bool mapped = A->cfg.max_seed_length >= A->graph->g.k;
    { HostStageTimer t("run_map"); if (int rc = run_map(A, d_seqs, d_offsets, n, A->dcfg.fwd_and_rc != 0, mapped, Lmax)) return rc; }
    for (;;) {
        { HostStageTimer t("run_align"); if (int rc = run_align(A, d_seqs, d_offsets, n, Lmax)) return rc; }
        { HostStageTimer t("collect_stats"); if (int rc = collect_stats(A, mapped, true)) return rc; }
        unsigned long long out_wanted = 0, seeds_wanted = 0;
        HIP_TRY(copy_sync(A, &out_wanted, cursor(A, CUR_OUT), 8, hipMemcpyDeviceToHost));
        bool again = false;
        if (out_wanted > A->out_words) { A->out_min_words = out_wanted + out_wanted / 8 + 1024; again = true; }
        HIP_TRY(copy_sync(A, &seeds_wanted, cursor(A, CUR_SEED), 8, hipMemcpyDeviceToHost));
        if (seeds_wanted > A->seed_cap) {
            A->seed_scale = seeds_wanted / std::max<uint64_t>(1, A->seed_cap / A->seed_scale) + 2;
            again = true;
        }
        if (!again) break;
    }
    A->h_results.clear();
    return MGX_OK;
}


int mgx_aligner_stats(const mgx_aligner *A, mgx_stats *out) { *out = A->hstats; return MGX_OK; }
void mgx_kernel_launch_counts(uint64_t *out5) { for (int x = 0; x < 5; ++x) out5[x] = g_kernel_launches[x].load(); }

}
```

### metagraph_amd/csrc/mgx_lane.hip

```cpp
#include <hip/hip_runtime.h>

#define mgx mgx_lane_ns
#include "wave.hpp"
#include "graph_build.hpp"
#include "lane_read.hpp"
#include "kernel_units.hpp"

using namespace mgx;

#ifndef MGX_LANE_WAVES_PER_SIMD
#define MGX_LANE_WAVES_PER_SIMD 2
#endif

__global__ void __launch_bounds__(64, MGX_LANE_WAVES_PER_SIMD) k_lane(const LaneParams *__restrict__ LPp) {
    const LaneParams &LP = *LPp;
    __shared__ uint64_t s_qw[LANE_QWORDS][64];
    __shared__ uint32_t s_cold[LANE_COLD_WORDS][64];
    const int lane = (int)threadIdx.x;
    uint8_t *scratch = LP.scratch + (uint64_t)blockIdx.x * LP.wave_stride + 4u * (uint32_t)lane;
    LaneChip chip;
    chip.lane = lane;
    chip.qw = &s_qw[0][lane]; chip.qstride = 64;
    chip.cold = &s_cold[0][lane]; chip.cstride = 64;
    const uint64_t n_items = LP.P.n_items ? LP.P.n_items : LP.P.n_reads;
    LaneCounters ctr;
    memset(&ctr, 0, sizeof(ctr));
#if MGX_LANE_TIMERS
    const uint64_t t_kernel = cycle_clock();
    uint64_t t_emit = 0;
#endif
    {
        uint32_t *rec = lane_record(LP, scratch, lane);
        for (int x = 26; x < 32; ++x) gst(rec + x, 0u);
    }
    uint64_t read = 0, item = 0;
    int pass = 0;
    bool holding = false;
    for (;;) {
        LV<bool> wantv;
        wantv.v = !holding;
        const uint64_t wm = wave_ballot(wantv);
        LV<uint64_t> bv;
        bv.v = 0;
        if (lane == 0 && wm) bv.v = atomicAdd(LP.P.read_cursor, (unsigned long long)popc64(wm));
        const uint64_t base = wave_bcast(bv, 0);
        if (!holding) {
            item = base + (uint64_t)popc64(wm & ((1ull << lane) - 1));
            pass = 0;
            if (item < n_items) { holding = true; read = LP.P.order ? (uint64_t)gld(LP.P.order + item) : item; }
        }
        LV<bool> actv;
        actv.v = holding;
        if (!wave_ballot(actv)) break;
        const bool active = holding;
        int rc = LR_DONE;
        LaneResult R;
        R.words = 0; R.have_aln = 0;
        if (active) rc = lane_read_dp(LP, read, (uint32_t)item, pass, scratch, chip, ctr, R);
        if (active && rc == LR_AGAIN) pass = 1; else holding = false;
        const bool done = active && rc == LR_DONE, bail = active && rc == LR_BAIL;
        LV<int32_t> wv;
        wv.v = done ? (int32_t)R.words : 0;
        const LV<int32_t> pre = wave_prefix_sum_excl(wv);
        const int32_t total = wave_sum(wv);
        LV<uint64_t> sv;
        sv.v = 0;
        if (lane == 0 && total) sv.v = atomicAdd(LP.P.out_cursor, (unsigned long long)total);
        const uint64_t so = wave_bcast(sv, 0) + (uint64_t)pre.v;
#if MGX_LANE_TIMERS
        const uint64_t te0 = cycle_clock();
#endif
        if (done) {
            lane_emit_t<false>(LP, read, scratch, chip, R, so);
            uint32_t *rec = lane_record(LP, scratch, lane);
            gst(rec + 29, gld(rec + 29) + 1u); gst(rec + 30, gld(rec + 30) + R.rr.n_extensions);
            gst(rec + 31, gld(rec + 31) + (uint32_t)(R.rr.status != ST_OK));
        }
#if MGX_LANE_TIMERS
        t_emit += cycle_clock() - te0;
#endif
        LV<bool> bl;
        bl.v = bail;
        const uint64_t bm = wave_ballot(bl);
        if (bm) {
            LV<uint64_t> pv;
            pv.v = 0;
            if (lane == 0) pv.v = atomicAdd(LP.bail_count, (unsigned long long)popc64(bm));
            const uint64_t p0 = wave_bcast(pv, 0);
            if (bail) gst(LP.bail_list + p0 + (uint64_t)popc64(bm & ((1ull << lane) - 1)), (uint32_t)read);
            uint64_t left = bm;
            while (left) {
                LV<uint32_t> rv;
                rv.v = ctr.reason;
                const uint32_t code = wave_bcast(rv, ctz64(left)) & 31u;
                LV<bool> same;
                same.v = bail && (ctr.reason & 31u) == code;
                const uint64_t sm = wave_ballot(same);
                if (lane == 0) atomicAdd(LP.bail_hist + code, (unsigned long long)popc64(sm));
                left &= ~sm;
            }
        }
    }
    const uint32_t *rec = lane_record(LP, scratch, lane);
    LV<int32_t> v;
    v.v = (int32_t)gld(rec + 27); const int32_t rl = wave_sum(v);
    v.v = (int32_t)gld(rec + 28); const int32_t sl = wave_sum(v);
    v.v = (int32_t)gld(rec + 26); const int32_t cl = wave_sum(v);
    v.v = (int32_t)gld(rec + 29); const int32_t nd = wave_sum(v);
    v.v = (int32_t)gld(rec + 30); const int32_t ne = wave_sum(v);
    v.v = (int32_t)gld(rec + 31); const int32_t nc = wave_sum(v);
#if MGX_LANE_TIMERS
    if (lane == 0) {
        for (int x = 0; x < 8; ++x) atomicAdd(LP.bail_hist + 32 + x, (unsigned long long)ctr.t[x]);
        atomicAdd(LP.bail_hist + 40, (unsigned long long)t_emit);
        atomicAdd(LP.bail_hist + 41, (unsigned long long)(cycle_clock() - t_kernel));
    }
#endif
    if (lane == 0) {
        atomicAdd(&LP.P.stats->rank_lines, (unsigned long long)rl);
        atomicAdd(&LP.P.stats->select_lines, (unsigned long long)sl);
        atomicAdd(&LP.P.stats->columns, (unsigned long long)cl);
        atomicAdd(&LP.P.stats->fast_columns, (unsigned long long)cl);
        atomicAdd(&LP.P.stats->lane_lines, (unsigned long long)rl + (unsigned long long)sl);
        atomicAdd(&LP.P.stats->lane_columns, (unsigned long long)cl);
        atomicAdd(&LP.P.stats->extensions, (unsigned long long)ne);
        atomicAdd(&LP.P.stats->capacity_errors, (unsigned long long)nc);
        atomicAdd(LP.done_count, (unsigned long long)nd);
    }
}

template <bool LABELED>
__device__ __forceinline__ void lane_exact_body(const LaneParams &LP) {
    const int lane = (int)threadIdx.x;
    const uint64_t n_reads = LP.P.n_reads;
    LaneChip chip;
    chip.lane = lane; chip.qw = nullptr; chip.qstride = 0; chip.cold = nullptr; chip.cstride = 0;
    uint32_t n_done = 0, n_path = 0, n_cap = 0;
    for (uint64_t base = (uint64_t)blockIdx.x * 64; base < n_reads; base += (uint64_t)gridDim.x * 64) {
        const uint64_t read = base + (uint64_t)lane;
        LaneResult R;
        R.words = 0;
        LV<bool> hv;
        const int cls = read < n_reads ? lane_exact_t<LABELED>(LP, read, R) : LANE_EXACT_NONE;
        hv.v = cls != LANE_EXACT_NONE;
        if (!wave_ballot(hv)) continue;
        LV<int32_t> wv;
        wv.v = hv.v ? (int32_t)R.words : 0;
        const LV<int32_t> pre = wave_prefix_sum_excl(wv);
        const int32_t total = wave_sum(wv);
        LV<uint64_t> sv;
        sv.v = 0;
        if (lane == 0) sv.v = atomicAdd(LP.P.out_cursor, (unsigned long long)total);
        const uint64_t so = wave_bcast(sv, 0) + (uint64_t)pre.v;
        if (hv.v) {
            lane_emit_t<true>(LP, read, nullptr, chip, R, so);
            gst(LP.P.work_key + read, LP.done_key);
            ++n_done; n_path += (uint32_t)(cls == LANE_EXACT_PATH); n_cap += (uint32_t)(R.rr.status != ST_OK);
        }
    }
    LV<int32_t> v;
    v.v = (int32_t)n_done; const int32_t nd = wave_sum(v);
    v.v = (int32_t)n_cap; const int32_t nc = wave_sum(v);
    v.v = (int32_t)n_path; const int32_t np = wave_sum(v);
    if (lane == 0 && nd) {
        atomicAdd(LP.done_count, (unsigned long long)nd);
        atomicAdd(LP.bail_hist + LANE_HIST_EXACT, (unsigned long long)nd);
        if (np) atomicAdd(LP.bail_hist + LANE_HIST_EXACT_PATH, (unsigned long long)np);
        if (nc) atomicAdd(&LP.P.stats->capacity_errors, (unsigned long long)nc);
    }
}

__global__ void __launch_bounds__(64) k_lane_exact(const LaneParams *__restrict__ LPp) { lane_exact_body<false>(*LPp); }
__global__ void __launch_bounds__(64) k_lane_exact_labeled(const LaneParams *__restrict__ LPp) { lane_exact_body<true>(*LPp); }

extern "C" int mgx_launch_lane(const void *d_params, uint32_t blocks, void *stream) {
    static_assert(sizeof(LaneParams) == MGX_LANE_PARAMS_BYTES, "LaneParams differs from what mgx.hip passes");
    k_lane<<<blocks, 64, 0, (hipStream_t)stream>>>(static_cast<const LaneParams *>(d_params));
    return (int)hipGetLastError();
}
extern "C" int mgx_launch_lane_exact(const void *d_params, uint32_t blocks, int labeled, void *stream) {
    if (labeled) k_lane_exact_labeled<<<blocks, 64, 0, (hipStream_t)stream>>>(static_cast<const LaneParams *>(d_params));
    else k_lane_exact<<<blocks, 64, 0, (hipStream_t)stream>>>(static_cast<const LaneParams *>(d_params));
    return (int)hipGetLastError();
}
extern "C" int mgx_lane_waves_per_simd(void) { return MGX_LANE_WAVES_PER_SIMD; }
```

Baseline: 15.22 million reads/s.

## Add exact fast path for reads with a single substitution via graph walk

Adds an exact-mode level where reads with exactly one contiguous run of missing k-mers are treated as single-substitution candidates. The first pass gathers them into a list. A second kernel walks the graph across the mismatch, checks seed consistency and score cutoffs, and emits a match/mismatch/match alignment directly, so these reads skip the DP lane kernel. This adds an extra kernel launch and more classification work, and the checks have to reproduce what DP would output.

Result: faster. 16.64 million reads/s (median of 6 runs) (+9.3%).

```diff
diff --git a/include/mgx.h b/include/mgx.h
--- a/include/mgx.h
+++ b/include/mgx.h
@@ -157,6 +157,7 @@
     uint64_t seed_lane_left_reads[16];
     uint64_t n_lane_exact_reads;
     uint64_t n_lane_exact_path_reads;
+    uint64_t n_lane_exact_sub_reads;
 } mgx_stats;
 enum { MGX_KERNEL_GRP8 = 1, MGX_KERNEL_GRP8_PRIM = 2, MGX_KERNEL_GRP8_ALT = 4, MGX_KERNEL_EXT64 = 8, MGX_KERNEL_LANE = 16,
        MGX_KERNEL_LAB64 = 32, MGX_KERNEL_GRP8_LAB = 64,
diff --git a/metagraph_amd/capi.py b/metagraph_amd/capi.py
--- a/metagraph_amd/capi.py
+++ b/metagraph_amd/capi.py
@@ -122,7 +122,8 @@
                 ("lane_ms", C.c_double), ("n_lane_lines", C.c_uint64), ("n_lane_columns", C.c_uint64),
                 ("lane_bail_reads", C.c_uint64 * 32), ("n_capacity_retried", C.c_uint64),
                 ("n_seed_lane_reads", C.c_uint64), ("seed_lane_ms", C.c_double), ("seed_lane_left_reads", C.c_uint64 * 16),
-                ("n_lane_exact_reads", C.c_uint64), ("n_lane_exact_path_reads", C.c_uint64)]
+                ("n_lane_exact_reads", C.c_uint64), ("n_lane_exact_path_reads", C.c_uint64),
+                ("n_lane_exact_sub_reads", C.c_uint64)]
 
 
 KERNEL_GRP8, KERNEL_GRP8_PRIM, KERNEL_GRP8_ALT, KERNEL_EXT64, KERNEL_LANE, KERNEL_LAB64, KERNEL_GRP8_LAB = 1, 2, 4, 8, 16, 32, 64
diff --git a/metagraph_amd/csrc/host_state.hpp b/metagraph_amd/csrc/host_state.hpp
--- a/metagraph_amd/csrc/host_state.hpp
+++ b/metagraph_amd/csrc/host_state.hpp
@@ -203,6 +203,7 @@
     uint64_t lane_done = 0;
     uint64_t lane_exact = 0;
     uint64_t lane_exact_path = 0;
+    uint64_t lane_exact_sub = 0;
     unsigned long long lane_hist_h[32] = { 0 };
     DevBuf seedlane_scratch, seedlane_params, seedlane_bail, seedlane_hist;
     uint64_t seedlane_launched = 0;
diff --git a/metagraph_amd/csrc/kernel_units.hpp b/metagraph_amd/csrc/kernel_units.hpp
--- a/metagraph_amd/csrc/kernel_units.hpp
+++ b/metagraph_amd/csrc/kernel_units.hpp
@@ -3,7 +3,7 @@
 #include <stdint.h>
 
 constexpr size_t MGX_ALIGN_PARAMS_BYTES = 728;
-constexpr size_t MGX_LANE_PARAMS_BYTES = 856;
+constexpr size_t MGX_LANE_PARAMS_BYTES = 864;
 constexpr size_t MGX_SEED_LANE_PARAMS_BYTES = 824;
 constexpr size_t MGX_DEV_GRAPH_BYTES = 160;
 constexpr size_t MGX_FORMAT_ARGS_BYTES = 128;
@@ -55,6 +55,7 @@
 
 int mgx_launch_lane(const void *d_params, uint32_t blocks, void *stream);
 int mgx_launch_lane_exact(const void *d_params, uint32_t blocks, int labeled, void *stream);
+int mgx_launch_lane_exact_sub(const void *d_params, uint32_t blocks, void *stream);
 int mgx_lane_waves_per_simd(void);
 
 int mgx_launch_seed_lane(const void *d_params, uint32_t blocks, int long_reads, void *stream);
diff --git a/metagraph_amd/csrc/lane_read.hpp b/metagraph_amd/csrc/lane_read.hpp
--- a/metagraph_amd/csrc/lane_read.hpp
+++ b/metagraph_amd/csrc/lane_read.hpp
@@ -1170,7 +1170,7 @@
 #undef f_idx
 #undef f_max_val
 
-enum { LANE_EXACT_NONE = 0, LANE_EXACT_SPAN = 1, LANE_EXACT_PATH = 2 };
+enum { LANE_EXACT_NONE = 0, LANE_EXACT_SPAN = 1, LANE_EXACT_PATH = 2, LANE_EXACT_SUB = 3 };
 
 struct alignas(16) LaneNodeQuad { uint32_t v[4]; };
 MGX_DEV bool lane_all_nodes(const uint32_t *p, const int32_t n) {
@@ -1183,6 +1183,36 @@
     }
     for (; x < n; ++x)
         if (!gld(p + x)) return false;
+    return true;
+}
+
+struct LaneZeroRun { int32_t a, b; bool ok; };
+MGX_DEV LaneZeroRun lane_zero_run_word(LaneZeroRun r, const uint32_t v, const int32_t x) {
+    if (v) return r;
+    if (r.a < 0) { r.a = x; r.b = x; }
+    else if (r.b == x - 1) r.b = x;
+    else r.ok = false;
+    return r;
+}
+MGX_DEV bool lane_one_zero_run(const uint32_t *p, const int32_t n, int32_t &lo, int32_t &hi) {
+    LaneZeroRun r = { -1, -1, true };
+    int32_t x = 0;
+    for (; x < n && ((uintptr_t)(p + x) & 15u); ++x) {
+        r = lane_zero_run_word(r, gld(p + x), x);
+        if (!r.ok) return false;
+    }
+    for (; x + 4 <= n; x += 4) {
+        const LaneNodeQuad q = gld((const LaneNodeQuad *)(p + x));
+        if (q.v[0] && q.v[1] && q.v[2] && q.v[3]) continue;
+        r = lane_zero_run_word(r, q.v[0], x); r = lane_zero_run_word(r, q.v[1], x + 1);
+        r = lane_zero_run_word(r, q.v[2], x + 2); r = lane_zero_run_word(r, q.v[3], x + 3);
+        if (!r.ok) return false;
+    }
+    for (; x < n; ++x) {
+        r = lane_zero_run_word(r, gld(p + x), x);
+        if (!r.ok) return false;
+    }
+    lo = r.a; hi = r.b;
     return true;
 }
 
@@ -1257,7 +1287,8 @@
 }
 
 template <bool LABELED>
-MGX_DEV int lane_exact_class(const LaneParams &LP, const uint64_t read, int32_t *L_out, int *strand, uint32_t hdr4[4], uint32_t *label_out) {
+MGX_DEV int lane_exact_class(const LaneParams &LP, const uint64_t read, int32_t *L_out, int *strand, uint32_t hdr4[4], uint32_t *label_out,
+                             int32_t &run_lo, int32_t &run_hi) {
     const AlignParams &P = LP.P;
     const DevConfig &cfg = P.cfg;
     if (P.labeled && (!LABELED || !(P.labeled & 2u))) return LANE_EXACT_NONE;
@@ -1301,7 +1332,18 @@
     if (full < cfg.min_path_score || full < cfg.min_cell_score) return LANE_EXACT_NONE;
     const uint32_t *rn = (s ? P.nodes_rc : P.nodes_fwd) + gld(P.node_begin + read);
     const int32_t nk = L - k + 1;
-    if (len != L) {
+    int cls = len == L ? LANE_EXACT_SPAN : LANE_EXACT_PATH;
+    if (!LABELED && len != L && LP.exact >= 3u) {
+        int32_t lo = -1, hi = -1;
+        if (!lane_one_zero_run(rn, nk, lo, hi)) return LANE_EXACT_NONE;
+        if (lo >= 0) {
+            const int32_t len_run = hi - lo + 1;
+            if (lo < 1 || len_run > k || (hi != nk - 1 && len_run != k)) return LANE_EXACT_NONE;
+            run_lo = lo; run_hi = hi;
+            cls = LANE_EXACT_SUB;
+        }
+    }
+    if ((LABELED || LP.exact < 3u) && len != L) {
         const int32_t next = len - k + 1;
         if (next > 0 && next < nk && !gld(rn + next)) return LANE_EXACT_NONE;
         if (!labeled && !lane_all_nodes(rn, nk)) return LANE_EXACT_NONE;
@@ -1309,16 +1351,17 @@
     if (labeled && !lane_all_rows(P, rn, nk, label)) return LANE_EXACT_NONE;
     *L_out = L; *strand = s; *label_out = label;
     hdr4[0] = nm0; hdr4[1] = nm1; hdr4[2] = (uint32_t)ns0; hdr4[3] = (uint32_t)ns1;
-    return len == L ? LANE_EXACT_SPAN : LANE_EXACT_PATH;
+    return cls;
 }
 
 template <bool LABELED>
-MGX_DEV int lane_exact_t(const LaneParams &LP, const uint64_t read, LaneResult &R) {
+MGX_DEV int lane_exact_t(const LaneParams &LP, const uint64_t read, LaneResult &R, int32_t &run_lo, int32_t &run_hi) {
     int32_t L = 0;
     int s = 0;
     uint32_t h[4], label = 0;
-    const int cls = lane_exact_class<LABELED>(LP, read, &L, &s, h, &label);
+    const int cls = lane_exact_class<LABELED>(LP, read, &L, &s, h, &label, run_lo, run_hi);
     if (cls == LANE_EXACT_NONE) return cls;
+    if (cls == LANE_EXACT_SUB) { R.strand = s; return cls; }
     const int32_t k = (int32_t)LP.P.g.k;
     ReadResult &rr = R.rr;
     rr.status = ST_OK; rr.n_alignments = 0; rr.score = 0; rr.offset = 0; rr.n_nodes = rr.n_cigar = rr.seq_len = 0;
@@ -1331,17 +1374,124 @@
     R.words = (uint32_t)R.n_nodes + 1u + ((uint32_t)L + 3) / 4 + ((LABELED && LP.P.labeled) ? 2u : 0u);
     return cls;
 }
+MGX_DEV uint32_t lane_sub_step(const DevGraph &g, const uint32_t vv, const uint32_t c, LineCtr &lc) {
+    const uint64_t v = vv;
+    ++lc.rank_lines;
+    const Block cur = load_block(g, (uint32_t)(v >> 6));
+    const uint32_t w = block_W(cur, (int)(v & 63));
+    if (v > 1 && w == 0) return 0;
+    Block tgt;
+    const uint64_t lst = fwd_from(g, v, cur, w % SIGMA, tgt, lc);
+    if (!lst) return 0;
+    const uint64_t e = pick_edge_from(g, lst, tgt, c, lc);
+    return (e >= 2 && in_graph(g, e)) ? (uint32_t)e : 0u;
+}
+MGX_DEV int lane_sub_children(const DevGraph &g, const uint32_t v, uint32_t *first, uint32_t *first_code, LineCtr &lc) {
+    uint64_t nodes[4] = { 0, 0, 0, 0 };
+    uint32_t codes[4] = { 0, 0, 0, 0 };
+    const int n = outgoing(g, v, nodes, codes, lc);
+    *first = (uint32_t)nodes[0]; *first_code = codes[0];
+    return n;
+}
+
+MGX_DEV bool lane_exact_sub(const LaneParams &LP, const uint64_t read, const int s, const int32_t lo, const int32_t hi,
+                            uint32_t *walk, const int32_t wstride, LaneResult &R, LineCtr &lc) {
+    const AlignParams &P = LP.P;
+    const DevConfig &cfg = P.cfg;
+    const int32_t k = (int32_t)P.g.k, m = LP.self_score;
+    const uint64_t off = gld(P.offsets + read);
+    const int32_t L = (int32_t)(gld(P.offsets + read + 1) - off);
+    const int32_t nk = L - k + 1, p = lo + k - 1;
+    if (lo < 1 || hi < lo || hi >= nk || hi - lo + 1 > k || hi - lo + 1 > LANE_SUB_MAX_WALK) return false;
+    const uint32_t *rn = (s ? P.nodes_rc : P.nodes_fwd) + gld(P.node_begin + read);
+    const uint64_t wb = packed_word_begin(off, read);
+    const uint64_t *pw = LP.pk[s] + wb;
+    for (int32_t j = 0; j < (L + 31) >> 5; ++j)
+        if (gld(LP.iv[s] + wb + j)) return false;
+    auto qcode = [&](const int32_t j) -> uint32_t { return ((uint32_t)(gld(pw + (j >> 5)) >> (2 * (j & 31))) & 3u) + 1u; };
+    uint32_t g_node = 0, g = 0;
+    const uint32_t qp = qcode(p);
+    if (lane_sub_children(P.g, gld(rn + lo - 1), &g_node, &g, lc) != 1 || g == qp) return false;
+    const int32_t mm = (int32_t)(int8_t)(LP.t4[g - 1] >> (8 * (qp - 1)));
+    const int32_t lb = cfg.left_end_bonus, rb = cfg.right_end_bonus;
+    const int32_t core = m * (L - 1) + mm + lb, score = core + rb;
+    if (score < cfg.min_path_score || score < cfg.min_cell_score) return false;
+    if (!(mm + m * (L - 1 - p) + rb > 0)) return false;
+    if (!((double)(4 * L + 1) / (double)L < cfg.max_nodes_per_seq_char)) return false;
+    if (!((double)(4 * L + 1) * (double)(272 + 24 * (L + 1)) / 1'000'000 <= cfg.max_ram_per_alignment)) return false;
+    if (core < (int32_t)((double)(m * p + lb) * cfg.rel_score_cutoff)) return false;
+    uint32_t cur = g_node;
+    walk[0] = cur;
+    for (int32_t x = 1; x <= hi - lo; ++x) {
+        const uint32_t nx = lane_sub_step(P.g, cur, qcode(p + x), lc);
+        if (!nx) return false;
+        cur = nx;
+        walk[x * wstride] = cur;
+    }
+    if (hi < nk - 1) {
+        const uint32_t nx = lane_sub_step(P.g, cur, qcode(p + k), lc);
+        if (!nx || nx != gld(rn + hi + 1)) return false;
+    }
+    for (int32_t x = imax(L - 2 * k, 0); x <= lo - 2; ++x) {
+        uint32_t f = 0, fc = 0;
+        if (lane_sub_children(P.g, gld(rn + x), &f, &fc, lc) != 1) return false;
+    }
+    const SeedHdr *hp = P.seed_hdr + read;
+    const int32_t ns0 = (int32_t)gld(&hp->n_seeds[0]), ns1 = (int32_t)gld(&hp->n_seeds[1]);
+    const DevSeed *seeds = P.seed_stream + gld(&hp->off) + (s ? ns0 : 0);
+    const int32_t n = s ? ns1 : ns0;
+    for (int32_t t = 1; t < n; ++t) {
+        const DevSeed *sj = seeds + t;
+        const int32_t cl = (int32_t)gld(&sj->clipping), len = (int32_t)gld(&sj->length), so = (int32_t)gld(&sj->offset);
+        const int32_t lpos = len + cl - 1;
+        const int32_t lscore = len * m + (!cl ? lb : 0) + (!(L - cl - len) ? rb : 0);
+        const int32_t prefix = m * (lpos + 1) + lb + (lpos >= p ? mm - m : 0) + (lpos == L - 1 ? rb : 0);
+        if (lpos < 0 || lpos >= L || prefix < lscore) return false;
+        if (so) {
+            const int32_t x = lpos - k + 1;
+            if (x < 0) return false;
+            const uint32_t on_path = (x >= lo && x <= hi) ? walk[(x - lo) * wstride] : gld(rn + x);
+            if (gld(&sj->node) != on_path) return false;
+        }
+    }
+    ReadResult &rr = R.rr;
+    rr.status = ST_OK; rr.n_alignments = 0; rr.score = 0; rr.offset = 0; rr.n_nodes = rr.n_cigar = rr.seq_len = 0;
+    rr.orientation = 0; rr.stream_off = 0;
+    rr.num_matches_fwd = gld(&hp->num_matching[0]); rr.num_matches_rc = gld(&hp->num_matching[1]);
+    rr.n_seeds_fwd = (uint32_t)ns0; rr.n_seeds_rc = (uint32_t)ns1;
+    rr.n_extensions = 0; rr.n_columns = 0;
+    R.have_aln = 1; R.mode = LANE_EMIT_EXACT; R.strand = s; R.trim = 0; R.label = g;
+    R.score = score;
+    R.offset = 0; R.clip = 0; R.end_clip = 0; R.n_runs = p == L - 1 ? 2 : 3; R.j_hi = p; R.n_nodes = nk; R.n_seq = L;
+    R.words = (uint32_t)R.n_nodes + (uint32_t)R.n_runs + ((uint32_t)L + 3) / 4;
+    return true;
+}
+static_assert(LANE_COLD_WORDS >= LANE_SUB_MAX_WALK, "the host model keeps a walk in the lane's cold words");
+
+MGX_DEV int lane_exact_walked(const LaneParams &LP, const uint64_t read, LaneResult &R, uint8_t *scratch, const LaneChip &chip) {
+    int32_t run_lo = 0, run_hi = 0;
+    const int cls = LP.P.labeled ? lane_exact_t<true>(LP, read, R, run_lo, run_hi) : lane_exact_t<false>(LP, read, R, run_lo, run_hi);
+    if (cls != LANE_EXACT_SUB) return cls;
+    if (!scratch || !chip.cold) return LANE_EXACT_NONE;
+    LineCtr lc = { 0, 0, 0 };
+    const bool ok = lane_exact_sub(LP, read, R.strand, run_lo, run_hi, chip.cold, chip.cstride, R, lc);
+    uint32_t *rec = lane_record(LP, scratch, chip.lane);
+    gst(rec + 27, gld(rec + 27) + lc.rank_lines + lc.bit_lines); gst(rec + 28, gld(rec + 28) + lc.select_lines);
+    return ok ? LANE_EXACT_SUB : LANE_EXACT_NONE;
+}
 MGX_DEV int lane_exact(const LaneParams &LP, const uint64_t read, LaneResult &R) {
-    return LP.P.labeled ? lane_exact_t<true>(LP, read, R) : lane_exact_t<false>(LP, read, R);
+    int32_t run_lo = 0, run_hi = 0;
+    const int cls = LP.P.labeled ? lane_exact_t<true>(LP, read, R, run_lo, run_hi) : lane_exact_t<false>(LP, read, R, run_lo, run_hi);
+    return cls == LANE_EXACT_SUB ? LANE_EXACT_NONE : cls;
 }
 
 MGX_DEV int lane_read(const LaneParams &LP, uint64_t read, const uint32_t item, const int pass, uint8_t *scratch, const LaneChip &chip,
                       LaneCounters &ctr, LaneResult &R) {
-    if (!pass && LP.exact && lane_exact(LP, read, R) != LANE_EXACT_NONE) return LR_DONE;
+    if (!pass && LP.exact && lane_exact_walked(LP, read, R, scratch, chip) != LANE_EXACT_NONE) return LR_DONE;
     return lane_read_dp(LP, read, item, pass, scratch, chip, ctr, R);
 }
 
-template <bool WITH_EXACT>
+template <bool WITH_EXACT, bool WITH_SUB = false>
 MGX_DEV void lane_emit_t(const LaneParams &LP, const uint64_t read, const uint8_t *scratch, const LaneChip &chip, LaneResult &R,
                          const uint64_t so) {
     const AlignParams &P = LP.P;
@@ -1370,15 +1520,23 @@
                 const uint64_t off = gld(P.offsets + read);
                 const uint32_t *rn = (R.strand ? P.nodes_rc : P.nodes_fwd) + gld(P.node_begin + read);
                 const uint64_t *pw = LP.pk[R.strand] + packed_word_begin(off, read);
-                for (int32_t x = 0; x < R.n_nodes; ++x) gst(dst + x, gld(rn + x));
-                gst(dst + R.n_nodes + nc++, ((uint32_t)R.n_seq << 3) | OP_MATCH);
+                const bool sub = WITH_SUB && R.n_runs > 1;
+                const int32_t sp = sub ? R.j_hi : -1, lo = sub ? sp - k_minus_1 : R.n_nodes;
+                for (int32_t x = 0; x < R.n_nodes; ++x) gst(dst + x, (x >= lo && x <= sp) ? chip.cold[(x - lo) * chip.cstride] : gld(rn + x));
+                if (sub) {
+                    gst(dst + R.n_nodes + nc++, ((uint32_t)sp << 3) | OP_MATCH);
+                    gst(dst + R.n_nodes + nc++, (1u << 3) | OP_MISMATCH);
+                    if (R.n_runs > 2) gst(dst + R.n_nodes + nc++, ((uint32_t)(R.n_seq - 1 - sp) << 3) | OP_MATCH);
+                } else {
+                    gst(dst + R.n_nodes + nc++, ((uint32_t)R.n_seq << 3) | OP_MATCH);
+                }
                 uint32_t *dw = dst + R.n_nodes + n_cigar;
                 uint64_t qw = 0;
                 for (int32_t x = 0; x < R.n_seq; x += 4) {
                     if (!(x & 31)) qw = gld(pw + (x >> 5));
                     uint32_t v = 0;
                     for (int t = 0; t < 4; ++t)
-                        if (x + t < R.n_seq) v |= (uint32_t)decode_code(((uint32_t)(qw >> (2 * ((x + t) & 31))) & 3u) + 1u) << (8 * t);
+                        if (x + t < R.n_seq) v |= (uint32_t)decode_code(x + t == sp ? R.label : ((uint32_t)(qw >> (2 * ((x + t) & 31))) & 3u) + 1u) << (8 * t);
                     gst(dw + (x >> 2), v);
                 }
             } else if (R.mode == LANE_EMIT_ARRAYS) {
@@ -1436,7 +1594,7 @@
 
 MGX_DEV void lane_emit(const LaneParams &LP, const uint64_t read, const uint8_t *scratch, const LaneChip &chip, LaneResult &R,
                        const uint64_t so) {
-    lane_emit_t<true>(LP, read, scratch, chip, R, so);
-}
-
-}
+    lane_emit_t<true, true>(LP, read, scratch, chip, R, so);
+}
+
+}
diff --git a/metagraph_amd/csrc/lane_types.hpp b/metagraph_amd/csrc/lane_types.hpp
--- a/metagraph_amd/csrc/lane_types.hpp
+++ b/metagraph_amd/csrc/lane_types.hpp
@@ -43,9 +43,14 @@
     unsigned long long *bail_hist;
     uint32_t exact;
     uint32_t done_key;
+    struct LaneSubCand *sub_list;
 };
+struct alignas(16) LaneSubCand { uint32_t read, strand, lo, hi; };
 constexpr int LANE_HIST_EXACT = 48;
 constexpr int LANE_HIST_EXACT_PATH = 49;
+constexpr int LANE_HIST_EXACT_SUB = 50;
+constexpr int LANE_HIST_SUB_CAND = 51;
+constexpr int LANE_SUB_MAX_WALK = 32;
 
 inline uint32_t lane_max_cols(uint32_t Lmax, int32_t xdrop) {
     return Lmax + (uint32_t)std::min<int64_t>(Lmax, std::max<int64_t>(xdrop, 0)) + 8;
@@ -77,7 +82,26 @@
     return true;
 }
 
+inline bool lane_exact_sub_config(const mgx_config &c, const DevConfig &d, uint32_t labeled_flags) {
+    if (labeled_flags || !lane_exact_config(c, d, labeled_flags)) return false;
+    const char acgt[4] = { 'A', 'C', 'G', 'T' };
+    const int m = c.score_matrix[(int)'A'][(int)'A'];
+    int lo = m, hi = -128;
+    for (int x = 0; x < 4; ++x)
+        for (int y = 0; y < 4; ++y)
+            if (x != y) { const int v = c.score_matrix[(int)acgt[x]][(int)acgt[y]]; lo = std::min(lo, v); hi = std::max(hi, v); }
+    if (!((int64_t)c.gap_opening_penalty + m < lo)) return false;
+    if (!(2 * hi - lo < m) || !(hi - lo < m)) return false;
+    if (!((int64_t)lo + c.xdrop >= 0)) return false;
+    return true;
+}
+inline uint32_t lane_exact_level(const mgx_config &c, const DevConfig &d, uint32_t labeled_flags, uint32_t level) {
+    if (!level || !lane_exact_config(c, d, labeled_flags)) return 0u;
+    return level >= 3u ? (lane_exact_sub_config(c, d, labeled_flags) ? 3u : 2u) : level;
+}
+
 constexpr bool LANE_EXACT_AUTO_LABELED = true;
+constexpr bool LANE_EXACT_AUTO_SUB = true;
 
 inline bool lane_enabled(const mgx_config &c, const DevConfig &d, uint32_t k, uint32_t Lmax, bool no_fast, LaneParams *LP, std::string *why,
                          uint32_t labeled_flags = 0) {
@@ -107,8 +131,9 @@
     if (!(c.rel_score_cutoff >= 0.0 && c.rel_score_cutoff <= 1.0)) return no("rel_score_cutoff outside [0, 1]");
     LP->self_score = m;
     const char *ex = std::getenv("MGX_EMU_LANE_EXACT");
-    const uint32_t level = (ex && (*ex == '1' || *ex == '2') && !ex[1]) ? (uint32_t)(*ex - '0') : 0u;
-    LP->exact = (level && lane_exact_config(c, d, labeled_flags)) ? level : 0u;
+    const uint32_t level = (ex && *ex >= '1' && *ex <= '3' && !ex[1]) ? (uint32_t)(*ex - '0') : 0u;
+    LP->exact = lane_exact_level(c, d, labeled_flags, level);
+    LP->sub_list = nullptr;
     return true;
 }
 
diff --git a/metagraph_amd/csrc/mgx.hip b/metagraph_amd/csrc/mgx.hip
--- a/metagraph_amd/csrc/mgx.hip
+++ b/metagraph_amd/csrc/mgx.hip
@@ -320,8 +320,10 @@
                  && (A->opt.lane == 1 || pl.n >= (uint64_t)pl.lane_blocks * 16);
     const uint32_t lflags = pl.labeled ? (1u | (A->anno_dummy_clean ? 2u : 0u)) : 0u;
     const bool exact_auto = pl.n >= (uint64_t)pl.lane_blocks * 16 && (!pl.labeled || LANE_EXACT_AUTO_LABELED);
-    LP.exact = (pl.lane_ok && A->opt.exact != 0 && lane_exact_config(A->cfg, A->dcfg, lflags)
-                && (A->opt.exact >= 1 || exact_auto)) ? (A->opt.exact >= 1 ? (uint32_t)A->opt.exact : 2u) : 0u;
+    const uint32_t exact_auto_level = (!pl.labeled && LANE_EXACT_AUTO_SUB) ? 3u : 2u;
+    LP.exact = (pl.lane_ok && A->opt.exact != 0 && (A->opt.exact >= 1 || exact_auto))
+                   ? lane_exact_level(A->cfg, A->dcfg, lflags, A->opt.exact >= 1 ? (uint32_t)A->opt.exact : exact_auto_level) : 0u;
+    LP.sub_list = nullptr;
     pl.key_bits = work_key_bits(pl.n) + (LP.exact ? 1 : 0);
     LP.done_key = LP.exact ? 1u << work_key_bits(pl.n) : 0u;
     if (!pl.lane_ok) return MGX_OK;
@@ -548,7 +550,7 @@
 
 static int prepare_lane(mgx_aligner *A, AlignPlan &pl) {
     LaneParams &LP = pl.LP;
-    if (int rc = A->lane_bail.ensure(pl.n * 4 + 4)) return rc;
+    if (int rc = A->lane_bail.ensure(std::max<uint64_t>(pl.n * 4 + 4, LP.exact >= 3u ? pl.n * sizeof(LaneSubCand) : 0))) return rc;
     if (int rc = A->lane_params.ensure(sizeof(LaneParams))) return rc;
     if (int rc = A->lane_hist.ensure(64 * 8)) return rc;
     HIP_TRY(hipMemsetAsync(A->lane_hist.p, 0, 64 * 8, A->hstream));
@@ -557,6 +559,7 @@
     LP.iv[0] = A->iv_fwd.as<uint32_t>(); LP.iv[1] = A->iv_rc.as<uint32_t>();
     LP.scratch = A->lane_scratch.as<uint8_t>();
     LP.bail_list = A->lane_bail.as<uint32_t>();
+    LP.sub_list = A->lane_bail.as<LaneSubCand>();
     LP.bail_count = cursor(A, CUR_LANE_BAIL);
     LP.done_count = cursor(A, CUR_LANE_DONE);
     LP.bail_hist = A->lane_hist.as<unsigned long long>();
@@ -570,14 +573,19 @@
     HIP_TRY(copy_sync(A, A->lane_params.p, &LP, sizeof(LP), hipMemcpyHostToDevice));
     const uint32_t blocks = (uint32_t)std::min<uint64_t>((uint64_t)pl.cus * 4 * 8 * 4, (pl.n + 63) / 64);
     if (int rc = mgx_launch_lane_exact(A->lane_params.p, blocks, pl.labeled ? 1 : 0, A->hstream)) return fail(MGX_ERR_NO_DEVICE, "lane kernel, exact exit: %d", rc);
+    if (LP.exact >= 3u && !pl.labeled) {
+        if (int rc = mgx_launch_lane_exact_sub(A->lane_params.p, blocks, A->hstream)) return fail(MGX_ERR_NO_DEVICE, "lane kernel, exact exit (substitutions): %d", rc);
+    }
     unsigned long long done = 0;
     HIP_TRY(copy_sync(A, &done, cursor(A, CUR_LANE_DONE), 8, hipMemcpyDeviceToHost));
     pl.n_exact = done;
-    unsigned long long path = 0;
+    static_assert(LANE_HIST_EXACT_SUB == LANE_HIST_EXACT_PATH + 1, "read back together");
+    unsigned long long apart[2] = { 0, 0 };
     if (LP.exact >= 2u && done)
-        HIP_TRY(copy_sync(A, &path, A->lane_hist.as<unsigned long long>() + LANE_HIST_EXACT_PATH, 8, hipMemcpyDeviceToHost));
-    A->lane_exact = done - path;
-    A->lane_exact_path = path;
+        HIP_TRY(copy_sync(A, apart, A->lane_hist.as<unsigned long long>() + LANE_HIST_EXACT_PATH, LP.exact >= 3u ? 16 : 8, hipMemcpyDeviceToHost));
+    A->lane_exact = done - apart[0] - apart[1];
+    A->lane_exact_path = apart[0];
+    A->lane_exact_sub = apart[1];
     return MGX_OK;
 }
 
@@ -743,7 +751,7 @@
     A->n_passes = 1;
     A->lane_done = 0;
     A->lane_exact = 0;
-    A->lane_exact_path = 0;
+    A->lane_exact_path = A->lane_exact_sub = 0;
     memset(A->lane_hist_h, 0, sizeof(A->lane_hist_h));
     bool multi = false;
     const bool exact = pl.lane_ok && pl.LP.exact && n;
@@ -773,7 +781,7 @@
     if (int rc = seed_stage(A, d_seqs, d_offsets, n, Lmax, false, pl)) return rc;
     for (AlignEvent e : { EV_SORTED, EV_LANE_END, EV_ALIGN_END }) HIP_TRY(hipEventRecord(A->ev[e], A->hstream));
     A->n_passes = 0;
-    A->lane_done = A->lane_exact = A->lane_exact_path = 0;
+    A->lane_done = A->lane_exact = A->lane_exact_path = A->lane_exact_sub = 0;
     memset(A->lane_hist_h, 0, sizeof(A->lane_hist_h));
     unsigned long long wanted = 0;
     HIP_TRY(copy_sync(A, &wanted, cursor(A, CUR_SEED), 8, hipMemcpyDeviceToHost));
@@ -798,6 +806,7 @@
     s.n_lane_reads = A->lane_done;
     s.n_lane_exact_reads = A->lane_exact;
     s.n_lane_exact_path_reads = A->lane_exact_path;
+    s.n_lane_exact_sub_reads = A->lane_exact_sub;
     s.n_lane_lines = ks.lane_lines; s.n_lane_columns = ks.lane_columns;
     for (int x = 0; x < 32; ++x) s.lane_bail_reads[x] = A->lane_hist_h[x];
     if (int on; aligned && A->seedlane_launched && env_int("MGX_SL_TIMERS", &on)) {
@@ -877,7 +886,7 @@
         else if (key == "no_flat") o.no_flat = v;
         else if (key == "lane") o.lane = v;
         else if (key == "exact") {
-            if (v < -1 || v > 2) return fail(MGX_ERR_INVALID, "unknown option '%s'", name);
+            if (v < -1 || v > 3) return fail(MGX_ERR_INVALID, "unknown option '%s'", name);
             o.exact = v;
         }
         else if (key == "device_share") o.device_share = std::max(1, std::min(v, 64));
diff --git a/metagraph_amd/csrc/mgx_lane.hip b/metagraph_amd/csrc/mgx_lane.hip
--- a/metagraph_amd/csrc/mgx_lane.hip
+++ b/metagraph_amd/csrc/mgx_lane.hip
@@ -141,8 +141,25 @@
         LaneResult R;
         R.words = 0;
         LV<bool> hv;
-        const int cls = read < n_reads ? lane_exact_t<LABELED>(LP, read, R) : LANE_EXACT_NONE;
-        hv.v = cls != LANE_EXACT_NONE;
+        int32_t run_lo = 0, run_hi = 0;
+        const int cls = read < n_reads ? lane_exact_t<LABELED>(LP, read, R, run_lo, run_hi) : LANE_EXACT_NONE;
+        if constexpr (!LABELED) {
+            LV<bool> cv;
+            cv.v = cls == LANE_EXACT_SUB;
+            const uint64_t cm = wave_ballot(cv);
+            if (cm) {
+                LV<uint64_t> pv;
+                pv.v = 0;
+                if (lane == 0) pv.v = atomicAdd(LP.bail_hist + LANE_HIST_SUB_CAND, (unsigned long long)popc64(cm));
+                const uint64_t p0 = wave_bcast(pv, 0) + (uint64_t)popc64(cm & ((1ull << lane) - 1));
+                if (cv.v) {
+                    LaneSubCand c;
+                    c.read = (uint32_t)read; c.strand = (uint32_t)R.strand; c.lo = (uint32_t)run_lo; c.hi = (uint32_t)run_hi;
+                    gst(LP.sub_list + p0, c);
+                }
+            }
+        }
+        hv.v = cls == LANE_EXACT_SPAN || cls == LANE_EXACT_PATH;
         if (!wave_ballot(hv)) continue;
         LV<int32_t> wv;
         wv.v = hv.v ? (int32_t)R.words : 0;
@@ -171,6 +188,62 @@
 }
 
 __global__ void __launch_bounds__(64) k_lane_exact(const LaneParams *__restrict__ LPp) { lane_exact_body<false>(*LPp); }
+
+__global__ void __launch_bounds__(64) k_lane_exact_sub(const LaneParams *__restrict__ LPp) {
+    const LaneParams &LP = *LPp;
+    __shared__ uint32_t s_walk[LANE_SUB_MAX_WALK][64];
+    const int lane = (int)threadIdx.x;
+    const uint64_t n_cand = (uint64_t)gld(LP.bail_hist + LANE_HIST_SUB_CAND);
+    LaneChip chip;
+    chip.lane = lane; chip.qw = nullptr; chip.qstride = 0; chip.cold = &s_walk[0][lane]; chip.cstride = 64;
+    LineCtr lc = { 0, 0, 0 };
+    uint32_t n_done = 0, n_cap = 0;
+    for (uint64_t base = (uint64_t)blockIdx.x * 64; base < n_cand; base += (uint64_t)gridDim.x * 64) {
+        const uint64_t at = base + (uint64_t)lane;
+        LaneResult R;
+        R.words = 0;
+        LV<bool> hv;
+        hv.v = false;
+        uint64_t read = 0;
+        if (at < n_cand) {
+            const LaneSubCand c = gld(LP.sub_list + at);
+            read = c.read;
+            hv.v = lane_exact_sub(LP, read, (int)c.strand, (int32_t)c.lo, (int32_t)c.hi, chip.cold, chip.cstride, R, lc);
+        }
+        if (!wave_ballot(hv)) continue;
+        LV<int32_t> wv;
+        wv.v = hv.v ? (int32_t)R.words : 0;
+        const LV<int32_t> pre = wave_prefix_sum_excl(wv);
+        const int32_t total = wave_sum(wv);
+        LV<uint64_t> sv;
+        sv.v = 0;
+        if (lane == 0) sv.v = atomicAdd(LP.P.out_cursor, (unsigned long long)total);
+        const uint64_t so = wave_bcast(sv, 0) + (uint64_t)pre.v;
+        if (hv.v) {
+            lane_emit_t<true, true>(LP, read, nullptr, chip, R, so);
+            gst(LP.P.work_key + read, LP.done_key);
+            ++n_done; n_cap += (uint32_t)(R.rr.status != ST_OK);
+        }
+    }
+    LV<int32_t> v;
+    v.v = (int32_t)n_done; const int32_t nd = wave_sum(v);
+    v.v = (int32_t)n_cap; const int32_t nc = wave_sum(v);
+    v.v = (int32_t)(lc.rank_lines + lc.bit_lines); const int32_t rl = wave_sum(v);
+    v.v = (int32_t)lc.select_lines; const int32_t sl = wave_sum(v);
+    if (lane == 0) {
+        if (nd) {
+            atomicAdd(LP.done_count, (unsigned long long)nd);
+            atomicAdd(LP.bail_hist + LANE_HIST_EXACT, (unsigned long long)nd);
+            atomicAdd(LP.bail_hist + LANE_HIST_EXACT_SUB, (unsigned long long)nd);
+        }
+        if (nc) atomicAdd(&LP.P.stats->capacity_errors, (unsigned long long)nc);
+        if (rl | sl) {
+            atomicAdd(&LP.P.stats->rank_lines, (unsigned long long)rl);
+            atomicAdd(&LP.P.stats->select_lines, (unsigned long long)sl);
+            atomicAdd(&LP.P.stats->lane_lines, (unsigned long long)rl + (unsigned long long)sl);
+        }
+    }
+}
 __global__ void __launch_bounds__(64) k_lane_exact_labeled(const LaneParams *__restrict__ LPp) { lane_exact_body<true>(*LPp); }
 
 extern "C" int mgx_launch_lane(const void *d_params, uint32_t blocks, void *stream) {
@@ -183,4 +256,8 @@
     else k_lane_exact<<<blocks, 64, 0, (hipStream_t)stream>>>(static_cast<const LaneParams *>(d_params));
     return (int)hipGetLastError();
 }
+extern "C" int mgx_launch_lane_exact_sub(const void *d_params, uint32_t blocks, void *stream) {
+    k_lane_exact_sub<<<blocks, 64, 0, (hipStream_t)stream>>>(static_cast<const LaneParams *>(d_params));
+    return (int)hipGetLastError();
+}
 extern "C" int mgx_lane_waves_per_simd(void) { return MGX_LANE_WAVES_PER_SIMD; }
```
